# JuanLuisGonzalez/FAL_net

Measured on AMD Instinct MI355X. Metric: stereo-pairs/sec Stage-1 step @256x512 N=49, higher is better.
Workload: dtype bf16; 1 GPU; Stage-1 training step (BASELINE configs[1]), batch 8/GPU, 256x512, N=49, seeded weights, seeded VGG19; global_batch=8, parallelism=dp1, launch=eager launches, recorded sequences issued by falnet_replay (C)

## Files before the change

### fal_net_amd/_lib.py

```python
import ctypes as C
import os
import threading

import torch

F32, BF16, F16 = 0, 1, 2
ACT_NONE, ACT_ELU, ACT_RELU = 0, 1, 2
OUT_NHWC, OUT_PLANAR_F32 = 0, 1
CPAD = 32

DETERMINISTIC = os.environ.get("FALNET_DETERMINISTIC") == "1"

def ab(name, default):
    if os.environ.get("FALNET_AB") != "1":
        return default
    return os.environ.get(name, default)


_LIB_PATH = os.environ.get("FALNET_LIB") or os.path.join(os.path.dirname(os.path.abspath(__file__)), "libfalnet_hip.so")


class Src(C.Structure):
    _fields_ = [("ptr", C.c_void_p), ("C", C.c_int32), ("H", C.c_int32), ("W", C.c_int32),
                ("sb", C.c_int64), ("sy", C.c_int64), ("sx", C.c_int64)]


class Conv(C.Structure):
    _fields_ = [("src", Src * 2), ("nsrc", C.c_int32), ("IH", C.c_int32), ("IW", C.c_int32),
                ("weight", C.c_void_p), ("cin_total", C.c_int32), ("ntaps", C.c_int32),
                ("tap_dy", C.c_int32 * 9), ("tap_dx", C.c_int32 * 9), ("tap_w", C.c_int32 * 9),
                ("w_taps", C.c_int32), ("w_rows", C.c_int32), ("isy", C.c_int32), ("isx", C.c_int32),
                ("B", C.c_int32), ("TH", C.c_int32), ("TW", C.c_int32),
                ("osy", C.c_int32), ("osx", C.c_int32), ("ooy", C.c_int32), ("oox", C.c_int32),
                ("out", C.c_void_p), ("OH", C.c_int32), ("OW", C.c_int32), ("Cout", C.c_int32),
                ("out_cstride", C.c_int32), ("out_layout", C.c_int32), ("bias", C.c_void_p),
                ("addend", C.c_void_p), ("act", C.c_int32), ("actout", C.c_void_p),
                ("actout_kind", C.c_int32), ("dtype", C.c_int32), ("ksplit", C.c_int32), ("splitk_ws", C.c_void_p),
                ("splitk_ws_bytes", C.c_int64), ("variant", C.c_int32), ("pool_out", C.c_void_p),
                ("pool_mode", C.c_int32), ("pool_actout_kind", C.c_int32), ("pool_actout", C.c_void_p), ("weight_up2", C.c_void_p),
                ("scratch", C.c_void_p), ("scratch_bytes", C.c_int64)]


class Wgrad(C.Structure):
    _fields_ = [("src", Src * 2), ("nsrc", C.c_int32), ("IH", C.c_int32), ("IW", C.c_int32),
                ("gout", C.c_void_p), ("gC", C.c_int32), ("ntaps", C.c_int32),
                ("tap_dy", C.c_int32 * 9), ("tap_dx", C.c_int32 * 9), ("isy", C.c_int32), ("isx", C.c_int32),
                ("B", C.c_int32), ("TH", C.c_int32), ("TW", C.c_int32), ("cin_total", C.c_int32),
                ("nsplit", C.c_int32), ("partial", C.c_void_p), ("dtype", C.c_int32), ("variant", C.c_int32), ("bias_grad", C.c_void_p),
                ("cout", C.c_int32), ("up2", C.c_int32)]


class ReduceDesc(C.Structure):
    _fields_ = [("partial", C.c_void_p), ("grad", C.c_void_p), ("nsplit", C.c_int32), ("ntaps", C.c_int32),
                ("w_rows", C.c_int32), ("cin_total", C.c_int32), ("cout", C.c_int32), ("cin", C.c_int32),
                ("c0_real", C.c_int32), ("c0_pad", C.c_int32), ("groups", C.c_int32), ("block_begin", C.c_int32)]


class PackDesc(C.Structure):
    _fields_ = [("w", C.c_void_p), ("wf", C.c_void_p), ("wd", C.c_void_p), ("cout", C.c_int32), ("cin", C.c_int32),
                ("taps", C.c_int32), ("c0_real", C.c_int32), ("c0_pad", C.c_int32), ("cin_pad", C.c_int32),
                ("cout_pad", C.c_int32), ("block_begin", C.c_int32), ("no_update", C.c_int32), ("reserved", C.c_int32)]


class PackUp2Desc(C.Structure):
    _fields_ = [("w", C.c_void_p), ("wu", C.c_void_p), ("cout", C.c_int32), ("cin", C.c_int32), ("cin_pad", C.c_int32), ("cout_pad", C.c_int32),
                ("block_begin", C.c_int32), ("reserved", C.c_int32), ("wdd", C.c_void_p)]


class Cmd(C.Structure):
    _fields_ = [("op", C.c_int32), ("stream", C.c_int32), ("event", C.c_int32), ("nint", C.c_int32), ("nflt", C.c_int32), ("reserved", C.c_int32),
                ("iarg", C.c_uint64 * 18), ("farg", C.c_double * 8)]


CMD_RECORD, CMD_WAIT = -1, -2


class BiasGradDesc(C.Structure):
    _fields_ = [("g", C.c_void_p), ("db", C.c_void_p), ("npix", C.c_int64), ("gC", C.c_int32), ("cout", C.c_int32),
                ("blocks", C.c_int32), ("block_begin", C.c_int32)]


class Aug(C.Structure):
    _fields_ = [("src", C.c_uint64 * 2), ("H", C.c_int32), ("W", C.c_int32), ("rw", C.c_int32), ("rh", C.c_int32), ("x1", C.c_int32),
                ("y1", C.c_int32), ("flip", C.c_int32), ("reserved", C.c_int32), ("gamma", C.c_double), ("bright", C.c_double),
                ("cb", (C.c_double * 3) * 2)]


_P, _I, _L, _F, _D = C.c_void_p, C.c_int, C.c_int64, C.c_float, C.c_double
SIGNATURES = {
    "falnet_version": [],
    "falnet_last_error": [],
    "falnet_channel_pad": [_I],
    "falnet_set_device": [_I],
    "falnet_set_deterministic": [_I],
    "falnet_get_deterministic": [],
    "falnet_conv2d": [C.POINTER(Conv), _P],
    "falnet_conv3x3_c3": [_P, _P, _P, _P, _I, _I, _I, _I, _I, _I, _P],
    "falnet_conv2d_multi": [C.POINTER(Conv), _I, _P],
    "falnet_conv2d_kernel_name": [C.POINTER(Conv), C.c_char_p, _I],
    "falnet_wgrad_workspace_bytes": [C.POINTER(Wgrad)],
    "falnet_wgrad": [C.POINTER(Wgrad), _P],
    "falnet_wgrad_fuses_bias": [C.POINTER(Wgrad)],
    "falnet_wgrad_reduce": [_P, _I, _I, _I, _I, _P, _I, _I, _I, _I, _I, _P],
    "falnet_bias_grad": [_P, _L, _I, _I, _P, _I, _I, _P],
    "falnet_pack_weights_batched": [_P, _I, _I, _I, _P],
    "falnet_adam_pack_batched": [_P, _I, _I, _I, _L, _L, _L, _P, _F, _F, _F, _F, _P, _P],
    "falnet_adam_ranges": [_P, _L, _L, _L, _P, _I, _P, _F, _F, _F, _F, _P, _P],
    "falnet_adam_tick": [_P, _P, _P],
    "falnet_adam_pack_batched_wd": [_P, _I, _I, _I, _L, _L, _L, _P, _F, _F, _F, _F, _D, _P, _P],
    "falnet_adam_ranges_wd": [_P, _L, _L, _L, _P, _P, _I, _P, _F, _F, _F, _F, _P, _P],
    "falnet_pack_up2_batched": [_P, _I, _I, _I, _P],
    "falnet_wgrad_reduce_batched": [_P, _I, _I, _I, _P],
    "falnet_wgrad_reduce_blocks": [_I, _I, _I],
    "falnet_bias_grad_batched": [_P, _I, _I, _I, _P],
    "falnet_bias_grad_batched_det": [_P, _I, _I, _I, _P, _L, _P],
    "falnet_pack_weights": [_P, _I, _I, _I, _I, _I, _I, _I, _P, _P, _I, _P],
    "falnet_nchw_to_nhwc": [_P, _P, _I, _I, _I, _I, _I, _I, _P],
    "falnet_nhwc_to_nchw": [_P, _P, _I, _I, _I, _I, _I, _I, _P],
    "falnet_upsample_bwd": [_P, _P, _P, _I, _I, _I, _I, _I, _I, _I, _P],
    "falnet_wgrad_const_plane": [_P, _P, _L, _P, _L, _P, _I, _I, _I, _I, _I, _I, _I, _I, _I, _P],
    "falnet_maxpool2_fwd": [_P, _P, _I, _I, _I, _I, _I, _P],
    "falnet_maxpool2_bwd": [_P, _P, _P, _P, _I, _I, _I, _I, _I, _P],
    "falnet_act_bwd": [_P, _P, _P, _L, _I, _I, _P],
    "falnet_med_head_fwd": [_P, _P, _P, _P, _P, _P, _P, _I, _I, _I, _I, _P],
    "falnet_med_head_bwd": [_P, _P, _P, _P, _P, _P, _P, _P, _P, _P, _I, _I, _I, _I, _P],
    "falnet_med_head_bwd_nhwc": [_P, _P, _P, _P, _P, _P, _P, _P, _P, _P, _I, _I, _I, _I, _I, _I, _P],
    "falnet_med_head_kernel_name": [_I, _I, _I, _I, C.c_char_p, _I],
    "falnet_med_masks_fwd": [_P, _P, _P, _P, _P, _P, _I, _I, _I, _I, _P],
    "falnet_med_maskr_acfalse_fwd": [_P, _P, _P, _P, _P, _I, _I, _I, _I, _P],
    "falnet_l1_fwd": [_P, _P, _P, _I, _I, _L, _F, _P, _I, _P],
    "falnet_l1_bwd": [_P, _P, _P, _I, _I, _L, _F, _P, _P, _I, _P],
    "falnet_mse_fwd": [_P, _P, _L, _I, _F, _P, _I, _I, _P],
    "falnet_mse_bwd": [_P, _P, _L, _I, _F, _P, _P, _I, _P],
    "falnet_l1_fwd_bwd": [_P, _P, _I, _I, _L, _F, _P, _P, _P, _P],
    "falnet_l1_fwd_bwd_add": [_P, _P, _I, _I, _L, _F, _P, _P, _P, _P, _P],
    "falnet_mse_fwd_bwd": [_P, _P, _L, _I, _F, _P, _F, _P, _P, _I, _P],
    "falnet_mse3_fwd_bwd": [_P, _P, _P, _P, _P, _P, _P, _P, _I, _P],
    "falnet_smooth_fwd_bwd": [_P, _P, _I, _I, _I, _I, _I, _F, _F, _P, _P, _P, _P],
    "falnet_smooth_fwd": [_P, _P, _I, _I, _I, _I, _I, _F, _F, _P, _I, _P],
    "falnet_smooth_bwd": [_P, _P, _I, _I, _I, _I, _I, _F, _F, _P, _P, _I, _P],
    "falnet_step_scalars": [_P, _F, _P, _P],
    "falnet_mask_mix": [_P, _P, _P, _P, _I, _I, _L, _P],
    "falnet_adam_step": [_P, _P, _P, _P, _L, _F, _F, _F, _F, _I, _F, _P],
    "falnet_adam_step_dev": [_P, _P, _P, _P, _L, _P, _F, _F, _F, _F, _P],
    "falnet_adam_step_guarded": [_P, _P, _P, _P, _L, _P, _F, _F, _F, _F, _P, _P],
    "falnet_adam_step_wd": [_P, _P, _P, _P, _L, _P, _P, _I, _P, _F, _F, _F, _F, _P, _P],
    "falnet_grad_guard": [_P, _L, _P, _P],
    "falnet_loss_scale_update": [_P, _F, _F, _I, _F, _F, _P],
    "falnet_loss_seeds": [_P, _P, _P, _I, _P],
    "falnet_hflip": [_P, _P, _L, _I, _P],
    "falnet_resample_u8": [_P, _P, _I, _I, _I, _I, _I, _P, _P, _I, _P],
    "falnet_augment_normalize": [_P, _I, _I, _I, _I, _I, _I, _I, _D, _D, _D, _D, _D, _F, _F, _F, _P, _P],
    "falnet_augment_batch": [_P, _P, _I, _I, _I, _F, _F, _F, _P, _P, _P],
    "falnet_rowmax": [_P, _P, _I, _L, _P],
    "falnet_gemm_f32_small": [_P, _L, _L, _P, _L, _L, _P, _I, _I, _I, _I, _P],
    "falnet_resize_planar": [_P, _P, _L, _I, _I, _I, _I, _I, _F, _P],
    "falnet_disp_prologue": [_P, _P, _F, _F, _P, _P, _P, _I, _I, _I, _P],
    "falnet_occlusion_mask": [_P, _P, _P, _I, _I, _I, _I, _I, _P],
    "falnet_mirror_weight": [_P, _P, _P, _I, _I, _I, _I, _I, _P],
    "falnet_replay_op_index": [C.c_char_p],
    "falnet_replay_op_args": [_I, C.POINTER(C.c_int), C.POINTER(C.c_int)],
    "falnet_replay": [_P, _I, _P, _I, _P, _I, C.POINTER(C.c_int)],
    "falnet_fill_f32": [_P, _L, _F, _P],
    "falnet_copy_bytes": [_P, _P, _L, _P],
    "falnet_spin": [_I, _P],
    "falnet_mfma_probe": [_P, _P, _I, _I, _P],
    "falnet_percentile_workspace_bytes": [_I],
    "falnet_percentile_f32": [_P, _L, _I, _D, _P, _P, _P],
    "falnet_disp_to_plasma_u8": [_P, _P, _P, _P, _I, _I, _I, _P],
    "falnet_image_to_u8": [_P, _F, _F, _F, _P, _I, _I, _I, _P],
    "falnet_feature_to_u8": [_P, _P, _L, _P],
    "falnet_local_norm": [_P, _F, _F, _F, _P, _P, _P, _I, _I, _I, _I, _P],
    "falnet_point_cloud": [_P, _F, _F, _F, _F, _P, _D, _D, _P, _P, _I, _I, _I, _P],
    "falnet_metrics_workspace_bytes": [],
    "falnet_depth_median_scale": [_P, _P, _I, _I, _I, _D, _D, _P, _P, _P],
    "falnet_depth_errors": [_P, _P, _I, _I, _I, _D, _P, _D, _D, _P, _P, _P],
    "falnet_epe": [_P, _I, _I, _P, _I, _I, _I, _I, _P, _P, _P],
    "falnet_view_errors": [_P, _P, _F, _F, _F, _I, _I, _I, _P, _P, _P],
}
_RESTYPES = {"falnet_last_error": C.c_char_p, "falnet_wgrad_workspace_bytes": C.c_int64, "falnet_percentile_workspace_bytes": C.c_int64,
             "falnet_metrics_workspace_bytes": C.c_int64}

_lib = None
_TLS = threading.local()
EXPECTED_VERSION = 600


def lib():
    global _lib
    if _lib is None:
        if not os.path.exists(_LIB_PATH):
            raise RuntimeError(
                f"{_LIB_PATH} is missing: build it with `python -m fal_net_amd._build` "
                "(there is no CPU or PyTorch fallback for the FAL_netB kernels)")
        l = C.CDLL(_LIB_PATH)
        for name, args in SIGNATURES.items():
            fn = getattr(l, name)
            fn.argtypes = args
            fn.restype = _RESTYPES.get(name, C.c_int)
        got = l.falnet_version()
        if got != EXPECTED_VERSION:
            raise RuntimeError(f"{_LIB_PATH} reports falnet_version() = {got}, this binding expects {EXPECTED_VERSION}: rebuild it "
                               "(`python -m fal_net_amd._build`; experiment builds: `--ab <tag>`)")
        if DETERMINISTIC:
            l.falnet_set_deterministic(1)
        _lib = _LibProxy(l)
    return _lib


_MASK64 = (1 << 64) - 1


def _int_arg(a):
    if a is None:
        return 0
    if isinstance(a, int):
        return a & _MASK64
    if isinstance(a, C.c_void_p):
        return a.value or 0
    if isinstance(a, (C.Structure, C.Array)):
        return C.addressof(a)
    obj = getattr(a, "_obj", None)
    if obj is not None:
        return C.addressof(obj)
    if isinstance(a, C._SimpleCData):
        return int(a.value or 0) & _MASK64
    raise TypeError(f"cannot record argument {a!r}")


class Segment:

    def __init__(self, cmds, streams, events, keep):
        self.n = len(cmds)
        self.cmds = (Cmd * max(self.n, 1))(*cmds)
        self.streams = (C.c_void_p * len(streams))(*streams)
        self.events = (C.c_void_p * max(len(events), 1))(*events)
        self.ns, self.ne = len(streams), len(events)
        self.failed = C.c_int(-1)
        self._keep = keep
        self._fn = _lib._cdll.falnet_replay

    def run(self, main_ptr):
        self.streams[0] = main_ptr
        rc = self._fn(self.cmds, self.n, self.streams, self.ns, self.events, self.ne, C.byref(self.failed))
        if rc != 0:
            msg = _lib._cdll.falnet_last_error().decode(errors="replace")
            raise RuntimeError(f"libfalnet_hip replay failed at command {self.failed.value} (rc={rc}): {msg}")


class SegmentChain:

    def __init__(self, parts):
        self.parts = parts

    def run(self, main_ptr):
        for p in self.parts:
            if isinstance(p, Segment):
                p.run(main_ptr)
            else:
                p()


class Recorder:

    def __init__(self, main_ptr):
        self.streams = [int(main_ptr or 0)]
        self.events, self.cmds, self.keep = [], [], []
        self.parts = []
        self._ops = {}

    def cut(self, fn):
        self.parts.append(self.cmds)
        self.parts.append(fn)
        self.cmds = []

# ... 164 lines not shown
```

### fal_net_amd/csrc/conv.hip

```cpp
#include <limits.h>
#include <stdlib.h>
#include <type_traits>
#include "common.h"
#include "conv_epilogue.h"

#define CONV_THREADS 256
#define CONV_BM 128
#define ROWB 64
#define ROWP 80

template <typename T> struct KC;
template <> struct KC<float> { static constexpr int value = 16; };
template <> struct KC<bf16_t> { static constexpr int value = 32; };
template <> struct KC<f16_t> { static constexpr int value = 32; };

template <typename T, int MT, int NT, typename RowOff, typename PoolOff = NoPool>
__device__ __forceinline__ void epilogue_nhwc(const falnet_conv_t& p, f32x16 (&acc)[MT][NT], float* stage, int nbase, int lane,
                                              RowOff rowoff, PoolOff pooloff = PoolOff()) {
    constexpr bool POOL = !std::is_same<PoolOff, NoPool>::value;
    constexpr int PITCHF = NT * 32 + 4;
    constexpr int CS = NT * 4;
    constexpr int RPP = 64 / CS;
    constexpr int PASSES = 32 / RPP;
    const int r = lane & 31, h = lane >> 5;
// ... 1326 lines not shown
    if constexpr (sizeof(T) == 2) {
#pragma unroll
        for (int ks = 0; ks < 2; ++ks)
#pragma unroll
            for (int nt = 0; nt < NT; ++nt)
#pragma unroll
                for (int j = 0; j < 8; ++j) bfr[ks][nt][j] = (short)H16<T>::bits(wv[ks][nt][j]);
    }
    constexpr int MT = PT_TH / 4;
    auto a_elem = [&](const float* base, int k0, int k1) -> float {
        const int o0 = k0 < 27 ? ((k0 / 9) * PH + (k0 % 9) / 3) * PW + (k0 % 9) % 3 : 0;
        const int o1 = k1 < 27 ? ((k1 / 9) * PH + (k1 % 9) / 3) * PW + (k1 % 9) % 3 : 0;
        const float v = base[h ? o1 : o0];
        return ((h ? k1 : k0) < 27) ? v : 0.f;
    };
    const int cstride = p.out_cstride;
    const int tiles_x = (p.OW + PT_TW - 1) / PT_TW;
    C3_STAMP(2);
    __syncthreads();
    C3_STAMP(3);
    for (int tt = 0; tt < C3_TPW; ++tt) {
        if (tt == 1) C3_STAMP(4);
        const int tix = tix0 + tt;
        if (tix >= tiles_x) break;
        const int tx0 = tix * PT_TW;
#pragma unroll 1
        for (int mt = 0; mt < MT; ++mt) {
            f32x16 acc[1][NT];
#pragma unroll
            for (int nt = 0; nt < NT; ++nt)
#pragma unroll
                for (int j = 0; j < 16; ++j) acc[0][nt][j] = 0.f;
            const float* base = patch + (wave * MT + mt) * PW + tt * PT_TW + r;
            if constexpr (sizeof(T) == 2) {
#pragma unroll
                for (int ks = 0; ks < 2; ++ks) {
                    s16x8_t afr;
#pragma unroll
                    for (int j = 0; j < 8; ++j) afr[j] = (short)H16<T>::bits(a_elem(base, ks * 16 + j, ks * 16 + 8 + j));
#pragma unroll
                    for (int nt = 0; nt < NT; ++nt) acc[0][nt] = H16<T>::mma(bfr[ks][nt], afr, acc[0][nt]);
                }
            } else {
#pragma unroll
                for (int ks = 0; ks < 16; ++ks) {
                    const float a = a_elem(base, ks * 2, ks * 2 + 1);
#pragma unroll
                    for (int nt = 0; nt < NT; ++nt) acc[0][nt] = __builtin_amdgcn_mfma_f32_32x32x2f32(wv[ks][nt][0], a, acc[0][nt], 0, 0, 0);
                }
            }
            auto pixoff = [&](int) -> int64_t {
                const int y = ty0 + wave * MT + mt, xx = tx0 + r;
                return (y < p.OH && xx < p.OW) ? (((int64_t)b * p.OH + y) * p.OW + xx) * cstride : (int64_t)-1;
            };
            epilogue_direct<T, 1, NT, decltype(pixoff), NoPool, 1, false, true>(p, acc, bias, 0, lane, pixoff);
        }
    }
    C3_STAMP(5);
    asm volatile("s_waitcnt vmcnt(0)" ::: "memory");
    C3_STAMP(6);
}
#undef C3_STAMP

template <typename T, bool SWAP>
static void launch_conv(const falnet_conv_t& p, int bn, dim3 grid, hipStream_t st) {
    if (bn == 128)
        hipLaunchKernelGGL(HIP_KERNEL_NAME(conv_igemm_kernel<T, 128, SWAP>), grid, dim3(CONV_THREADS), 0, st, p);
    else if (bn == 64)
        hipLaunchKernelGGL(HIP_KERNEL_NAME(conv_igemm_kernel<T, 64, SWAP>), grid, dim3(CONV_THREADS), 0, st, p);
    else
        hipLaunchKernelGGL(HIP_KERNEL_NAME(conv_igemm_kernel<T, 32, SWAP>), grid, dim3(CONV_THREADS), 0, st, p);
}

static bool falnet_mfma16_enabled() {
    static const bool on = [] { const char* e = falnet_ab_env("FALNET_MFMA16"); return !(e && e[0] == '0'); }();
    return on;
}

enum class ConvFamily {
    Gather,
    Patch,
    WeightStationary,
    Dma,
    S2fDma,
    Up2Dma,
    Deep,
    Dma2,
    Dma16,
    Up2d,
    Wave32,
    Wave64p,
};
struct ConvChoice {
    ConvFamily family;
    int bn, kcb, tps, adb, th, nwaves, flip, swap;
};

static bool g_disable_patch = [] { const char* e = falnet_ab_env("FALNET_DISABLE_PATCH"); return e && e[0] == '1'; }();
static int g_patch_kcb = [] { const char* e = falnet_ab_env("FALNET_PATCH_KCB"); return e ? atoi(e) : 128; }();


bool falnet_conv_dma_applicable(const falnet_conv_t& p, int min_oh);
int falnet_conv_dma_launch(const falnet_conv_t& p, int flip, hipStream_t st, int th);
bool falnet_conv_dma2_applicable(const falnet_conv_t& p, int th);
int falnet_conv_dma2_launch(const falnet_conv_t& p, int flip, hipStream_t st, int th);
int falnet_conv_dma16_launch(const falnet_conv_t& p, int flip, hipStream_t st, int th);
bool falnet_conv_up2_dma_applicable(const falnet_conv_t& p);
int falnet_conv_up2_dma_launch(const falnet_conv_t& p, hipStream_t st);
bool falnet_conv_wave32_applicable(const falnet_conv_t& p);
int falnet_conv_wave32_launch(const falnet_conv_t& p, int flip, hipStream_t st);
bool falnet_conv_wave64p_applicable(const falnet_conv_t& p);
int falnet_conv_wave64p_launch(const falnet_conv_t& p, int flip, hipStream_t st);
bool falnet_conv_up2d_applicable(const falnet_conv_t& p);
int falnet_conv_up2d_launch(const falnet_conv_t& p, hipStream_t st);
bool falnet_conv_deep_applicable(const falnet_conv_t& p);
int falnet_conv_deep_launch(const falnet_conv_t& p, hipStream_t st);
int falnet_conv_deep_mtiles(const falnet_conv_t& p);
bool falnet_conv_s2d_dma_applicable(const falnet_conv_t* d, int n);
int falnet_conv_s2d_dma_launch(const falnet_conv_t* d, hipStream_t st);
bool falnet_conv_s2f_dma_applicable(const falnet_conv_t& p);
int falnet_conv_s2f_dma_launch(const falnet_conv_t& p, hipStream_t st);

static int choose_conv_kernel(const falnet_conv_t& p, ConvChoice& c) {
    const bool planar = p.out_layout == FALNET_OUT_PLANAR_F32;
    int ctot = 0;
    for (int s = 0; s < p.nsrc; ++s) ctot += p.src[s].C;
    bool dense3x3 = p.ntaps == 9 && p.isy == 1 && p.isx == 1 && p.osy == 1 && p.osx == 1 && p.ooy == 0 && p.oox == 0 &&
                    p.TH == p.OH && p.TW == p.OW && p.TH == p.IH && p.TW == p.IW && p.TW >= 16;
    int flip = -1;
    if (dense3x3 && p.w_taps == 9) {
        bool fwd = true, bwd = true;
        for (int t = 0; t < 9; ++t) {
            const int sp = (p.tap_dy[t] + 1) * 3 + (p.tap_dx[t] + 1);
            if (p.tap_dy[t] < -1 || p.tap_dy[t] > 1 || p.tap_dx[t] < -1 || p.tap_dx[t] > 1) fwd = bwd = false;
            fwd = fwd && p.tap_w[t] == sp;
            bwd = bwd && p.tap_w[t] == 8 - sp;
        }
        flip = fwd ? 0 : (bwd ? 1 : -1);
    }
    dense3x3 = dense3x3 && flip >= 0;
    const int esz = p.dtype == FALNET_F32 ? 4 : 2;
    bool c128 = true;
    for (int s = 0; s < p.nsrc; ++s) c128 = c128 && (p.src[s].C % (128 / esz) == 0);
    int variant = p.variant;
    int forced_bn = 0;
    if (variant == 11 || variant == 12) {
        forced_bn = variant == 11 ? 32 : 64;
        if (p.w_rows % forced_bn != 0 || p.pool_out) {
            falnet_set_error("conv2d: variant %d (gather, %d channels per workgroup) not applicable to this launch", variant, forced_bn);
            return -2;
        }
        variant = 1;
    }
    if (g_disable_patch) variant = 1;
    switch (variant) {
        case 0: case 1: case 2: case 3: case 4: case 5: case 6: case 7: case 8: case 9: case 10:
        case 13: case 15: case 16: case 17: case 18: case 19: case 20: case 21: case 22: case 23: case 24: case 25: case 26: case 27: case 29:
            break;
        default:
            falnet_set_error("conv2d: unknown variant %d", variant);
            return -1;
    }
    if (variant == 19) {
        if (!falnet_conv_deep_applicable(p)) {
            falnet_set_error("conv2d: variant 19 needs a 16-bit nine-tap stride-1/2 launch on maps of at most 128 positions (128 %% (TH TW) == 0), dense NHWC output, "
                             "w_rows %% 64 == 0, ksplit = cin_total / 32 or / 64 (a multiple of 4), scratch for the partial tiles and the split-K workspace");
            return -2;
        }
        c.flip = 0;
        c.swap = 0;
        c.family = ConvFamily::Deep;
        c.bn = 64; c.kcb = p.ksplit * 32 == p.cin_total ? 1 : 2; c.tps = 9; c.adb = 1; c.th = 0; c.nwaves = falnet_conv_deep_mtiles(p);
        return 0;
    }
    if (variant == 15) {
        if (!falnet_conv_s2f_dma_applicable(p)) {
            falnet_set_error("conv2d: variant 15 needs a canonical 16-bit 3x3 stride-2 pad-1 NHWC launch (>= 8 x 32 outputs) with sources at the input size");
            return -2;
        }
        c.flip = 0;
        c.swap = 0;
        c.family = ConvFamily::S2fDma;
        c.bn = 64; c.kcb = 32; c.tps = 9; c.adb = 1; c.th = 8; c.nwaves = 8;
        return 0;
    }
    if (variant == 29) {
        if (!(dense3x3 && falnet_conv_wave64p_applicable(p))) {
            falnet_set_error("conv2d: variant 29 needs a 16-bit dense 3x3 stride-1 launch over ONE 64-channel source at the launch size, planar f32 output of <= 4 channels, no addend / activation-gradient operand / pool / split-K");
            return -2;
        }
        c.flip = flip;
        c.swap = 0;
        c.family = ConvFamily::Wave64p;
        c.bn = 16; c.kcb = 32; c.tps = 9; c.adb = 1; c.th = 1; c.nwaves = 8;
        return 0;
    }
    if (variant == 27) {
        if (!(dense3x3 && falnet_conv_wave32_applicable(p))) {
            falnet_set_error("conv2d: variant 27 needs a 16-bit dense 3x3 stride-1 NHWC launch over ONE 32-channel source at the launch size with a 32-row packed weight, no pool / split-K");
            return -2;
        }
        c.flip = flip;
        c.swap = 0;
        c.family = ConvFamily::Wave32;
        c.bn = 32; c.kcb = 32; c.tps = 9; c.adb = 1; c.th = 1; c.nwaves = 8;
        return 0;
    }
    if (variant == 26) {
        if (!(falnet_conv_up2d_applicable(p) && p.ntaps == 4 && p.isy == 1 && p.isx == 1 && p.osy == 1 && p.osx == 1 && p.ooy == 0 && p.oox == 0 && p.TH == p.OH && p.TW == p.OW)) {
            falnet_set_error("conv2d: variant 26 needs a 16-bit NHWC launch over ONE source at exactly twice the output map (>= 16 x 32), w_taps = ntaps = 4, cin_total = 4 C, no pool / split-K");
            return -2;
        }
        c.flip = 0;
        c.swap = 0;
        c.family = ConvFamily::Up2d;
        c.bn = 64; c.kcb = 32; c.tps = 4; c.adb = 1; c.th = 16; c.nwaves = 8;
        return 0;
    }
    if (variant == 18) {
        if (!(dense3x3 && flip == 0 && !p.addend && !p.actout && falnet_conv_up2_dma_applicable(p))) {
            falnet_set_error("conv2d: variant 18 needs a 16-bit dense 3x3 forward launch over ONE source at exactly half the launch size, weight_up2 set, no residual / activation-gradient operand");
            return -2;
        }
        c.flip = 0;
        c.swap = 0;
        c.family = ConvFamily::Up2Dma;
        c.bn = 32; c.kcb = 64; c.tps = 16; c.adb = 1; c.th = 16; c.nwaves = 8;
        return 0;
    }
    if (variant >= 23 && variant <= 25) {
        const int th = variant == 23 ? 16 : (variant == 24 ? 4 : 8);
        if (!(dense3x3 && falnet_conv_dma_applicable(p, th)) || (th != 16 && (p.pool_out || planar)) || (planar && p.pool_out)) {
            falnet_set_error("conv2d: variant %d needs a 16-bit dense 3x3 stride-1 launch (>= %d x 32 positions%s) with sources at the launch size or half of it",
                             variant, th, th != 16 ? ", NHWC output, no fused pool" : "");
            return -2;
        }
        c.flip = flip;
        c.swap = 0;
        c.family = ConvFamily::Dma16;
        c.bn = 64; c.kcb = 32; c.tps = 9; c.adb = 1; c.th = th; c.nwaves = th == 4 ? 4 : 8;
        return 0;
    }
    if (variant == 21 || variant == 22) {
        const int th = variant == 21 ? 16 : 32;
        if (!(dense3x3 && falnet_conv_dma2_applicable(p, th))) {
            falnet_set_error("conv2d: variant %d needs a 16-bit dense 3x3 stride-1 NHWC launch (>= %d x 32 positions) with sources at the launch size or half of it", variant, th);
            return -2;
        }
        c.flip = flip;
        c.swap = 0;
        c.family = ConvFamily::Dma2;
        c.bn = 64; c.kcb = 16; c.tps = 9; c.adb = 1; c.th = th; c.nwaves = th / 4;
        return 0;
    }
    if (variant == 13 || variant == 17 || variant == 20) {
        const int th = variant == 17 ? 4 : (variant == 20 ? 8 : 16);
        if (!(dense3x3 && falnet_conv_dma_applicable(p, th)) || (th != 16 && p.pool_out)) {
            falnet_set_error("conv2d: variant %d needs a 16-bit dense 3x3 stride-1 launch (>= %d x 32 positions%s) with sources at the launch size or half of it",
                             variant, th, th != 16 ? ", no fused pool" : "");
            return -2;
        }
        c.flip = flip;
        c.swap = 0;
        c.family = ConvFamily::Dma;
        c.bn = 64; c.kcb = 64; c.tps = 9; c.adb = 1; c.th = th; c.nwaves = th == 4 ? 4 : 8;
        return 0;
    }
    if (variant == 10 || variant == 16) {
        bool ok = dense3x3 && ctot * esz <= 128 && ctot * esz % 64 == 0 && p.src[0].C * esz % 64 == 0;
        for (int s = 0; s < p.nsrc && ok; ++s)
            ok = (p.src[s].H == p.IH || 2 * p.src[s].H == p.IH) && (p.src[s].W == p.IW || 2 * p.src[s].W == p.IW) && p.src[s].C < 4096;
        if (!ok) {
            falnet_set_error("conv2d: variant 10 needs a dense 3x3 launch with <= 128 B of input channels per pixel");
            return -2;
        }
        c.flip = flip;
        c.swap = 0;
        c.family = ConvFamily::WeightStationary;
        c.bn = (p.w_rows % 64 == 0 && p.Cout > 32) ? 64 : 32;
        c.kcb = ctot * esz / 64;
        c.tps = 9; c.adb = variant == 16; c.th = (c.bn == 64 ? 8 : 16) >> c.adb; c.nwaves = 8;
        return 0;
    }
    if (variant >= 2 && (!dense3x3 || (variant == 2 && !c128) || ((variant == 3 || variant == 5 || variant == 6 || variant == 8) && ctot / (64 / esz) < 2) ||
                         ((variant == 6 || variant == 7) && p.OH < 16))) {
        falnet_set_error("conv2d: variant %d not applicable to this launch", variant);
        return -2;
    }
    if (variant == 0) {
        if (!dense3x3 || p.TW < 32) variant = 1;
        else if (c128 && g_patch_kcb == 128) variant = 2;
        else if (ctot / (64 / esz) >= 2 && g_patch_kcb != 0) variant = 3;
        else variant = 4;
    }
    const bool bn64 = p.w_rows % 64 == 0 && p.Cout > 32;
    c.flip = flip;
    c.swap = planar ? 1 : 0;
    c.family = variant >= 2 ? ConvFamily::Patch : ConvFamily::Gather;
    if (p.pool_out && c.family == ConvFamily::Gather) {
        falnet_set_error("conv2d: the fused max pool needs a halo-patch variant (dense 3x3 stride-1 launch)");
        return -2;
    }
    if (c.family == ConvFamily::Gather) {
        c.bn = forced_bn ? forced_bn : (p.w_rows % 128 == 0 && p.Cout > 64) ? 128 : (bn64 ? 64 : 32);
        c.kcb = 64; c.tps = 1; c.adb = 0; c.th = 0; c.nwaves = 4;
        return 0;
    }
    c.th = variant >= 8 ? 4 : (variant >= 6 ? 16 : 8);
    c.nwaves = (variant == 6 || variant == 7) ? 8 : 4;
    const int tiles = p.B * ((p.OW + PT_TW - 1) / PT_TW) * ((p.OH + c.th - 1) / c.th);
    const bool bn128 = p.w_rows % 128 == 0 && p.Cout > 64 && (c.th == 16 || tiles >= 256);
    switch (variant) {
        case 2: c.bn = bn128 ? 128 : (bn64 ? 64 : 32); c.kcb = 128; c.tps = 1; c.adb = ctot / (128 / esz) > 1; break;
        case 3: case 6: c.bn = bn128 ? 128 : (bn64 ? 64 : 32); c.kcb = 64; c.tps = 1; c.adb = 1; break;
        case 8: c.bn = bn64 ? 64 : 32; c.kcb = 64; c.tps = 1; c.adb = 1; break;
        case 5: c.bn = bn64 ? 64 : 32; c.kcb = 64; c.tps = 9; c.adb = 1; break;
        default: c.bn = bn64 ? 64 : 32; c.kcb = 64; c.tps = 9; c.adb = 0; break;
    }
    if (p.pool_out && (c.th / (c.nwaves / (c.bn >= 128 ? 2 : 1))) % 2 != 0) {
        falnet_set_error("conv2d: variant %d gives every wave an odd number of rows: no fused max pool", variant);
        return -2;
    }
    return 0;
}

static bool ws2_whole_lines(const falnet_conv_t& p) {
    static const bool on = !(falnet_ab_env("FALNET_WS2_FULL") && atoi(falnet_ab_env("FALNET_WS2_FULL")) == 0);
    return on && p.nsrc == 1 && (int64_t)p.src[0].C * (p.dtype == FALNET_F32 ? 4 : 2) == 128;
}

static int launch_gather(const falnet_conv_t& p, const ConvChoice& c, hipStream_t st) {
    const bool planar = p.out_layout == FALNET_OUT_PLANAR_F32;
    const int bn = c.bn;
    const int64_t M = (int64_t)p.B * p.TH * p.TW;
    int ksplit = p.ksplit > 1 ? p.ksplit : 1;
    if (ksplit > 1) {
        FALNET_CHECK_ARG(!planar && p.splitk_ws && p.Cout % 8 == 0, "conv2d: split-K needs an NHWC output and a workspace");
        FALNET_CHECK_ARG(M * p.w_rows * 4 <= p.splitk_ws_bytes, "conv2d: split-K workspace too small (%lld needed)", (long long)(M * p.w_rows * 4));
    }
    const dim3 grid((unsigned)((M + CONV_BM - 1) / CONV_BM), (unsigned)((p.Cout + bn - 1) / bn), (unsigned)ksplit);
#define GATHER_L(T)                                          \
    if (planar) launch_conv<T, true>(p, bn, grid, st);       \
    else launch_conv<T, false>(p, bn, grid, st);
    FALNET_DISPATCH_DTYPE(p.dtype, GATHER_L);
#undef GATHER_L
    if (ksplit > 1) {
        const int64_t total = M * (p.w_rows / 8);
        const unsigned eg = (unsigned)((total + 255) / 256 > 2048 ? 2048 : (total + 255) / 256);
#define SPLITK_E(T) hipLaunchKernelGGL(splitk_epilogue_kernel<T>, dim3(eg), dim3(256), 0, st, p)
        FALNET_DISPATCH_DTYPE(p.dtype, SPLITK_E);
#undef SPLITK_E
    }
    return 0;
}

static int launch_patch(const falnet_conv_t& p, const ConvChoice& c, hipStream_t st) {
    const int tiles_x = (p.OW + PT_TW - 1) / PT_TW, tiles_y = (p.OH + c.th - 1) / c.th;
    const dim3 grid((unsigned)(p.B * tiles_x * tiles_y), (unsigned)((p.Cout + c.bn - 1) / c.bn));
    bool launched = false;
#define TRY_PATCH(T, BN, KCB, TPS, ADB, TH, NW)                                                                              \
    if (!launched && c.bn == BN && c.kcb == KCB && c.tps == TPS && c.adb == (ADB ? 1 : 0) && c.th == TH) {                     \
    hipLaunchKernelGGL(HIP_KERNEL_NAME(conv3x3_patch_kernel<T, BN, KCB, TPS, ADB, TH, NW>), grid, dim3(NW * 64), 0, st, p, \
                       tiles_x, tiles_y, c.flip);                                                                          \
    launched = true;                                                                                                       \
    }
#define PATCH_TABLE(T)                                                                                   \
    TRY_PATCH(T, 128, 128, 1, true, 8, 4) TRY_PATCH(T, 64, 128, 1, true, 8, 4) TRY_PATCH(T, 32, 128, 1, true, 8, 4)      \
    TRY_PATCH(T, 128, 128, 1, false, 8, 4) TRY_PATCH(T, 64, 128, 1, false, 8, 4) TRY_PATCH(T, 32, 128, 1, false, 8, 4)   \
    TRY_PATCH(T, 128, 64, 1, true, 8, 4) TRY_PATCH(T, 64, 64, 1, true, 8, 4) TRY_PATCH(T, 32, 64, 1, true, 8, 4)         \
    TRY_PATCH(T, 64, 64, 9, false, 8, 4) TRY_PATCH(T, 32, 64, 9, false, 8, 4)                                             \
    TRY_PATCH(T, 64, 64, 9, true, 8, 4) TRY_PATCH(T, 32, 64, 9, true, 8, 4)                                               \
    TRY_PATCH(T, 128, 64, 1, true, 16, 8) TRY_PATCH(T, 64, 64, 1, true, 16, 8) TRY_PATCH(T, 32, 64, 1, true, 16, 8)      \
    TRY_PATCH(T, 64, 64, 9, false, 16, 8) TRY_PATCH(T, 32, 64, 9, false, 16, 8)                                           \
    TRY_PATCH(T, 64, 64, 1, true, 4, 4) TRY_PATCH(T, 32, 64, 1, true, 4, 4)                                               \
    TRY_PATCH(T, 64, 64, 9, false, 4, 4) TRY_PATCH(T, 32, 64, 9, false, 4, 4)
    FALNET_DISPATCH_DTYPE(p.dtype, PATCH_TABLE);
#undef PATCH_TABLE
#undef TRY_PATCH
    FALNET_CHECK_ARG(launched, "conv2d: no instantiation for bn=%d kcb=%d tps=%d adb=%d th=%d", c.bn, c.kcb, c.tps, c.adb, c.th);
    return 0;
}

static int launch_ws(const falnet_conv_t& p, const ConvChoice& c, hipStream_t st) {
    const int ws_th = c.th;
    const int tiles_x = (p.OW + PT_TW - 1) / PT_TW, tiles_y = (p.OH + ws_th - 1) / ws_th;
    const int ny = (p.Cout + c.bn - 1) / c.bn, ntiles = p.B * tiles_x * tiles_y;
    int gx = 256 / ny;
    if (gx < 1) gx = 1;
    if (gx > ntiles) gx = ntiles;
    const dim3 grid((unsigned)gx, (unsigned)ny);
    const bool m16 = falnet_mfma16_enabled();
    const bool ws2_full = ws2_whole_lines(p);
#define LAUNCH_WS1(K, T, BN, NCH) do { if (m16 && sizeof(T) == 2) hipLaunchKernelGGL(HIP_KERNEL_NAME(K<T, BN, NCH, true>), grid, dim3(512), 0, st, p, tiles_x, tiles_y, c.flip); \
                                   else hipLaunchKernelGGL(HIP_KERNEL_NAME(K<T, BN, NCH, false>), grid, dim3(512), 0, st, p, tiles_x, tiles_y, c.flip); } while (0)
#define LAUNCH_WS2(T, BN, NCH) do { if (NCH == 2 && ws2_full) { if (m16 && sizeof(T) == 2) hipLaunchKernelGGL(HIP_KERNEL_NAME(conv3x3_ws2_kernel<T, BN, 2, true, true>), grid, dim3(512), 0, st, p, tiles_x, tiles_y, c.flip); \
                                     else hipLaunchKernelGGL(HIP_KERNEL_NAME(conv3x3_ws2_kernel<T, BN, 2, false, true>), grid, dim3(512), 0, st, p, tiles_x, tiles_y, c.flip); } \
                                 else LAUNCH_WS1(conv3x3_ws2_kernel, T, BN, NCH); } while (0)
#define LAUNCH_WS(T, BN, NCH) do { if (c.adb) LAUNCH_WS2(T, BN, NCH); else LAUNCH_WS1(conv3x3_ws_kernel, T, BN, NCH); } while (0)
#define WS_TABLE(T)                                                                                 \
    if (c.bn == 64) { if (c.kcb == 2) LAUNCH_WS(T, 64, 2); else LAUNCH_WS(T, 64, 1); }              \
    else { if (c.kcb == 2) LAUNCH_WS(T, 32, 2); else LAUNCH_WS(T, 32, 1); }
    FALNET_DISPATCH_DTYPE(p.dtype, WS_TABLE);
#undef WS_TABLE
#undef LAUNCH_WS
#undef LAUNCH_WS1
#undef LAUNCH_WS2
    return 0;
}

static int ws_symbol(char* buf, int len, const char* t, const falnet_conv_t& p, const ConvChoice& c) {
    const int m16 = (int)(falnet_mfma16_enabled() && p.dtype != FALNET_F32);
    if (c.adb) return snprintf(buf, len, "_Z18conv3x3_ws2_kernelI%sLi%dELi%dELb%dELb%dEEv13falnet_conv_tiii", t, c.bn, c.kcb, m16, (int)(c.kcb == 2 && ws2_whole_lines(p)));
    return snprintf(buf, len, "_Z17conv3x3_ws_kernelI%sLi%dELi%dELb%dEEv13falnet_conv_tiii", t, c.bn, c.kcb, m16);
}

struct ConvFamilyRow {
    ConvFamily family;
    int (*symbol)(char* buf, int len, const char* t, const falnet_conv_t& p, const ConvChoice& c);
    int (*launch)(const falnet_conv_t& p, const ConvChoice& c, hipStream_t st);
};
#define SYMBOL(...) [](char* buf, int len, const char* t, const falnet_conv_t& p, const ConvChoice& c) { return snprintf(buf, len, __VA_ARGS__); }
#define LAUNCH(...) [](const falnet_conv_t& p, const ConvChoice& c, hipStream_t st) { return __VA_ARGS__; }
static const ConvFamilyRow conv_families[] = {
    {ConvFamily::Gather, SYMBOL("_Z17conv_igemm_kernelI%sLi%dELb%dEEv13falnet_conv_t", t, c.bn, c.swap), launch_gather},
    {ConvFamily::Patch, SYMBOL("_Z20conv3x3_patch_kernelI%sLi%dELi%dELi%dELb%dELi%dELi%dEEv13falnet_conv_tiii", t, c.bn, c.kcb, c.tps, c.adb, c.th, c.nwaves), launch_patch},
    {ConvFamily::WeightStationary, ws_symbol, launch_ws},
    {ConvFamily::Dma, SYMBOL("_Z18conv3x3_dma_kernelI%sLi%dELi%dEEv13falnet_conv_tiiii", t, c.th, c.nwaves), LAUNCH(falnet_conv_dma_launch(p, c.flip, st, c.th))},
    {ConvFamily::S2fDma, SYMBOL("_Z22conv3x3_s2f_dma_kernelI%sLi%dEEv13falnet_conv_tiii", t, c.bn), LAUNCH(falnet_conv_s2f_dma_launch(p, st))},
    {ConvFamily::Up2Dma, SYMBOL("_Z22conv3x3_up2_dma_kernelI%sEv13falnet_conv_tiiiii", t), LAUNCH(falnet_conv_up2_dma_launch(p, st))},
    {ConvFamily::Deep, SYMBOL("_Z19conv3x3_deep_kernelI%sLi%dELi%dEEv13falnet_conv_t18falnet_deep_geom_t", t, c.kcb, c.nwaves), LAUNCH(falnet_conv_deep_launch(p, st))},
    {ConvFamily::Dma2, SYMBOL("_Z19conv3x3_dma2_kernelI%sLb%dELi%dEEv13falnet_conv_tiiiii", t, p.pool_out ? 1 : 0, c.nwaves), LAUNCH(falnet_conv_dma2_launch(p, c.flip, st, c.th))},
    {ConvFamily::Dma16, SYMBOL("_Z20conv3x3_dma16_kernelI%sLb%dELi%dELi%dELb%dEEv13falnet_conv_tiiii", t, p.pool_out ? 1 : 0, c.th, c.nwaves, p.out_layout == FALNET_OUT_PLANAR_F32 ? 1 : 0),
     LAUNCH(falnet_conv_dma16_launch(p, c.flip, st, c.th))},
    {ConvFamily::Up2d, SYMBOL("_Z25conv2x2_up2d_dma16_kernelI%sEv13falnet_conv_tiii", t), LAUNCH(falnet_conv_up2d_launch(p, st))},
    {ConvFamily::Wave32, SYMBOL("_Z21conv3x3_wave32_kernelI%sEv13falnet_conv_tiiii", t), LAUNCH(falnet_conv_wave32_launch(p, c.flip, st))},
    {ConvFamily::Wave64p, SYMBOL("_Z22conv3x3_wave64p_kernelI%sEv13falnet_conv_tiiii", t), LAUNCH(falnet_conv_wave64p_launch(p, c.flip, st))},
};
#undef SYMBOL
#undef LAUNCH

static const ConvFamilyRow* conv_family_row(ConvFamily f) {
    for (const ConvFamilyRow& r : conv_families)
        if (r.family == f) return &r;
    falnet_set_error("conv2d: kernel family %d has no table row", (int)f);
    return nullptr;
}

extern "C" int falnet_conv2d_kernel_name(const falnet_conv_t* pp, char* buf, int len) {
    FALNET_CHECK_ARG(pp && buf && len > 0, "conv2d_kernel_name: bad argument");
    ConvChoice c;
    if (int r = choose_conv_kernel(*pp, c)) return r;
    const ConvFamilyRow* row = conv_family_row(c.family);
    if (!row) return -1;
    row->symbol(buf, len, pp->dtype == FALNET_BF16 ? "DF16b" : pp->dtype == FALNET_F16 ? "DF16_" : "f", *pp, c);
    return 0;
}

extern "C" int falnet_conv2d(const falnet_conv_t* pp, void* stream) {
    FALNET_ENTER(stream);
    FALNET_CHECK_ARG(pp, "conv2d: null descriptor");
    const falnet_conv_t& p = *pp;
    FALNET_CHECK_ARG(p.dtype == FALNET_F32 || p.dtype == FALNET_BF16 || p.dtype == FALNET_F16, "conv2d: bad dtype %d", p.dtype);
    const int kc = p.dtype == FALNET_F32 ? 16 : 32;
    FALNET_CHECK_ARG(p.nsrc == 1 || p.nsrc == 2, "conv2d: nsrc=%d", p.nsrc);
    int ctot = 0;
    for (int s = 0; s < p.nsrc; ++s) {
        if (int r = check_src(p.src[s], kc, "conv2d")) return r;
        ctot += p.src[s].C;
    }
    FALNET_CHECK_ARG(ctot <= p.cin_total, "conv2d: sources carry %d channels, packed weight row holds %d", ctot, p.cin_total);
    FALNET_CHECK_ARG(p.ntaps >= 1 && p.ntaps <= 9 && p.w_taps >= 1, "conv2d: ntaps=%d", p.ntaps);
    for (int t = 0; t < p.ntaps; ++t) FALNET_CHECK_ARG(p.tap_w[t] >= 0 && p.tap_w[t] < p.w_taps, "conv2d: tap_w[%d] out of range", t);
    FALNET_CHECK_ARG(p.B > 0 && p.TH > 0 && p.TW > 0 && p.IH > 0 && p.IW > 0 && p.OH > 0 && p.OW > 0, "conv2d: empty shape");
    FALNET_CHECK_ARG(p.weight && (p.out || p.pool_out) && p.Cout > 0 && p.w_rows >= p.Cout && p.w_rows % 32 == 0, "conv2d: bad weight/out (Cout=%d w_rows=%d)", p.Cout, p.w_rows);
    FALNET_CHECK_ARG(!p.pool_out || (p.out_layout == FALNET_OUT_NHWC && !p.actout && p.ksplit <= 1 && (p.pool_mode == 0 || p.pool_mode == 1)),
                     "conv2d: pool_out needs a plain NHWC launch (no actout / split-K) and pool_mode 0|1");
    FALNET_CHECK_ARG((int64_t)p.B * p.OH * p.OW * (p.out_layout == FALNET_OUT_PLANAR_F32 ? p.Cout : 1) < (1ll << 31), "conv2d: output too large for 32-bit pixel index");
    const bool planar = p.out_layout == FALNET_OUT_PLANAR_F32;
    FALNET_CHECK_ARG(!planar || (!p.addend && !p.actout), "conv2d: planar output supports bias/act epilogue only");
    if (p.ksplit > 1 && p.variant != 19 && falnet_deterministic()) {
        falnet_set_error("conv2d: split-K (f32 atomics) is not available in deterministic mode");
        return -2;
    }
    hipStream_t st = (hipStream_t)stream;
    ConvChoice c;
    if (int r = choose_conv_kernel(p, c)) return r;
    const ConvFamilyRow* row = conv_family_row(c.family);
    if (!row) return -1;
    if (int r = row->launch(p, c, st)) return r;
    FALNET_RETURN_LAUNCH();
}

extern "C" int falnet_conv3x3_c3(const float* x_nchw, const float* w_oihw, const float* bias, void* out, int B, int H, int W, int Cout,
                                 int act, int dtype, void* stream) {
    FALNET_ENTER(stream);
    FALNET_CHECK_ARG(x_nchw && w_oihw && out && B > 0 && H > 0 && W > 0, "conv3x3_c3: bad argument");
    FALNET_CHECK_ARG(Cout == 32 || Cout == 64, "conv3x3_c3: Cout must be 32 or 64 (got %d)", Cout);
    falnet_conv_t p = {};
    p.IH = p.OH = H;
    p.IW = p.OW = W;
    p.out = out;
    p.Cout = Cout;
    p.out_cstride = Cout;
    p.bias = bias;
    p.act = act;
#ifdef C3_STAMPS
    if (const char* e = getenv("FALNET_C3_STAMP_PTR")) p.pool_actout = reinterpret_cast<const void*>(strtoull(e, nullptr, 10));
#endif
    const int tiles_x = ((W + PT_TW - 1) / PT_TW + C3_TPW - 1) / C3_TPW , tiles_y = (H + PT_TH - 1) / PT_TH;
    const dim3 grid((unsigned)(B * tiles_x * tiles_y));
    hipStream_t st = (hipStream_t)stream;
#define C3_L(T)                                                                                                                                          \
    if (Cout == 64) hipLaunchKernelGGL(HIP_KERNEL_NAME(conv3x3_c3_kernel<T, 2>), grid, dim3(CONV_THREADS), 0, st, x_nchw, w_oihw, p, tiles_x, tiles_y); \
    else hipLaunchKernelGGL(HIP_KERNEL_NAME(conv3x3_c3_kernel<T, 1>), grid, dim3(CONV_THREADS), 0, st, x_nchw, w_oihw, p, tiles_x, tiles_y);
    FALNET_CHECK_ARG(dtype == FALNET_F32 || dtype == FALNET_BF16 || dtype == FALNET_F16, "conv3x3_c3: bad dtype %d", dtype);
    FALNET_DISPATCH_DTYPE(dtype, C3_L);
#undef C3_L
    FALNET_RETURN_LAUNCH();
}

extern "C" int falnet_conv2d_multi(const falnet_conv_t* descs, int n, void* stream) {
    FALNET_ENTER(stream);
    FALNET_CHECK_ARG(descs && n >= 1 && n <= 4, "conv2d_multi: 1..4 descriptors");
    if (descs[0].variant == 14) {
        for (int i = 0; i < n; ++i)
            for (int s = 0; s < descs[i].nsrc && s < 2; ++s)
                if (int r = check_src(descs[i].src[s], 32, "conv2d_multi")) return r;
        FALNET_CHECK_ARG(falnet_conv_s2d_dma_applicable(descs, n), "conv2d_multi: variant 14 needs the four parity classes of one 16-bit 3x3 stride-2 data gradient");
        return falnet_conv_s2d_dma_launch(descs, (hipStream_t)stream);
    }
    if (descs[0].ksplit > 1 && falnet_deterministic()) {
        falnet_set_error("conv2d_multi: split-K (f32 atomics) is not available in deterministic mode");
        return -2;
    }
    falnet_conv4_t pp;
    int64_t maxM = 0;
    ConvChoice c0;
    for (int i = 0; i < n; ++i) {
        const falnet_conv_t& p = descs[i];
        FALNET_CHECK_ARG(p.dtype == descs[0].dtype && p.w_rows == descs[0].w_rows && p.Cout == descs[0].Cout && p.out_layout == FALNET_OUT_NHWC &&
                         p.ksplit == descs[0].ksplit && p.nsrc >= 1 && p.nsrc <= 2 && p.weight && p.out && p.ntaps >= 1 && p.ntaps <= 9,
                         "conv2d_multi: members must share dtype / Cout / w_rows / ksplit and be plain NHWC gather launches");
        if (p.ksplit > 1) {
            const int64_t need = (int64_t)p.B * p.TH * p.TW * p.w_rows * 4;
            FALNET_CHECK_ARG(p.splitk_ws && p.Cout % 8 == 0 && need <= p.splitk_ws_bytes, "conv2d_multi: split-K needs a workspace of %lld bytes per member", (long long)need);
            for (int j = 0; j < i; ++j) {
                const char* a = (const char*)p.splitk_ws; const char* bq = (const char*)descs[j].splitk_ws;
                const int64_t needj = (int64_t)descs[j].B * descs[j].TH * descs[j].TW * descs[j].w_rows * 4;
                FALNET_CHECK_ARG(a + need <= bq || bq + needj <= a, "conv2d_multi: split-K workspace regions of members %d and %d overlap", j, i);
            }
        }
        for (int s = 0; s < p.nsrc; ++s)
            if (int r = check_src(p.src[s], p.dtype == FALNET_F32 ? 16 : 32, "conv2d_multi")) return r;
        ConvChoice c;
        falnet_conv_t q = p;
        q.variant = (p.variant == 11 || p.variant == 12) ? p.variant : 1;
        if (int r = choose_conv_kernel(q, c)) return r;
        if (i == 0) c0 = c;
        const int64_t M = (int64_t)p.B * p.TH * p.TW;
        maxM = M > maxM ? M : maxM;
        pp.c[i] = p;
    }
    for (int i = n; i < 4; ++i) pp.c[i] = descs[0];
    const int ksplit = descs[0].ksplit > 1 ? descs[0].ksplit : 1;
    const dim3 grid((unsigned)((maxM + CONV_BM - 1) / CONV_BM), (unsigned)((descs[0].Cout + c0.bn - 1) / c0.bn), (unsigned)(n * ksplit));
    hipStream_t st = (hipStream_t)stream;
#define LAUNCH_MULTI(T)                                                                                              \
    do {                                                                                                             \
        if (c0.bn == 128) hipLaunchKernelGGL(HIP_KERNEL_NAME(conv_igemm_multi_kernel<T, 128>), grid, dim3(CONV_THREADS), 0, st, pp, ksplit); \
        else if (c0.bn == 64) hipLaunchKernelGGL(HIP_KERNEL_NAME(conv_igemm_multi_kernel<T, 64>), grid, dim3(CONV_THREADS), 0, st, pp, ksplit); \
        else hipLaunchKernelGGL(HIP_KERNEL_NAME(conv_igemm_multi_kernel<T, 32>), grid, dim3(CONV_THREADS), 0, st, pp, ksplit);  \
    } while (0)
    FALNET_DISPATCH_DTYPE(descs[0].dtype, LAUNCH_MULTI);
#undef LAUNCH_MULTI
    if (ksplit > 1) {
        const int64_t total = maxM * (descs[0].w_rows / 8);
        const dim3 eg((unsigned)((total + 255) / 256 > 1024 ? 1024 : (total + 255) / 256), (unsigned)n);
#define SPLITK_M(T) hipLaunchKernelGGL(splitk_epilogue_multi_kernel<T>, eg, dim3(256), 0, st, pp)
        FALNET_DISPATCH_DTYPE(descs[0].dtype, SPLITK_M);
#undef SPLITK_M
    }
    FALNET_RETURN_LAUNCH();
}
```

### fal_net_amd/csrc/conv_dma.hip

```cpp
#include <stdlib.h>
#include "conv_epilogue.h"

#ifndef FALNET_DMA_ROW_REUSE
#define FALNET_DMA_ROW_REUSE 1
#endif
#ifndef FALNET_DMA_EPI_AHEAD
#define FALNET_DMA_EPI_AHEAD -1
#endif
#ifndef FALNET_DMA16_EPI_AHEAD
#define FALNET_DMA16_EPI_AHEAD 0
#endif

#define CD_ZERO_BYTES 32768
__device__ uint4 g_cd_zero[CD_ZERO_BYTES / 16] = {};

typedef __attribute__((address_space(3))) void* cd_lptr_t;

__device__ __forceinline__ void cd_glds16(const void* gsrc, unsigned lds_dst) {
    unsigned keep;
    asm volatile("s_mov_b32 %0, m0\n\ts_mov_b32 m0, %2\n\ts_nop 0\n\tglobal_load_lds_dwordx4 %1, off\n\ts_mov_b32 m0, %0"
                 : "=&s"(keep)
                 : "v"(gsrc), "s"(lds_dst)
                 : "memory");
}
// ... 402 lines not shown
        q.c0 += KCV;
        q.kofs += KCV;
        if (q.s == 0 && q.c0 >= C0) {
            q.s = 1;
            q.c0 = 0;
            tile_offsets(q.tile, 1);
        }
    };
    auto issue_piece = [&](const Cur& q, int buf, int i) {
        const unsigned dst0 = lds_base + buf * BUF;
        if (i < KP) {
            const int id = wave + NWAVES * i;
            const T* sbase = (q.s == 0 ? sptr[0] + sbat[0] : sptr[1] + sbat[1]) + q.c0;
            if (id < A_PIECES) cd_glds16(sbase + a_off[i], dst0 + id * 1024);
        } else {
            const int wid = wave + NWAVES * (i - KP);
            if (wid < B_PIECES) cd_glds16(wptr + q.kofs + w_off[i - KP], dst0 + A_BYTES + wid * 1024);
        }
    };

    int a_lane[3];
#pragma unroll
    for (int dx = 0; dx < 3; ++dx) a_lane[dx] = ((wave * MT) * C2_PW + dx + r) * 32 + ((h ^ (((dx + r) >> 3) & 1)) << 4);
    const int b_lane = A_BYTES + r * 32 + ((h ^ ((r >> 3) & 1)) << 4);

    f32x16 acc[NT][MT][1];
#pragma unroll
    for (int mt = 0; mt < MT; ++mt)
#pragma unroll
        for (int nt = 0; nt < NT; ++nt)
#pragma unroll
            for (int j = 0; j < 16; ++j) acc[nt][mt][0][j] = 0.f;
    Cur qi = {(int)blockIdx.x, 0, 0, 0, 0};
    if (total > 0) {
        tile_offsets(qi.tile, 0);
#pragma unroll
        for (int i = 0; i < KP + KW; ++i) issue_piece(qi, 0, i);
        advance(qi);
    }
    int ctile = blockIdx.x, cc = 0;
    for (int it = 0; it < total; ++it) {
        asm volatile("s_waitcnt vmcnt(0) lgkmcnt(0)" ::: "memory");
        __builtin_amdgcn_s_barrier();
        const bool more = it + 1 < total;
        int bo = (it & 1) * BUF;
        asm volatile("" : "+s"(bo));
        const char* const Bf = lds;
        int aa[3];
#pragma unroll
        for (int dx = 0; dx < 3; ++dx) aa[dx] = a_lane[dx] + bo;
        const int bb = b_lane + bo;
        s16x8_t fa[3][MT + 2], fb[2][NT];
        auto a_read = [&](int dx, int rs) { return *reinterpret_cast<const s16x8_t*>(Bf + aa[dx] + rs * ROWB); };
        auto b_read = [&](int st, int set) {
            const int t = (st % 3) * 3 + st / 3;
#pragma unroll
            for (int nt = 0; nt < NT; ++nt) fb[set][nt] = *reinterpret_cast<const s16x8_t*>(Bf + bb + (t * BN + nt * 32) * 32);
        };
#pragma unroll
        for (int rs = 0; rs < 4; ++rs) fa[0][rs] = a_read(0, rs);
        b_read(0, 0);
#pragma unroll
        for (int st = 0; st < 9; ++st) {
            const int dx = st / 3, dy = st % 3;
            if (st + 1 < 9) b_read(st + 1, (st + 1) & 1);
            if (dy == 0) fa[dx][4] = a_read(dx, 4);
            if (dy == 1) fa[dx][5] = a_read(dx, 5);
            if (dx + 1 < 3) {
                if (dy == 1) { fa[dx + 1][0] = a_read(dx + 1, 0); fa[dx + 1][1] = a_read(dx + 1, 1); }
                if (dy == 2) { fa[dx + 1][2] = a_read(dx + 1, 2); fa[dx + 1][3] = a_read(dx + 1, 3); }
            }
#pragma unroll
            for (int half = 0; half < 2; ++half) {
                const int i = 2 * st + half;
                if (i < KP + KW && more) issue_piece(qi, (it + 1) & 1, i);
#pragma unroll
                for (int m2 = 0; m2 < 2; ++m2) {
                    const int mt = 2 * half + m2;
#pragma unroll
                    for (int nt = 0; nt < NT; ++nt) acc[nt][mt][0] = H16<T>::mma(fb[st & 1][nt], fa[dx][mt + dy], acc[nt][mt][0]);
                }
            }
            if (st == 8) __builtin_amdgcn_sched_group_barrier(0x100, 0, 0);
            else if (dy == 1 && dx < 2) __builtin_amdgcn_sched_group_barrier(0x100, 5, 0);
            else if (dy == 2) __builtin_amdgcn_sched_group_barrier(0x100, 4, 0);
            else __builtin_amdgcn_sched_group_barrier(0x100, 3, 0);
            __builtin_amdgcn_sched_group_barrier(0x008, MT * NT, 0);
        }
        if (more) advance(qi);
        if (++cc == nchunks) {
            cc = 0;
            int b, ty0, tx0;
            tile_coords(ctile, b, ty0, tx0);
            ctile += gridDim.x;
            const int cstride = p.out_cstride;
            const int x = tx0 + r;
            auto pixoff = [&](int mt) -> int64_t {
                const int y = ty0 + wave * MT + mt;
                if (!(y < p.OH && x < p.OW)) return (int64_t)-1;
                return (((int64_t)b * p.OH + y) * p.OW + x) * cstride;
            };
            auto pooloff = [&](int mt) -> int64_t {
                const int py = (ty0 + wave * MT + mt) >> 1, px = x >> 1, PH = p.OH >> 1, PW = p.OW >> 1;
                return (py < PH && px < PW) ? (((int64_t)b * PH + py) * PW + px) * cstride : (int64_t)-1;
            };
#pragma unroll
            for (int nt = 0; nt < NT; ++nt) {
                float bias[1][16];
                load_bias16_lds(lds_bias, 32 * nt, h, bias);
                if constexpr (POOL) epilogue_direct<T, MT, 1, decltype(pixoff), decltype(pooloff), -1, false, true>(p, acc[nt], bias, n0 + 32 * nt, lane, pixoff, pooloff);
                else epilogue_direct<T, MT, 1, decltype(pixoff), NoPool, -1, false, true>(p, acc[nt], bias, n0 + 32 * nt, lane, pixoff);
#pragma unroll
                for (int mt = 0; mt < MT; ++mt)
#pragma unroll
                    for (int j = 0; j < 16; ++j) acc[nt][mt][0][j] = 0.f;
            }
        }
    }
}

bool falnet_conv_dma2_applicable(const falnet_conv_t& p, int th) {
    return falnet_conv_dma_applicable(p, th) && p.out_layout == FALNET_OUT_NHWC;
}

int falnet_conv_dma2_launch(const falnet_conv_t& p, int flip, hipStream_t st, int th) {
    const int tiles_x = (p.OW + 31) / 32, tiles_y = (p.OH + th - 1) / th;
    const int ntiles = p.B * tiles_x * tiles_y;
    const int ny = (p.Cout + 63) / 64;
    int gx = (th == 32 ? 256 : 512) / ny;
    if (gx < 1) gx = 1;
    if (gx > ntiles) gx = ntiles;
    const dim3 grid((unsigned)gx, (unsigned)ny);
    static const int skew_pct = [] { const char* e = falnet_ab_env("FALNET_DMA2_SKEW"); return e ? atoi(e) : 0; }();
    int cin = 0;
    for (int s = 0; s < p.nsrc; ++s) cin += p.src[s].C;
    const int skew = (th == 16 && gx * ny > 256) ? (int)((int64_t)skew_pct * (cin / 16) * 5200 / 100 / 64) : 0;
#define DMA2_K(T, PL, NW) hipLaunchKernelGGL(HIP_KERNEL_NAME(conv3x3_dma2_kernel<T, PL, NW>), grid, dim3(NW * 64), 0, st, p, tiles_x, tiles_y, flip, ntiles, skew)
#define DMA2_L(T)                                              \
    do {                                                       \
        if (th == 32) {                                        \
            if (p.pool_out) DMA2_K(T, true, 8);                \
            else DMA2_K(T, false, 8);                          \
        } else {                                               \
            if (p.pool_out) DMA2_K(T, true, 4);                \
            else DMA2_K(T, false, 4);                          \
        }                                                      \
    } while (0)
    FALNET_DISPATCH_16(p.dtype, DMA2_L);
#undef DMA2_L
#undef DMA2_K
    FALNET_RETURN_LAUNCH();
}

template <typename T, bool POOL, int TH, int NWAVES, bool PLANAR>
__global__ __launch_bounds__(NWAVES * 64, NWAVES == 8 ? 2 : 1) void conv3x3_dma16_kernel(const falnet_conv_t p, int tiles_x, int tiles_y, int flip, int ntiles) {
    constexpr int MT = TH / NWAVES, BN = 64, NT = BN / 32;
    static_assert(sizeof(T) == 2 && (MT == 1 || MT == 2) && (MT == 2 || !POOL), "16-bit operands; one or two rows per wave; the fused pool needs row pairs");
    constexpr int KCV = 32;
    constexpr int NPIX = (TH + 2) * CD_PW;
    constexpr int A_PIECES = (NPIX + 15) / 16, B_PIECES = 9 * BN / 16, NPIECES = A_PIECES + B_PIECES;
    constexpr int A_BYTES = A_PIECES * 1024, BUF = NPIECES * 1024;
    constexpr int ROWB = CD_PW * 64;
    __shared__ __attribute__((aligned(1024))) char lds[2 * BUF];
    __shared__ __attribute__((aligned(16))) float lds_bias[BN];
    const int tid = threadIdx.x, lane = tid & 63;
    const int wave = __builtin_amdgcn_readfirstlane(tid >> 6);
    const unsigned lds_base = (unsigned)(unsigned long)(cd_lptr_t)lds;
    const int r = lane & 31, h = lane >> 5;
    const int lp = lane & 15, lg = lane >> 4;
    const int n0 = blockIdx.y * BN;
    const char* const zero_page = reinterpret_cast<const char*>(g_cd_zero);
    stage_bias_lds(p, n0, BN, lds_bias);

    const int nsrc = p.nsrc, IH = p.IH, IW = p.IW;
    const int C0 = p.src[0].C, C1 = nsrc > 1 ? p.src[1].C : 0;
    const int nchunks = (C0 + C1) / KCV;
    int my_tiles = 0;
    for (int t = blockIdx.x; t < ntiles; t += gridDim.x) ++my_tiles;
    const int total = my_tiles * nchunks;

    constexpr int KP = (A_PIECES + NWAVES - 1) / NWAVES, KW = (B_PIECES + NWAVES - 1) / NWAVES;
    const int l4 = lane >> 2, segpos = lane & 3;
    const T* const wptr = reinterpret_cast<const T*>(p.weight);
    const T* const zero_t = reinterpret_cast<const T*>(zero_page);
    int64_t w_off[KW];
#pragma unroll
    for (int k = 0; k < KW; ++k) {
        const int wid = wave + NWAVES * k;
        const int tap = wid >> 2, co = n0 + ((wid & 3) << 4) + l4;
        const int gseg = segpos ^ (((l4 >> 2) & 1) << 1);
        w_off[k] = (wid < B_PIECES && co < p.w_rows) ? (int64_t)(co * p.w_taps + (flip ? 8 - tap : tap)) * p.cin_total + gseg * 8 : (int64_t)(zero_t - wptr);
    }
    const T* sptr[2] = {reinterpret_cast<const T*>(p.src[0].ptr), reinterpret_cast<const T*>(nsrc > 1 ? p.src[1].ptr : p.src[0].ptr)};
    struct TPos { int b, ty, tx; };
    TPos step_;
    {
        const int g = (int)gridDim.x;
        step_.tx = g % tiles_x;
        const int q = g / tiles_x;
        step_.ty = q % tiles_y;
        step_.b = q / tiles_y;
    }
    auto pos_of = [&](int tile) {
        TPos t;
        t.tx = tile % tiles_x;
        const int q = tile / tiles_x;
        t.ty = q % tiles_y;
        t.b = q / tiles_y;
        return t;
    };
    auto pos_next = [&](TPos& t) {
        t.tx += step_.tx;
        if (t.tx >= tiles_x) { t.tx -= tiles_x; ++t.ty; }
        t.ty += step_.ty;
        if (t.ty >= tiles_y) { t.ty -= tiles_y; ++t.b; }
        t.b += step_.b;
    };
    int pr_[KP], pc_[KP], a_lc[2][KP];
#pragma unroll
    for (int k = 0; k < KP; ++k) {
        const int pix = 16 * (wave + NWAVES * k) + l4;
        const int pr = pix / CD_PW, pc = pix - pr * CD_PW;
        pr_[k] = pix < NPIX ? pr : -(1 << 20);
        pc_[k] = pc;
#pragma unroll
        for (int s2 = 0; s2 < 2; ++s2) {
            const falnet_src_t& S = s2 == 0 ? p.src[0] : p.src[(nsrc > 1) ? 1 : 0];
            const int hs = S.H != IH ? 1 : 0, ws = S.W != IW ? 1 : 0;
            a_lc[s2][k] = ((pr - 1) >> hs) * (int)S.sy + ((pc - 1) >> ws) * (int)S.sx + (segpos ^ (((pc >> 2) & 1) << 1)) * 8;
        }
    }
    int a_off[KP];
    unsigned a_ok = 0;
    const T* a_base = sptr[0];
    auto tile_offsets = [&](const TPos& t, int s2) {
        const falnet_src_t& S = s2 == 0 ? p.src[0] : p.src[1];
        const int hs = S.H != IH ? 1 : 0, ws = S.W != IW ? 1 : 0;
        const int ty0 = t.ty * TH, tx0 = t.tx * 32;
        a_base = sptr[s2] + ((int64_t)t.b * S.sb + (int64_t)((ty0 >> hs) * (int)S.sy + (tx0 >> ws) * (int)S.sx));
        a_ok = 0;
#pragma unroll
        for (int k = 0; k < KP; ++k) {
            const int vy = ty0 - 1 + pr_[k], vx = tx0 - 1 + pc_[k];
            a_ok |= (vy >= 0 && vy < IH && vx >= 0 && vx < IW) ? 1u << k : 0u;
            a_off[k] = a_lc[s2][k];
        }
    };
    struct Cur { int tile, c, s, c0, kofs; TPos t; };
    auto advance = [&](Cur& q) {
        if (++q.c == nchunks) {
            q.c = 0; q.s = 0; q.c0 = 0; q.kofs = 0;
            q.tile += gridDim.x;
            pos_next(q.t);
            if (q.tile < ntiles) tile_offsets(q.t, 0);
            return;
        }
        q.c0 += KCV;
        q.kofs += KCV;
        if (q.s == 0 && q.c0 >= C0) {
            q.s = 1;
            q.c0 = 0;
            tile_offsets(q.t, 1);
        }
    };
    auto issue_piece = [&](const Cur& q, int buf, int i) {
        const unsigned dst0 = lds_base + buf * BUF;
        if (i < KP) {
            const int id = wave + NWAVES * i;
            const T* src = ((a_ok >> i) & 1) ? a_base + q.c0 + a_off[i] : zero_t;
            if (id < A_PIECES) cd_glds16(src, dst0 + id * 1024);
        } else {
            const int wid = wave + NWAVES * (i - KP);
            if (wid < B_PIECES) cd_glds16(wptr + q.kofs + w_off[i - KP], dst0 + A_BYTES + wid * 1024);
        }
    };

    int a_lane[3][2];
#pragma unroll
    for (int dx = 0; dx < 3; ++dx)
#pragma unroll
        for (int pt = 0; pt < 2; ++pt) {
            const int col = dx + 16 * pt + lp;
            a_lane[dx][pt] = ((wave * MT) * CD_PW + col) * 64 + ((lg ^ (((col >> 2) & 1) << 1)) << 4);
        }
    const int wrow = m16_row_channel(lp);
    const int b_lane = A_BYTES + wrow * 64 + ((lg ^ (((wrow >> 2) & 1) << 1)) << 4);

    Acc16 acc[MT][NT];
#pragma unroll
    for (int mt = 0; mt < MT; ++mt)
#pragma unroll
        for (int nt = 0; nt < NT; ++nt) acc[mt][nt].zero();
    Cur qi = {(int)blockIdx.x, 0, 0, 0, 0, pos_of((int)blockIdx.x)};
    TPos ct = qi.t;
    if (total > 0) {
        tile_offsets(qi.t, 0);
#pragma unroll
        for (int i = 0; i < KP + KW; ++i) issue_piece(qi, 0, i);
        advance(qi);
    }
    int cc = 0;
#ifdef FALNET_CD_STAMPS
    unsigned long long* stamp_out = reinterpret_cast<unsigned long long*>(p.splitk_ws);
    int stamp_i = 0;
#define CD16_STAMP()                                                                                 \
    do {                                                                                             \
        __builtin_amdgcn_sched_barrier(0);                                                           \
        unsigned long long t_;                                                                       \
        asm volatile("s_memtime %0\n\ts_waitcnt lgkmcnt(0)" : "=s"(t_)::"memory");                  \
        __builtin_amdgcn_sched_barrier(0);                                                           \
        if (stamp_out && blockIdx.x == 0 && blockIdx.y == 0 && lane == 0 && stamp_i < 256) stamp_out[wave * 256 + stamp_i] = t_; \
        ++stamp_i;                                                                                   \
    } while (0)
#else
#define CD16_STAMP() do {} while (0)
#endif
#if defined(FALNET_CD_STAMPS) && FALNET_CD_STAMPS == 2
#define CD16_A() do {} while (0)
#define CD16_B() CD16_STAMP()
#else
#define CD16_A() CD16_STAMP()
#define CD16_B() do {} while (0)
#endif
    for (int it = 0; it < total; ++it) {
        CD16_STAMP();
        asm volatile("s_waitcnt vmcnt(0) lgkmcnt(0)" ::: "memory");
        CD16_A();
        __builtin_amdgcn_s_barrier();
        CD16_STAMP();
        CD16_A();
        const bool more = it + 1 < total;
        int bo = (it & 1) * BUF;
        asm volatile("" : "+s"(bo));
        const char* const Bf = lds;
        int aa[3][2];
#pragma unroll
        for (int dx = 0; dx < 3; ++dx)
#pragma unroll
            for (int pt = 0; pt < 2; ++pt) aa[dx][pt] = a_lane[dx][pt] + bo;
        const int bb = b_lane + bo;
        s16x8_t fa[3][MT + 2][2], fb[2][NT][2];
        auto a_read = [&](int dx, int rs, int pt) { return *reinterpret_cast<const s16x8_t*>(Bf + aa[dx][pt] + rs * ROWB); };
        auto b_read = [&](int st, int set) {
            const int t = (st % 3) * 3 + st / 3;
#pragma unroll
            for (int nt = 0; nt < NT; ++nt)
#pragma unroll
                for (int ct = 0; ct < 2; ++ct) fb[set][nt][ct] = *reinterpret_cast<const s16x8_t*>(Bf + bb + (t * BN + nt * 32 + ct * 16) * 64);
        };
        static_assert(KP + KW <= 18, "two DMA issue slots per step");
#pragma unroll
        for (int rs = 0; rs < MT; ++rs)
#pragma unroll
            for (int pt = 0; pt < 2; ++pt) fa[0][rs][pt] = a_read(0, rs, pt);
        b_read(0, 0);
#pragma unroll
        for (int st = 0; st < 9; ++st) {
            const int dx = st / 3, dy = st % 3;
            if (st + 1 < 9) b_read(st + 1, (st + 1) & 1);
            if (dy < 2) { fa[dx][MT + dy][0] = a_read(dx, MT + dy, 0); fa[dx][MT + dy][1] = a_read(dx, MT + dy, 1); }
            if (dy == 2 && dx + 1 < 3) {
#pragma unroll
                for (int rs = 0; rs < MT; ++rs)
#pragma unroll
                    for (int pt = 0; pt < 2; ++pt) fa[dx + 1][rs][pt] = a_read(dx + 1, rs, pt);
            }
#pragma unroll
            for (int half = 0; half < 2; ++half) {
                const int i = 2 * st + half;
                if (i < KP + KW && more) issue_piece(qi, (it + 1) & 1, i);
#pragma unroll
                for (int mt = 0; mt < MT; ++mt)
#pragma unroll
                    for (int nt = (MT == 2 ? 0 : half); nt < (MT == 2 ? NT : half + 1); ++nt) {
                        if (MT == 2 && mt != half) continue;
#pragma unroll
                        for (int ct = 0; ct < 2; ++ct)
#pragma unroll
                            for (int pt = 0; pt < 2; ++pt)
                                acc[mt][nt].t[ct][pt] = H16<T>::mma16(fb[st & 1][nt][ct], fa[dx][mt + dy][pt], acc[mt][nt].t[ct][pt]);
                    }
            }
            if (st == 8) __builtin_amdgcn_sched_group_barrier(0x100, 0, 0);
            else if (dy == 2 && MT == 2) __builtin_amdgcn_sched_group_barrier(0x100, 8, 0);
            else __builtin_amdgcn_sched_group_barrier(0x100, 6, 0);
            if constexpr (MT == 2) __builtin_amdgcn_sched_group_barrier(0x008, 16, 0);
            else __builtin_amdgcn_sched_group_barrier(0x008, 8, 0);
        }
        CD16_STAMP();
        if (more) advance(qi);
        CD16_B();
        if (++cc == nchunks) {
            cc = 0;
            const int b = ct.b, ty0 = ct.ty * TH, tx0 = ct.tx * 32;
            pos_next(ct);
            const int cstride = p.out_cstride;
            const int x = tx0 + r;
            const int64_t obase = PLANAR ? ((int64_t)b * p.Cout * p.OH + ty0) * p.OW + tx0 : (((int64_t)b * p.OH + ty0) * p.OW + tx0) * cstride;
            auto pixoff = [&](int mt) -> int64_t {
                const int y = ty0 + wave * MT + mt;
                if (!(y < p.OH && x < p.OW)) return (int64_t)-1;
                if constexpr (PLANAR) return obase + ((wave * MT + mt) * p.OW + r);
                else return obase + ((wave * MT + mt) * p.OW + r) * cstride;
            };
            auto pooloff = [&](int mt) -> int64_t {
                const int py = (ty0 + wave * MT + mt) >> 1, px = x >> 1, PH = p.OH >> 1, PW = p.OW >> 1;
                return (py < PH && px < PW) ? (((int64_t)b * PH + py) * PW + px) * cstride : (int64_t)-1;
            };
#pragma unroll
            for (int nt = 0; nt < NT; ++nt) {
                float bias[1][16];
                load_bias16_lds(lds_bias, 32 * nt, h, bias);
                f32x16 v[MT][1];
#pragma unroll
                for (int mt = 0; mt < MT; ++mt) {
                    acc[mt][nt].to32(v[mt][0]);
                    acc[mt][nt].zero();
                }
                if constexpr (POOL) epilogue_direct<T, MT, 1, decltype(pixoff), decltype(pooloff), -1, false, true>(p, v, bias, n0 + 32 * nt, lane, pixoff, pooloff);
                else epilogue_direct<T, MT, 1, decltype(pixoff), NoPool, (PLANAR ? -1 : FALNET_DMA16_EPI_AHEAD), false, !PLANAR, PLANAR>(p, v, bias, n0 + 32 * nt, lane, pixoff);
                if (nt == 0) CD16_B();
            }
        } else {
            CD16_B();
        }
        CD16_STAMP();
    }
#undef CD16_STAMP
#undef CD16_A
#undef CD16_B
}

int falnet_conv_dma16_launch(const falnet_conv_t& p, int flip, hipStream_t st, int th) {
    const int tiles_x = (p.OW + 31) / 32, tiles_y = (p.OH + th - 1) / th;
    const int ntiles = p.B * tiles_x * tiles_y;
    const int ny = (p.Cout + 63) / 64;
    int gx = 256 / ny;
    if (gx < 1) gx = 1;
    if (gx > ntiles) gx = ntiles;
    const dim3 grid((unsigned)gx, (unsigned)ny);
    const bool planar = p.out_layout == FALNET_OUT_PLANAR_F32;
#define DMA16_K(T, PL, TH_, NW, PN) hipLaunchKernelGGL(HIP_KERNEL_NAME(conv3x3_dma16_kernel<T, PL, TH_, NW, PN>), grid, dim3(NW * 64), 0, st, p, tiles_x, tiles_y, flip, ntiles)
#define DMA16_L(T)                                        \
    do {                                                  \
        if (th == 4) DMA16_K(T, false, 4, 4, false);      \
        else if (th == 8) DMA16_K(T, false, 8, 8, false); \
        else if (planar) DMA16_K(T, false, 16, 8, true);  \
        else if (p.pool_out) DMA16_K(T, true, 16, 8, false); \
        else DMA16_K(T, false, 16, 8, false);             \
    } while (0)
    FALNET_DISPATCH_16(p.dtype, DMA16_L);
#undef DMA16_L
#undef DMA16_K
    FALNET_RETURN_LAUNCH();
}

template <typename T>
__global__ __launch_bounds__(512, 2) void conv2x2_up2d_dma16_kernel(const falnet_conv_t p, int tiles_x, int tiles_y, int ntiles) {
    constexpr int TH = 16, NWAVES = 8, MT = 2, BN = 64, NT = 2, KCV = 32;
    constexpr int NPIX = (TH + 1) * CD_PW;
    constexpr int A_PIECES = (NPIX + 15) / 16, B_PIECES = 4 * BN / 16, NPIECES = A_PIECES + B_PIECES;
    constexpr int A_BYTES = A_PIECES * 1024, BUF = NPIECES * 1024;
    constexpr int ROWB = CD_PW * 64;
    __shared__ __attribute__((aligned(1024))) char lds[2 * BUF];
    __shared__ __attribute__((aligned(16))) float lds_bias[BN];
    const int tid = threadIdx.x, lane = tid & 63;
    const int wave = __builtin_amdgcn_readfirstlane(tid >> 6);
    const unsigned lds_base = (unsigned)(unsigned long)(cd_lptr_t)lds;
    const int r = lane & 31;
    const int lp = lane & 15, lg = lane >> 4;
    const int n0 = blockIdx.y * BN;
    const char* const zero_page = reinterpret_cast<const char*>(g_cd_zero);
    stage_bias_lds(p, n0, BN, lds_bias);

    const falnet_src_t& S = p.src[0];
    const int GH = S.H, GW = S.W, CP = S.C;
    const int cpc = CP / KCV;
    const int nchunks = 4 * cpc;
    int my_tiles = 0;
    for (int t = blockIdx.x; t < ntiles; t += gridDim.x) ++my_tiles;
    const int total = my_tiles * nchunks;

    constexpr int KP = (A_PIECES + NWAVES - 1) / NWAVES, KW = (B_PIECES + NWAVES - 1) / NWAVES;
    static_assert(KP + KW <= 8, "two DMA issue slots per step");
    const int l4 = lane >> 2, segpos = lane & 3;
    const T* const wptr = reinterpret_cast<const T*>(p.weight);
    const T* const zero_t = reinterpret_cast<const T*>(zero_page);
    const T* const sptr = reinterpret_cast<const T*>(S.ptr);
    int64_t w_off[KW];
#pragma unroll
    for (int k = 0; k < KW; ++k) {
        const int wid = wave + NWAVES * k;
        const int tap = wid >> 2, co = n0 + ((wid & 3) << 4) + l4;
        const int gseg = segpos ^ (((l4 >> 2) & 1) << 1);
        w_off[k] = (wid < B_PIECES && co < p.w_rows) ? (int64_t)(co * 4 + tap) * p.cin_total + gseg * 8 : (int64_t)(zero_t - wptr);
    }
    struct TPos { int b, ty, tx; };
    TPos step_;
    {
        const int g = (int)gridDim.x;
        step_.tx = g % tiles_x;
        const int q = g / tiles_x;
        step_.ty = q % tiles_y;
        step_.b = q / tiles_y;
    }
    auto pos_of = [&](int tile) {
        TPos t;
        t.tx = tile % tiles_x;
        const int q = tile / tiles_x;
        t.ty = q % tiles_y;
        t.b = q / tiles_y;
        return t;
    };
    auto pos_next = [&](TPos& t) {
        t.tx += step_.tx;
        if (t.tx >= tiles_x) { t.tx -= tiles_x; ++t.ty; }
        t.ty += step_.ty;
        if (t.ty >= tiles_y) { t.ty -= tiles_y; ++t.b; }
        t.b += step_.b;
    };
    int pr_[KP], pc_[KP], a_off[KP];
#pragma unroll
    for (int k = 0; k < KP; ++k) {
        const int pix = 16 * (wave + NWAVES * k) + l4;
        const int pr = pix / CD_PW, pc = pix - pr * CD_PW;
        pr_[k] = pix < NPIX ? pr : (1 << 20);
        pc_[k] = pc;
        a_off[k] = 2 * pr * (int)S.sy + 2 * pc * (int)S.sx + (segpos ^ (((pc >> 2) & 1) << 1)) * 8;
    }
    unsigned a_ok = 0;
    const T* a_base = sptr;
    auto tile_offsets = [&](const TPos& t, int e, int f) {
        const int y0 = 2 * t.ty * TH - 1 + e, x0 = 2 * t.tx * 32 - 1 + f;
        a_base = sptr + ((int64_t)t.b * S.sb + (int64_t)y0 * (int)S.sy + (int64_t)x0 * (int)S.sx);
        a_ok = 0;
#pragma unroll
        for (int k = 0; k < KP; ++k) {
            const int vy = y0 + 2 * pr_[k], vx = x0 + 2 * pc_[k];
            a_ok |= (vy >= 0 && vy < GH && vx >= 0 && vx < GW) ? 1u << k : 0u;
        }
    };
    struct Cur { int tile, c, cin, ef, kofs; TPos t; };
    auto advance = [&](Cur& q) {
        q.kofs += KCV;
        ++q.c;
        if (++q.cin == cpc) {
            q.cin = 0;
            if (++q.ef == 4) {
                q.ef = 0; q.c = 0; q.kofs = 0;
                q.tile += gridDim.x;
                pos_next(q.t);
                if (q.tile >= ntiles) return;
            }
            tile_offsets(q.t, q.ef >> 1, q.ef & 1);
        }
    };
    auto issue_piece = [&](const Cur& q, int buf, int i) {
        const unsigned dst0 = lds_base + buf * BUF;
        if (i < KP) {
            const int id = wave + NWAVES * i;
            const T* src = ((a_ok >> i) & 1) ? a_base + q.cin * KCV + a_off[i] : zero_t;
            if (id < A_PIECES) cd_glds16(src, dst0 + id * 1024);
        } else {
            const int wid = wave + NWAVES * (i - KP);
            if (wid < B_PIECES) cd_glds16(wptr + q.kofs + w_off[i - KP], dst0 + A_BYTES + wid * 1024);
        }
    };

    int a_lane[2][2];
#pragma unroll
    for (int dv = 0; dv < 2; ++dv)
#pragma unroll
        for (int pt = 0; pt < 2; ++pt) {
            const int col = dv + 16 * pt + lp;
            a_lane[dv][pt] = ((wave * MT) * CD_PW + col) * 64 + ((lg ^ (((col >> 2) & 1) << 1)) << 4);
        }
    const int wrow = m16_row_channel(lp);
    const int b_lane = A_BYTES + wrow * 64 + ((lg ^ (((wrow >> 2) & 1) << 1)) << 4);

    Acc16 acc[MT][NT];
#pragma unroll
    for (int mt = 0; mt < MT; ++mt)
#pragma unroll
        for (int nt = 0; nt < NT; ++nt) acc[mt][nt].zero();
    Cur qi = {(int)blockIdx.x, 0, 0, 0, 0, pos_of((int)blockIdx.x)};
    TPos ct = qi.t;
    if (total > 0) {
        tile_offsets(qi.t, 0, 0);
#pragma unroll
        for (int i = 0; i < KP + KW; ++i) issue_piece(qi, 0, i);
        advance(qi);
    }
    int cc = 0;
    for (int it = 0; it < total; ++it) {
        asm volatile("s_waitcnt vmcnt(0) lgkmcnt(0)" ::: "memory");
        __builtin_amdgcn_s_barrier();
        const bool more = it + 1 < total;
        int bo = (it & 1) * BUF;
        asm volatile("" : "+s"(bo));
        const char* const Bf = lds;
// ... 1047 lines not shown
```

### fal_net_amd/csrc/conv_epilogue.h

```cpp
#pragma once
#include <type_traits>
#include "common.h"

typedef f32x16_t f32x16;

__device__ __forceinline__ float max_raw(float a, float b) {
    float r;
    asm("v_max_f32 %0, %1, %2" : "=v"(r) : "v"(a), "v"(b));
    return r;
}
__device__ __forceinline__ float elu_f(float v) {
    const float e = __builtin_amdgcn_fmed3f(__builtin_amdgcn_exp2f(v * 1.44269504088896340736f), 0.f, 1.f);
    return max_raw(v, e - 1.f);
}
__device__ __forceinline__ float relu_f(float v) { return max_raw(v, 0.f); }
__device__ __forceinline__ float elu_grad_from_out(float y) { return __builtin_amdgcn_fmed3f(y + 1.f, 0.f, 1.f); }
__device__ __forceinline__ float apply_act(float v, int act) {
    if (act == FALNET_ACT_ELU) return elu_f(v);
    if (act == FALNET_ACT_RELU) return relu_f(v);
    return v;
}
__device__ __forceinline__ float act_grad_from_out(float y, int kind) {
    if (kind == FALNET_ACT_ELU) return elu_grad_from_out(y);
    if (kind == FALNET_ACT_RELU) return y > 0.f ? 1.f : 0.f;
// ... 83 lines not shown
            v[4 * k + 2] = __uint_as_float(r.c[k].z);
            v[4 * k + 3] = __uint_as_float(r.c[k].w);
        }
    }
}
template <typename T>
__device__ __forceinline__ void tile_store(T* __restrict__ base, int64_t o, int cbase, int h, int Cout, const float (&v)[16]) {
    if constexpr (sizeof(T) == 2) {
        unsigned w[4][2];
#pragma unroll
        for (int k = 0; k < 4; ++k) {
            w[k][0] = pack16x2<T>(v[4 * k + 0], v[4 * k + 1]);
            w[k][1] = pack16x2<T>(v[4 * k + 2], v[4 * k + 3]);
        }
#pragma unroll
        for (int q = 0; q < 2; ++q) {
            half_swap(w[2 * q][0], w[2 * q + 1][0]);
            half_swap(w[2 * q][1], w[2 * q + 1][1]);
            const int cb = cbase + 16 * q + 8 * h;
            if (o >= 0 && cb < Cout) *reinterpret_cast<uint4*>(base + o + cb) = make_uint4(w[2 * q][0], w[2 * q][1], w[2 * q + 1][0], w[2 * q + 1][1]);
        }
    } else {
#pragma unroll
        for (int k = 0; k < 4; ++k) {
            const int cb = cbase + 8 * k + 4 * h;
            if (o >= 0 && cb < Cout) *reinterpret_cast<float4*>(base + o + cb) = make_float4(v[4 * k], v[4 * k + 1], v[4 * k + 2], v[4 * k + 3]);
        }
    }
}
template <typename T>
struct PackedTile {
    static constexpr int N = sizeof(T) == 2 ? 8 : 16;
    unsigned w[N];
};
template <typename T>
__device__ __forceinline__ void tile_pack(const float (&v)[16], PackedTile<T>& t) {
    if constexpr (sizeof(T) == 2) {
#pragma unroll
        for (int k = 0; k < 4; ++k) {
            t.w[2 * k + 0] = pack16x2<T>(v[4 * k + 0], v[4 * k + 1]);
            t.w[2 * k + 1] = pack16x2<T>(v[4 * k + 2], v[4 * k + 3]);
        }
    } else {
#pragma unroll
        for (int j = 0; j < 16; ++j) t.w[j] = __float_as_uint(v[j]);
    }
}
template <typename T>
__device__ __forceinline__ void tile_store_packed(T* __restrict__ base, int64_t o, int cbase, int h, int Cout, PackedTile<T>& t) {
    if constexpr (sizeof(T) == 2) {
#pragma unroll
        for (int q = 0; q < 2; ++q) {
            half_swap(t.w[4 * q + 0], t.w[4 * q + 2]);
            half_swap(t.w[4 * q + 1], t.w[4 * q + 3]);
            const int cb = cbase + 16 * q + 8 * h;
            if (o >= 0 && cb < Cout) *reinterpret_cast<uint4*>(base + o + cb) = make_uint4(t.w[4 * q + 0], t.w[4 * q + 1], t.w[4 * q + 2], t.w[4 * q + 3]);
        }
    } else {
#pragma unroll
        for (int k = 0; k < 4; ++k) {
            const int cb = cbase + 8 * k + 4 * h;
            if (o >= 0 && cb < Cout) *reinterpret_cast<uint4*>(base + o + cb) = make_uint4(t.w[4 * k], t.w[4 * k + 1], t.w[4 * k + 2], t.w[4 * k + 3]);
        }
    }
}
template <typename T, int MT, int NT>
struct PackedOut {
    PackedTile<T> out[MT][NT];
    PackedTile<T> pool[(MT + 1) / 2][NT];
};

__device__ __forceinline__ int m16_row_channel(int i) { return ((i >> 2) & 1) * 8 + (i >> 3) * 4 + (i & 3); }
struct Acc16 {
    f32x4_t t[2][2];
    __device__ __forceinline__ void zero() {
#pragma unroll
        for (int ct = 0; ct < 2; ++ct)
#pragma unroll
            for (int pt = 0; pt < 2; ++pt) t[ct][pt] = f32x4_t{0.f, 0.f, 0.f, 0.f};
    }
    __device__ __forceinline__ void to32(f32x16_t& v) const {
#pragma unroll
        for (int ct = 0; ct < 2; ++ct)
#pragma unroll
            for (int f = 0; f < 4; ++f) {
                const auto r = __builtin_amdgcn_permlane16_swap(__float_as_uint(t[ct][0][f]), __float_as_uint(t[ct][1][f]), false, false);
                v[4 * (2 * ct) + f] = __uint_as_float(r[0]);
                v[4 * (2 * ct + 1) + f] = __uint_as_float(r[1]);
            }
    }
};

__device__ __forceinline__ void act16(float (&v)[16], int act) {
    if (act == FALNET_ACT_ELU) {
#pragma unroll
        for (int j0 = 0; j0 < 16; j0 += 8) {
            typedef float f32x2 __attribute__((ext_vector_type(2)));
            f32x2 e[4];
#pragma unroll
            for (int j = 0; j < 4; ++j) e[j] = f32x2{v[j0 + 2 * j], v[j0 + 2 * j + 1]} * 1.44269504088896340736f;
#pragma unroll
            for (int j = 0; j < 4; ++j) {
                e[j].x = __builtin_amdgcn_fmed3f(__builtin_amdgcn_exp2f(e[j].x), 0.f, 1.f);
                e[j].y = __builtin_amdgcn_fmed3f(__builtin_amdgcn_exp2f(e[j].y), 0.f, 1.f);
            }
#pragma unroll
            for (int j = 0; j < 4; ++j) e[j] = e[j] - 1.f;
#pragma unroll
            for (int j = 0; j < 4; ++j) {
                v[j0 + 2 * j] = max_raw(v[j0 + 2 * j], e[j].x);
                v[j0 + 2 * j + 1] = max_raw(v[j0 + 2 * j + 1], e[j].y);
            }
        }
    } else if (act == FALNET_ACT_RELU) {
#pragma unroll
        for (int j = 0; j < 16; ++j) v[j] = relu_f(v[j]);
    }
}
__device__ __forceinline__ void actgrad16(float (&v)[16], const float (&y)[16], int kind) {
    if (kind == FALNET_ACT_ELU) {
#pragma unroll
        for (int j = 0; j < 16; ++j) v[j] *= elu_grad_from_out(y[j]);
    } else if (kind == FALNET_ACT_RELU) {
#pragma unroll
        for (int j = 0; j < 16; ++j) v[j] = y[j] > 0.f ? v[j] : 0.f;
    }
}
template <int NT>
__device__ __forceinline__ void load_bias16(const falnet_conv_t& p, int nbase, int h, float (&bias)[NT][16]) {
#pragma unroll
    for (int nt = 0; nt < NT; ++nt)
#pragma unroll
        for (int j = 0; j < 16; ++j) {
            const int c = nbase + nt * 32 + 8 * (j >> 2) + 4 * h + (j & 3);
            bias[nt][j] = (p.bias && c < p.Cout) ? p.bias[c] : 0.f;
        }
}
__device__ __forceinline__ void stage_bias_lds(const falnet_conv_t& p, int n0, int bn, float* lds_bias) {
    for (int i = threadIdx.x; i < bn; i += blockDim.x) lds_bias[i] = (p.bias && n0 + i < p.Cout) ? p.bias[n0 + i] : 0.f;
}
__device__ __forceinline__ void load_bias16_lds(const float* lds_bias, int cb, int h, float (&bias)[1][16]) {
#pragma unroll
    for (int m = 0; m < 4; ++m) {
        const float4 v = *reinterpret_cast<const float4*>(lds_bias + cb + 8 * m + 4 * h);
        bias[0][4 * m + 0] = v.x;
        bias[0][4 * m + 1] = v.y;
        bias[0][4 * m + 2] = v.z;
        bias[0][4 * m + 3] = v.w;
    }
}
__device__ __forceinline__ float lane_xor1(float v) {
    return __int_as_float(__builtin_amdgcn_mov_dpp(__float_as_int(v), 0xB1, 0xF, 0xF, true));
}
template <typename T, int MT, int NT, typename PixOff, typename PoolOff = NoPool, int AHEAD = 1, bool DEFER = false, bool NHWC_ONLY = false, bool PLANAR_PTR = false>
__device__ __forceinline__ void epilogue_direct(const falnet_conv_t& p, f32x16 (&acc)[MT][NT], const float (&bias)[NT][16], int nbase, int lane,
                                                PixOff pixoff, PoolOff pooloff = PoolOff(), PackedOut<T, MT, NT>* defer = nullptr) {
    constexpr bool POOL = !std::is_same<PoolOff, NoPool>::value;
    const int h = lane >> 5;
    const T* addend = reinterpret_cast<const T*>(p.addend);
    const T* actout = reinterpret_cast<const T*>(p.actout);
    T* out = reinterpret_cast<T*>(p.out);
    T* pool_out = reinterpret_cast<T*>(p.pool_out);
    const bool pooling = POOL && pool_out != nullptr;
    const bool psum = p.pool_mode == 1;
#pragma unroll
    for (int nt = 0; nt < NT; ++nt) {
        const int cbase = nbase + nt * 32;
        float hp[16];
        constexpr int NR = AHEAD < 0 ? 1 : 1 + AHEAD;
        TileRaw<T> ra[NR], rb[NR];
        if (AHEAD > 0) {
            if (addend) tile_fetch<T>(addend, pixoff(0), cbase, h, p.Cout, ra[0]);
            if (actout) tile_fetch<T>(actout, pixoff(0), cbase, h, p.Cout, rb[0]);
        }
#pragma unroll
        for (int mt = 0; mt < MT; ++mt) {
            const int64_t o = pixoff(mt);
            if (AHEAD >= 0 && (AHEAD ? mt + 1 < MT : true)) {
                const int mf = mt + AHEAD;
                if (addend) tile_fetch<T>(addend, pixoff(mf), cbase, h, p.Cout, ra[mf & AHEAD]);
                if (actout) tile_fetch<T>(actout, pixoff(mf), cbase, h, p.Cout, rb[mf & AHEAD]);
            }
            float v[16];
#pragma unroll
            for (int j = 0; j < 16; ++j) v[j] = acc[mt][nt][j] + bias[nt][j];
            if (addend) {
                float a[16];
                if constexpr (AHEAD < 0) tile_load<T>(addend, o, cbase, h, p.Cout, a);
                else tile_unpack<T>(ra[mt & (AHEAD < 0 ? 0 : AHEAD)], a);
#pragma unroll
                for (int j = 0; j < 16; ++j) v[j] += a[j];
            }
            act16(v, p.act);
            if (actout) {
                float a[16];
                if constexpr (AHEAD < 0) tile_load<T>(actout, o, cbase, h, p.Cout, a);
                else tile_unpack<T>(rb[mt & (AHEAD < 0 ? 0 : AHEAD)], a);
                actgrad16(v, a, p.actout_kind);
            }
            if constexpr (DEFER) {
                tile_pack<T>(v, defer->out[mt][nt]);
            } else if (!NHWC_ONLY && p.out_layout == FALNET_OUT_PLANAR_F32) {
                float* po = reinterpret_cast<float*>(p.out);
                const int64_t cs = (int64_t)p.OH * p.OW;
                if constexpr (PLANAR_PTR) {
                    if (o >= 0) {
                        float* q = po + o + (int64_t)(cbase + 4 * h) * cs;
#pragma unroll
                        for (int j = 0; j < 16; ++j) {
                            const int c = cbase + 8 * (j >> 2) + 4 * h + (j & 3);
                            asm volatile("" : "+v"(q));
                            if (c < p.Cout) *q = v[j];
                            q += ((j & 3) == 3) ? 5 * cs : cs;
                        }
                    }
                } else if (o >= 0) {
#pragma unroll
                    for (int j = 0; j < 16; ++j) {
                        const int c = cbase + 8 * (j >> 2) + 4 * h + (j & 3);
                        if (c < p.Cout) po[o + c * cs] = v[j];
                    }
                }
            } else if (!POOL || out) tile_store<T>(out, o, cbase, h, p.Cout, v);
            if constexpr (POOL) {
                if (pooling) {
                    float m[16];
                    if (psum) {
#pragma unroll
                        for (int j = 0; j < 16; ++j) m[j] = v[j] + lane_xor1(v[j]);
                    } else {
#pragma unroll
                        for (int j = 0; j < 16; ++j) m[j] = fmaxf(v[j], lane_xor1(v[j]));
                    }
                    if ((mt & 1) == 0) {
#pragma unroll
                        for (int j = 0; j < 16; ++j) hp[j] = m[j];
                    } else {
                        if (psum) {
#pragma unroll
                            for (int j = 0; j < 16; ++j) m[j] += hp[j];
                        } else {
#pragma unroll
                            for (int j = 0; j < 16; ++j) m[j] = fmaxf(m[j], hp[j]);
                        }
                        const int64_t po = (lane & 1) ? (int64_t)-1 : pooloff(mt);
                        if (p.pool_actout) {
                            float a[16];
                            tile_load<T>(reinterpret_cast<const T*>(p.pool_actout), po, cbase, h, p.Cout, a);
                            actgrad16(m, a, p.pool_actout_kind);
                        }
                        if constexpr (DEFER) tile_pack<T>(m, defer->pool[mt >> 1][nt]);
                        else tile_store<T>(pool_out, po, cbase, h, p.Cout, m);
                    }
                }
            }
        }
    }
}

template <typename T, int MT, int NT, typename PixOff, typename PoolOff>
__device__ __forceinline__ void epilogue_store_packed(const falnet_conv_t& p, PackedOut<T, MT, NT>& d, int nbase, int lane, PixOff pixoff, PoolOff pooloff) {
    const int h = lane >> 5;
    T* out = reinterpret_cast<T*>(p.out);
    T* pool_out = reinterpret_cast<T*>(p.pool_out);
#pragma unroll
    for (int nt = 0; nt < NT; ++nt) {
        const int cbase = nbase + nt * 32;
#pragma unroll
        for (int mt = 0; mt < MT; ++mt) {
            if (out) tile_store_packed<T>(out, pixoff(mt), cbase, h, p.Cout, d.out[mt][nt]);
            if ((mt & 1) && pool_out) {
                const int64_t po = (lane & 1) ? (int64_t)-1 : pooloff(mt);
                tile_store_packed<T>(pool_out, po, cbase, h, p.Cout, d.pool[mt >> 1][nt]);
            }
        }
    }
}
```

### fal_net_amd/csrc/elementwise.hip

```cpp
#include <stdlib.h>
#include "common.h"

#define EW_THREADS 256
static inline int ew_grid(int64_t n) {
    int64_t g = (n + EW_THREADS - 1) / EW_THREADS;
    return (int)(g < 1 ? 1 : (g > 8192 ? 8192 : g));
}

__device__ __forceinline__ void store8_as(float* p, const float (&v)[8]) {
    reinterpret_cast<float4*>(p)[0] = make_float4(v[0], v[1], v[2], v[3]);
    reinterpret_cast<float4*>(p)[1] = make_float4(v[4], v[5], v[6], v[7]);
}
template <typename T>
__device__ __forceinline__ void store8_as(T* p, const float (&v)[8]) {
    uint4 q;
#pragma unroll
    for (int i = 0; i < 4; ++i) (&q.x)[i] = pack16x2<T>(v[2 * i], v[2 * i + 1]);
    *reinterpret_cast<uint4*>(p) = q;
}
__device__ __forceinline__ void load8_as(const float* p, float (&v)[8]) {
    const float4 a = reinterpret_cast<const float4*>(p)[0], b = reinterpret_cast<const float4*>(p)[1];
    v[0] = a.x; v[1] = a.y; v[2] = a.z; v[3] = a.w; v[4] = b.x; v[5] = b.y; v[6] = b.z; v[7] = b.w;
}
template <typename T>
// ... 17 lines not shown
    const int ld = Cpad + 1;
    for (int i = threadIdx.x; i < 64 * Cpad; i += blockDim.x) {
        const int c = i >> 6, px = i & 63;
        const int64_t p = p0 + px;
        tile[px * ld + c] = (c < C && p < HW) ? src[((int64_t)b * C + c) * HW + p] : 0.f;
    }
    __syncthreads();
    if (Cpad % 8 == 0) {
        const int cg = Cpad / 8;
        for (int i = threadIdx.x; i < 64 * cg; i += blockDim.x) {
            const int px = i / cg, c0 = (i % cg) * 8;
            const int64_t p = p0 + px;
            if (p < HW) {
                float v[8];
#pragma unroll
                for (int j = 0; j < 8; ++j) v[j] = tile[px * ld + c0 + j];
                store8_as(dst + ((int64_t)b * HW + p) * Cpad + c0, v);
            }
        }
        return;
    }
    for (int i = threadIdx.x; i < 64 * Cpad; i += blockDim.x) {
        const int px = i / Cpad, c = i % Cpad;
        const int64_t p = p0 + px;
        if (p < HW) dst[((int64_t)b * HW + p) * Cpad + c] = from_f32<T>(tile[px * ld + c]);
    }
}

template <typename T>
__global__ __launch_bounds__(EW_THREADS) void nhwc_to_nchw_kernel(const T* __restrict__ src, float* __restrict__ dst,
                                                                  int C, int64_t HW, int Cpad) {
    extern __shared__ __attribute__((aligned(16))) char smem[];
    float* tile = reinterpret_cast<float*>(smem);
    const int b = blockIdx.y;
    const int64_t p0 = (int64_t)blockIdx.x * 64;
    const int ld = Cpad + 1;
    for (int i = threadIdx.x; i < 64 * Cpad; i += blockDim.x) {
        const int px = i / Cpad, c = i % Cpad;
        const int64_t p = p0 + px;
        tile[px * ld + c] = p < HW ? to_f32(src[((int64_t)b * HW + p) * Cpad + c]) : 0.f;
    }
    __syncthreads();
    for (int i = threadIdx.x; i < 64 * C; i += blockDim.x) {
        const int c = i >> 6, px = i & 63;
        const int64_t p = p0 + px;
        if (p < HW) dst[((int64_t)b * C + c) * HW + p] = tile[px * ld + c];
    }
}

__device__ __forceinline__ float elu_grad_from_out(float y) { return y > 0.f ? 1.f : y + 1.f; }

template <typename T>
__global__ __launch_bounds__(EW_THREADS) void upsample_bwd_kernel(const T* __restrict__ gup, T* __restrict__ gsrc,
                                                                  const T* __restrict__ actout, int B, int IH, int IW,
                                                                  int H, int W, int C) {
    const int cg = C / 8;
    const int64_t total = (int64_t)B * H * W * cg;
    for (int64_t i = (int64_t)blockIdx.x * blockDim.x + threadIdx.x; i < total; i += (int64_t)gridDim.x * blockDim.x) {
        const int c0 = (int)(i % cg) * 8;
        const int sx = (int)((i / cg) % W), sy = (int)((i / ((int64_t)cg * W)) % H), b = (int)(i / ((int64_t)cg * W * H));
        const int vy0 = (sy * IH + H - 1) / H, vy1 = ((sy + 1) * IH + H - 1) / H;
        const int vx0 = (sx * IW + W - 1) / W, vx1 = ((sx + 1) * IW + W - 1) / W;
        float acc[8] = {0, 0, 0, 0, 0, 0, 0, 0};
        for (int vy = vy0; vy < vy1; ++vy)
            for (int vx = vx0; vx < vx1; ++vx) {
                const T* g = gup + (((int64_t)b * IH + vy) * IW + vx) * C + c0;
#pragma unroll
                for (int j = 0; j < 8; ++j) acc[j] += to_f32(g[j]);
            }
        const int64_t o = (((int64_t)b * H + sy) * W + sx) * C + c0;
#pragma unroll
        for (int j = 0; j < 8; ++j) {
            float v = acc[j];
            if (actout) v *= elu_grad_from_out(to_f32(actout[o + j]));
            gsrc[o + j] = from_f32<T>(v);
        }
    }
}

template <typename T>
__global__ __launch_bounds__(EW_THREADS) void maxpool2_fwd_kernel(const T* __restrict__ x, T* __restrict__ y, int B, int H,
                                                                  int W, int C) {
    const int OH = H / 2, OW = W / 2;
    const int64_t total = (int64_t)B * OH * OW * C;
    for (int64_t i = (int64_t)blockIdx.x * blockDim.x + threadIdx.x; i < total; i += (int64_t)gridDim.x * blockDim.x) {
        const int c = (int)(i % C), ox = (int)((i / C) % OW), oy = (int)((i / ((int64_t)C * OW)) % OH);
        const int b = (int)(i / ((int64_t)C * OW * OH));
        const T* p = x + (((int64_t)b * H + 2 * oy) * W + 2 * ox) * C + c;
        const float v = fmaxf(fmaxf(to_f32(p[0]), to_f32(p[C])), fmaxf(to_f32(p[(int64_t)W * C]), to_f32(p[(int64_t)W * C + C])));
        y[i] = from_f32<T>(v);
    }
}

template <typename T>
__global__ __launch_bounds__(EW_THREADS) void maxpool2_bwd_kernel(const T* __restrict__ x, const T* __restrict__ gy,
                                                                  T* __restrict__ gx, int B, int H, int W, int C) {
    const int OH = H / 2, OW = W / 2;
    const int64_t total = (int64_t)B * OH * OW * C;
    for (int64_t i = (int64_t)blockIdx.x * blockDim.x + threadIdx.x; i < total; i += (int64_t)gridDim.x * blockDim.x) {
        const int c = (int)(i % C), ox = (int)((i / C) % OW), oy = (int)((i / ((int64_t)C * OW)) % OH);
        const int b = (int)(i / ((int64_t)C * OW * OH));
        const int64_t base = (((int64_t)b * H + 2 * oy) * W + 2 * ox) * C + c;
        const int64_t off[4] = {0, C, (int64_t)W * C, (int64_t)W * C + C};
        float best = to_f32(x[base]);
        int arg = 0;
#pragma unroll
        for (int j = 1; j < 4; ++j) {
            const float v = to_f32(x[base + off[j]]);
            if (v > best) {
                best = v;
                arg = j;
            }
        }
        const float g = best > 0.f ? to_f32(gy[i]) : 0.f;
#pragma unroll
        for (int j = 0; j < 4; ++j) gx[base + off[j]] = from_f32<T>(j == arg ? g : 0.f);
    }
}

template <typename T>
__global__ __launch_bounds__(EW_THREADS) void maxpool2_bwd_vec_kernel(const T* __restrict__ x, const T* __restrict__ gy,
                                                                      T* __restrict__ gx, int B, int H, int W, int C) {
    const int OH = H / 2, OW = W / 2, cg = C / 8;
    const int64_t total = (int64_t)B * OH * OW * cg;
    for (int64_t i = (int64_t)blockIdx.x * blockDim.x + threadIdx.x; i < total; i += (int64_t)gridDim.x * blockDim.x) {
        const int c0 = (int)(i % cg) * 8, ox = (int)((i / cg) % OW), oy = (int)((i / ((int64_t)cg * OW)) % OH);
        const int b = (int)(i / ((int64_t)cg * OW * OH));
        const int64_t base = (((int64_t)b * H + 2 * oy) * W + 2 * ox) * C + c0;
        const int64_t off[4] = {0, C, (int64_t)W * C, (int64_t)W * C + C};
        float xv[4][8], g[8], o[4][8];
#pragma unroll
        for (int j = 0; j < 4; ++j) load8_as(x + base + off[j], xv[j]);
        load8_as(gy + (((int64_t)b * OH + oy) * OW + ox) * C + c0, g);
#pragma unroll
        for (int e = 0; e < 8; ++e) {
            float best = xv[0][e];
            int arg = 0;
#pragma unroll
            for (int j = 1; j < 4; ++j)
                if (xv[j][e] > best) {
                    best = xv[j][e];
                    arg = j;
                }
            const float ge = best > 0.f ? g[e] : 0.f;
#pragma unroll
            for (int j = 0; j < 4; ++j) o[j][e] = j == arg ? ge : 0.f;
        }
#pragma unroll
        for (int j = 0; j < 4; ++j) store8_as(gx + base + off[j], o[j]);
    }
}

template <typename T>
__global__ __launch_bounds__(EW_THREADS) void act_bwd_kernel(const T* __restrict__ g, const T* __restrict__ y,
                                                             T* __restrict__ gx, int64_t n, int kind) {
    for (int64_t i = (int64_t)blockIdx.x * blockDim.x + threadIdx.x; i < n; i += (int64_t)gridDim.x * blockDim.x) {
        const float yy = to_f32(y[i]);
        const float d = kind == FALNET_ACT_RELU ? (yy > 0.f ? 1.f : 0.f) : elu_grad_from_out(yy);
        gx[i] = from_f32<T>(to_f32(g[i]) * d);
    }
}


extern "C" int falnet_nchw_to_nhwc(const float* src, void* dst, int B, int C, int H, int W, int Cpad, int dtype,
                                   void* stream) {
    FALNET_ENTER(stream);
    FALNET_CHECK_ARG(src && dst && B > 0 && C > 0 && H > 0 && W > 0 && Cpad >= C && Cpad <= 512, "nchw_to_nhwc: bad argument");
    const int64_t HW = (int64_t)H * W;
    const dim3 grid((unsigned)((HW + 63) / 64), B);
    const size_t lds = (size_t)64 * (Cpad + 1) * sizeof(float);
#define EW_L(T) hipLaunchKernelGGL(nchw_to_nhwc_kernel<T>, grid, dim3(EW_THREADS), lds, (hipStream_t)stream, src, (T*)dst, C, HW, Cpad)
    FALNET_DISPATCH_DTYPE(dtype, EW_L);
#undef EW_L
    FALNET_RETURN_LAUNCH();
}

extern "C" int falnet_nhwc_to_nchw(const void* src, float* dst, int B, int C, int H, int W, int Cpad, int dtype,
                                   void* stream) {
    FALNET_ENTER(stream);
    FALNET_CHECK_ARG(src && dst && B > 0 && C > 0 && H > 0 && W > 0 && Cpad >= C && Cpad <= 512, "nhwc_to_nchw: bad argument");
    const int64_t HW = (int64_t)H * W;
    const dim3 grid((unsigned)((HW + 63) / 64), B);
    const size_t lds = (size_t)64 * (Cpad + 1) * sizeof(float);
#define EW_L(T) hipLaunchKernelGGL(nhwc_to_nchw_kernel<T>, grid, dim3(EW_THREADS), lds, (hipStream_t)stream, (const T*)src, dst, C, HW, Cpad)
    FALNET_DISPATCH_DTYPE(dtype, EW_L);
#undef EW_L
    FALNET_RETURN_LAUNCH();
}

extern "C" int falnet_upsample_bwd(const void* gup, void* gsrc, const void* actout, int B, int IH, int IW, int H, int W,
                                   int C, int dtype, void* stream) {
    FALNET_ENTER(stream);
    FALNET_CHECK_ARG(gup && gsrc && B > 0 && IH >= H && IW >= W && H > 0 && W > 0 && C % 8 == 0, "upsample_bwd: bad argument");
    FALNET_CHECK_ARG((int64_t)H * IH + H <= INT32_MAX && (int64_t)W * IW + W <= INT32_MAX, "upsample_bwd: %dx%d -> %dx%d too large for 32-bit index ranges", H, W, IH, IW);
    const int64_t total = (int64_t)B * H * W * (C / 8);
#define EW_L(T) hipLaunchKernelGGL(upsample_bwd_kernel<T>, dim3(ew_grid(total)), dim3(EW_THREADS), 0, (hipStream_t)stream, (const T*)gup, (T*)gsrc, (const T*)actout, B, IH, IW, H, W, C)
    FALNET_DISPATCH_DTYPE(dtype, EW_L);
#undef EW_L
    FALNET_RETURN_LAUNCH();
}

template <typename T>
__global__ __launch_bounds__(256) void const_plane_stats_kernel(const T* __restrict__ g, float* __restrict__ ws, int TH, int TW, int gC, int rows_per_block) {
    __shared__ float red[256 * 8];
    const int b = blockIdx.y, segs = gC >> 3, npl = 256 / segs;
    const int seg = threadIdx.x % segs, pl = threadIdx.x / segs;
    const int r0 = blockIdx.x * rows_per_block, r1 = min(r0 + rows_per_block, TH);
    float st[9][8];
#pragma unroll
    for (int k = 0; k < 9; ++k)
#pragma unroll
        for (int i = 0; i < 8; ++i) st[k][i] = 0.f;
    const bool has_top = r0 == 0, has_bot = r1 == TH;
    if (pl < npl) {
        for (int y = r0; y < r1; ++y) {
            const bool top = y == 0, bot = y == TH - 1;
            const T* row = g + (((int64_t)b * TH + y) * TW) * gC + seg * 8;
            float rs[8];
#pragma unroll
            for (int i = 0; i < 8; ++i) rs[i] = 0.f;
            for (int x = pl; x < TW; x += npl) {
                float v[8];
                load8_as(row + (int64_t)x * gC, v);
#pragma unroll
                for (int i = 0; i < 8; ++i) rs[i] += v[i];
                if (x == 0) {
#pragma unroll
                    for (int i = 0; i < 8; ++i) {
                        st[3][i] += v[i];
                        if (top) st[5][i] += v[i];
                        if (bot) st[7][i] += v[i];
                    }
                }
                if (x == TW - 1) {
#pragma unroll
                    for (int i = 0; i < 8; ++i) {
                        st[4][i] += v[i];
                        if (top) st[6][i] += v[i];
                        if (bot) st[8][i] += v[i];
                    }
                }
            }
#pragma unroll
            for (int i = 0; i < 8; ++i) {
                st[0][i] += rs[i];
                if (top) st[1][i] += rs[i];
                if (bot) st[2][i] += rs[i];
            }
        }
    }
#pragma unroll
    for (int k = 0; k < 9; ++k) {
        if ((k == 1 || k == 5 || k == 6) && !has_top) continue;
        if ((k == 2 || k == 7 || k == 8) && !has_bot) continue;
#pragma unroll
        for (int i = 0; i < 8; ++i) red[threadIdx.x * 8 + i] = st[k][i];
        __syncthreads();
        if ((int)threadIdx.x < gC) {
            const int c = threadIdx.x, sg = c >> 3, i = c & 7;
            float t = 0.f;
            for (int q = 0; q < npl; ++q) t += red[(q * segs + sg) * 8 + i];
            if (t != 0.f) atomicAdd(ws + ((int64_t)b * 9 + k) * gC + c, t);
        }
        __syncthreads();
    }
}

template <typename T>
__global__ __launch_bounds__(1024) void const_plane_combine_kernel(float* __restrict__ ws, const T* __restrict__ plane, int64_t plane_stride, float* __restrict__ grad,
                                                                   int64_t co_stride, int B, int gC, int cout, int ex_bot, int ex_rt) {
    for (int e = threadIdx.x; e < cout * 9; e += blockDim.x) {
        const int co = e / 9, tap = e - co * 9, ky = tap / 3, kx = tap - ky * 3;
        const float et = ky == 0 ? 1.f : 0.f, eb = ((ex_bot >> ky) & 1) ? 1.f : 0.f, el = kx == 0 ? 1.f : 0.f, er = ((ex_rt >> kx) & 1) ? 1.f : 0.f;
        float acc = 0.f;
        for (int b = 0; b < B; ++b) {
            const float* w = ws + (int64_t)b * 9 * gC + co;
            const float s = w[0] - et * w[gC] - eb * w[2 * gC] - el * w[3 * gC] - er * w[4 * gC] + et * el * w[5 * gC] + et * er * w[6 * gC] +
                            eb * el * w[7 * gC] + eb * er * w[8 * gC];
            acc += to_f32(plane[b * plane_stride]) * s;
        }
        atomicAdd(grad + co * co_stride + tap, acc);
    }
    __syncthreads();
    for (int e = threadIdx.x; e < B * 9 * gC; e += blockDim.x) ws[e] = 0.f;
}

extern "C" int falnet_wgrad_const_plane(const void* gout, const void* plane, int64_t plane_stride, float* grad, int64_t grad_co_stride, float* ws, int B,
                                        int TH, int TW, int gC, int cout, int IH, int IW, int stride, int dtype, void* stream) {
    FALNET_ENTER(stream);
    FALNET_CHECK_ARG(gout && plane && grad && ws && B > 0 && TH >= 2 && TW >= 2 && gC % 8 == 0 && gC <= 256 && cout > 0 && cout <= gC,
                     "wgrad_const_plane: bad argument (B=%d TH=%d TW=%d gC=%d cout=%d)", B, TH, TW, gC, cout);
    FALNET_CHECK_ARG((stride == 1 || stride == 2) && TH == (IH + stride - 1) / stride && TW == (IW + stride - 1) / stride,
                     "wgrad_const_plane: a 3x3 pad-1 conv of stride %d maps %dx%d to %dx%d, not %dx%d", stride, IH, IW, (IH + stride - 1) / stride,
                     (IW + stride - 1) / stride, TH, TW);
    FALNET_CHECK_ARG(!falnet_deterministic(), "wgrad_const_plane adds with f32 atomics: not available in deterministic mode");
    int ex_bot = 0, ex_rt = 0;
    for (int k = 0; k < 3; ++k) {
        if ((TH - 1) * stride + k - 1 >= IH) ex_bot |= 1 << k;
        if ((TW - 1) * stride + k - 1 >= IW) ex_rt |= 1 << k;
    }
    const int rows_per_block = TH >= 64 ? 4 : 1;
    const dim3 grid((unsigned)((TH + rows_per_block - 1) / rows_per_block), (unsigned)B);
#define EW_L(T)                                                                                                                                         \
    hipLaunchKernelGGL(const_plane_stats_kernel<T>, grid, dim3(256), 0, (hipStream_t)stream, (const T*)gout, ws, TH, TW, gC, rows_per_block);           \
    hipLaunchKernelGGL(const_plane_combine_kernel<T>, dim3(1), dim3(1024), 0, (hipStream_t)stream, ws, (const T*)plane, plane_stride, grad, grad_co_stride, \
                       B, gC, cout, ex_bot, ex_rt)
    FALNET_DISPATCH_DTYPE(dtype, EW_L);
#undef EW_L
    FALNET_RETURN_LAUNCH();
}

extern "C" int falnet_maxpool2_fwd(const void* x, void* y, int B, int H, int W, int C, int dtype, void* stream) {
    FALNET_ENTER(stream);
    FALNET_CHECK_ARG(x && y && B > 0 && H >= 2 && W >= 2 && C > 0, "maxpool2_fwd: bad argument");
    const int64_t total = (int64_t)B * (H / 2) * (W / 2) * C;
#define EW_L(T) hipLaunchKernelGGL(maxpool2_fwd_kernel<T>, dim3(ew_grid(total)), dim3(EW_THREADS), 0, (hipStream_t)stream, (const T*)x, (T*)y, B, H, W, C)
    FALNET_DISPATCH_DTYPE(dtype, EW_L);
#undef EW_L
    FALNET_RETURN_LAUNCH();
}

extern "C" int falnet_maxpool2_bwd(const void* x, const void* y, const void* gy, void* gx, int B, int H, int W, int C,
                                   int dtype, void* stream) {
    FALNET_ENTER(stream);
    (void)y;
    FALNET_CHECK_ARG(x && gy && gx && B > 0 && H >= 2 && W >= 2 && H % 2 == 0 && W % 2 == 0 && C > 0,
                     "maxpool2_bwd: bad argument (even H, W required)");
    if (C % 8 == 0 && (((uintptr_t)x | (uintptr_t)gy | (uintptr_t)gx) & 15) == 0) {
        const int64_t tv = (int64_t)B * (H / 2) * (W / 2) * (C / 8);
#define EW_L(T) hipLaunchKernelGGL(maxpool2_bwd_vec_kernel<T>, dim3(ew_grid(tv)), dim3(EW_THREADS), 0, (hipStream_t)stream, (const T*)x, (const T*)gy, (T*)gx, B, H, W, C)
        FALNET_DISPATCH_DTYPE(dtype, EW_L);
#undef EW_L
        FALNET_RETURN_LAUNCH();
    }
    const int64_t total = (int64_t)B * (H / 2) * (W / 2) * C;
#define EW_L(T) hipLaunchKernelGGL(maxpool2_bwd_kernel<T>, dim3(ew_grid(total)), dim3(EW_THREADS), 0, (hipStream_t)stream, (const T*)x, (const T*)gy, (T*)gx, B, H, W, C)
    FALNET_DISPATCH_DTYPE(dtype, EW_L);
#undef EW_L
    FALNET_RETURN_LAUNCH();
}

extern "C" int falnet_act_bwd(const void* g, const void* y, void* gx, int64_t n, int kind, int dtype, void* stream) {
    FALNET_ENTER(stream);
    FALNET_CHECK_ARG(g && y && gx && n > 0, "act_bwd: bad argument");
#define EW_L(T) hipLaunchKernelGGL(act_bwd_kernel<T>, dim3(ew_grid(n)), dim3(EW_THREADS), 0, (hipStream_t)stream, (const T*)g, (const T*)y, (T*)gx, n, kind)
    FALNET_DISPATCH_DTYPE(dtype, EW_L);
#undef EW_L
    FALNET_RETURN_LAUNCH();
}

__global__ __launch_bounds__(EW_THREADS) void gemm_f32_small_kernel(const float* __restrict__ A, int64_t sam, int64_t sak,
                                                                    const float* __restrict__ Bm, int64_t sbk, int64_t sbn,
                                                                    float* __restrict__ C, int M, int N, int K, int accumulate) {
    for (int64_t i = (int64_t)blockIdx.x * blockDim.x + threadIdx.x; i < (int64_t)M * N; i += (int64_t)gridDim.x * blockDim.x) {
        const int m = (int)(i / N), n = (int)(i % N);
        const float* a = A + m * sam;
        const float* b = Bm + n * sbn;
        float acc = 0.f;
        int k = 0;
        for (; k + 8 <= K; k += 8) {
            float av[8], bv[8];
#pragma unroll
            for (int u = 0; u < 8; ++u) {
                av[u] = a[(k + u) * sak];
                bv[u] = b[(k + u) * sbk];
            }
#pragma unroll
            for (int u = 0; u < 8; ++u) acc = fmaf(av[u], bv[u], acc);
        }
        for (; k < K; ++k) acc = fmaf(a[k * sak], b[k * sbk], acc);
        C[i] = accumulate ? C[i] + acc : acc;
    }
}

__global__ __launch_bounds__(EW_THREADS) void gemm_f32_small_wave_kernel(const float* __restrict__ A, int64_t sam, int64_t sak,
                                                                         const float* __restrict__ Bm, int64_t sbk, int64_t sbn,
                                                                         float* __restrict__ C, int M, int N, int K, int accumulate) {
    const int lane = threadIdx.x & 63;
    const int64_t nwaves = (int64_t)gridDim.x * (blockDim.x >> 6);
    for (int64_t i = (int64_t)blockIdx.x * (blockDim.x >> 6) + (threadIdx.x >> 6); i < (int64_t)M * N; i += nwaves) {
        const int m = (int)(i / N), n = (int)(i % N);
        const float* a = A + m * sam;
        const float* b = Bm + n * sbn;
        float acc = 0.f;
        for (int k = lane; k < K; k += 64) acc = fmaf(a[k * sak], b[k * sbk], acc);
        acc = wave_sum(acc);
        if (lane == 0) C[i] = accumulate ? C[i] + acc : acc;
    }
}

extern "C" int falnet_gemm_f32_small(const float* A, int64_t sam, int64_t sak, const float* B, int64_t sbk, int64_t sbn, float* C,
                                     int M, int N, int K, int accumulate, void* stream) {
    FALNET_ENTER(stream);
    FALNET_CHECK_ARG(A && B && C && M > 0 && N > 0 && K > 0 && (int64_t)M * N * K <= (1ll << 32), "gemm_f32_small: bad argument (small products only)");
    static const bool wave_form = [] { const char* e = falnet_ab_env("FALNET_GEMM_WAVE"); return !(e && e[0] == '0'); }();
    if (wave_form && K >= 256 && (int64_t)M * N <= 65536) {
        const int64_t waves = (int64_t)M * N;
        hipLaunchKernelGGL(gemm_f32_small_wave_kernel, dim3((unsigned)((waves + 3) / 4 > 4096 ? 4096 : (waves + 3) / 4)), dim3(EW_THREADS), 0,
                           (hipStream_t)stream, A, sam, sak, B, sbk, sbn, C, M, N, K, accumulate);
        FALNET_RETURN_LAUNCH();
    }
    hipLaunchKernelGGL(gemm_f32_small_kernel, dim3(ew_grid((int64_t)M * N)), dim3(EW_THREADS), 0, (hipStream_t)stream, A, sam, sak, B, sbk, sbn, C,
                       M, N, K, accumulate);
    FALNET_RETURN_LAUNCH();
}

__global__ __launch_bounds__(EW_THREADS) void resize_planar_kernel(const float* __restrict__ src, float* __restrict__ dst, int H, int W,
                                                                   int OH, int OW, int bilinear, float scale, int64_t total) {
    const float ry = OH > 1 ? (float)(H - 1) / (float)(OH - 1) : 0.f, rx = OW > 1 ? (float)(W - 1) / (float)(OW - 1) : 0.f;
    const float ny = (float)H / (float)OH, nx = (float)W / (float)OW;
    for (int64_t i = (int64_t)blockIdx.x * blockDim.x + threadIdx.x; i < total; i += (int64_t)gridDim.x * blockDim.x) {
        const int ox = (int)(i % OW), oy = (int)((i / OW) % OH);
        const float* pl = src + (i / ((int64_t)OW * OH)) * ((int64_t)H * W);
        float v;
        if (bilinear) {
            const float fy = ry * oy, fx = rx * ox;
            const int y0 = (int)fy, x0 = (int)fx;
            const int y1 = min(y0 + 1, H - 1), x1 = min(x0 + 1, W - 1);
            const float wy = fy - y0, wx = fx - x0;
            v = (1.f - wy) * ((1.f - wx) * pl[(int64_t)y0 * W + x0] + wx * pl[(int64_t)y0 * W + x1]) +
                wy * ((1.f - wx) * pl[(int64_t)y1 * W + x0] + wx * pl[(int64_t)y1 * W + x1]);
        } else {
            const int sy = min((int)floorf(oy * ny), H - 1), sx = min((int)floorf(ox * nx), W - 1);
            v = pl[(int64_t)sy * W + sx];
        }
        dst[i] = v * scale;
    }
}

extern "C" int falnet_resize_planar(const float* src, float* dst, int64_t planes, int H, int W, int OH, int OW, int bilinear, float scale,
                                    void* stream) {
    FALNET_ENTER(stream);
    FALNET_CHECK_ARG(src && dst && planes > 0 && H > 0 && W > 0 && OH > 0 && OW > 0, "resize_planar: bad argument");
    const int64_t total = planes * OH * OW;
    hipLaunchKernelGGL(resize_planar_kernel, dim3(ew_grid(total)), dim3(EW_THREADS), 0, (hipStream_t)stream, src, dst, H, W, OH, OW, bilinear, scale, total);
    FALNET_RETURN_LAUNCH();
}

template <typename T>
__global__ void disp_prologue_kernel(const float* __restrict__ max_disp, const float* __restrict__ min_disp, float mul, float div,
                                     float* __restrict__ min_out, float* __restrict__ max_out, T* __restrict__ flow, int flow_stride, int B) {
    const int b = blockIdx.x * blockDim.x + threadIdx.x;
    if (b >= B) return;
    const float mx = max_disp[b];
    min_out[b] = min_disp ? min_disp[b] : mx * mul / div;
    max_out[b] = mx;
    flow[(int64_t)b * flow_stride] = from_f32<T>(mx / 100.0f);
}

extern "C" int falnet_disp_prologue(const float* max_disp, const float* min_disp, float mul, float div, float* min_out, float* max_out,
                                    void* flow, int flow_stride, int B, int dtype, void* stream) {
    FALNET_ENTER(stream);
    FALNET_CHECK_ARG(max_disp && min_out && max_out && flow && B > 0 && flow_stride > 0 && (min_disp || div != 0.0f), "disp_prologue: bad argument");
#define EW_L(T) hipLaunchKernelGGL(disp_prologue_kernel<T>, dim3((B + 63) / 64), dim3(64), 0, (hipStream_t)stream, max_disp, min_disp, mul, div, min_out, max_out, (T*)flow, flow_stride, B)
    FALNET_DISPATCH_DTYPE(dtype, EW_L);
#undef EW_L
    FALNET_RETURN_LAUNCH();
}

__global__ void spin_kernel(long long ticks) {
    const long long t0 = (long long)__builtin_amdgcn_s_memrealtime();
    while ((long long)__builtin_amdgcn_s_memrealtime() - t0 < ticks) __builtin_amdgcn_s_sleep(8);
}
extern "C" int falnet_spin(int microseconds, void* stream) {
    FALNET_ENTER(stream);
    FALNET_CHECK_ARG(microseconds >= 0 && microseconds <= 100000, "spin: 0..100000 us");
    hipLaunchKernelGGL(spin_kernel, dim3(1), dim3(64), 0, (hipStream_t)stream, (long long)microseconds * 100);
    FALNET_RETURN_LAUNCH();
}

template <typename T>
__global__ __launch_bounds__(256, 2) void mfma_probe_kernel(const T* __restrict__ ab, float* __restrict__ out, int iters) {
    const int lane = threadIdx.x & 63, wave = (blockIdx.x * 4 + (threadIdx.x >> 6)) & 63;
    s16x8_t a[4], b[4];
#pragma unroll
    for (int k = 0; k < 4; ++k) {
        a[k] = *reinterpret_cast<const s16x8_t*>(ab + ((size_t)(wave * 8 + k) * 64 + lane) * 8);
        b[k] = *reinterpret_cast<const s16x8_t*>(ab + ((size_t)(wave * 8 + 4 + k) * 64 + lane) * 8);
    }
    f32x4_t acc[4][4];
#pragma unroll
    for (int i = 0; i < 4; ++i)
#pragma unroll
        for (int j = 0; j < 4; ++j) acc[i][j] = f32x4_t{0.f, 0.f, 0.f, 0.f};
    for (int it = 0; it < iters; ++it) {
#pragma unroll
        for (int i = 0; i < 4; ++i)
#pragma unroll
            for (int j = 0; j < 4; ++j) acc[i][j] = H16<T>::mma16(a[i], b[j], acc[i][j]);
// ... 17 lines not shown
```

### fal_net_amd/csrc/replay.cpp

```cpp
#include <string.h>
#include <tuple>
#include <type_traits>
#include <utility>

#include "common.h"

namespace {

template <typename T>
inline T take(const falnet_cmd_t& c, int& ii, int& fi) {
    if constexpr (std::is_floating_point<T>::value) return (T)c.farg[fi++];
    else if constexpr (std::is_pointer<T>::value) return (T)(uintptr_t)c.iarg[ii++];
    else return (T)(int64_t)c.iarg[ii++];
}

template <typename F>
struct FnTraits;
template <typename... Args>
struct FnTraits<int (*)(Args...)> {
    using tuple = std::tuple<Args...>;
    static constexpr size_t N = sizeof...(Args);
};

template <auto FN>
struct OpThunk {
    using Tup = typename FnTraits<decltype(FN)>::tuple;
    static constexpr size_t N = FnTraits<decltype(FN)>::N;
    static_assert(N >= 1 && std::is_same<std::tuple_element_t<N - 1, Tup>, void*>::value, "launch functions end in `void* stream`");
    template <size_t... I>
    static int call_impl(const falnet_cmd_t& c, void* stream, std::index_sequence<I...>) {
        int ii = 0, fi = 0;
        std::tuple<std::tuple_element_t<I, Tup>...> args{take<std::tuple_element_t<I, Tup>>(c, ii, fi)...};
        (void)ii, (void)fi;
        return FN(std::get<I>(args)..., stream);
    }
    static int call(const falnet_cmd_t& c, void* stream) { return call_impl(c, stream, std::make_index_sequence<N - 1>{}); }
    template <size_t... I>
    static constexpr int count_flt(std::index_sequence<I...>) {
        return (0 + ... + (std::is_floating_point<std::tuple_element_t<I, Tup>>::value ? 1 : 0));
    }
    static constexpr int nflt() { return count_flt(std::make_index_sequence<N - 1>{}); }
    static constexpr int nint() { return (int)(N - 1) - nflt(); }
    static_assert(nint() <= FALNET_CMD_MAX_INT && nflt() <= FALNET_CMD_MAX_FLT, "entry point does not fit a falnet_cmd_t: widen iarg / farg");
};
static_assert(sizeof(((falnet_cmd_t*)0)->iarg) / sizeof(uint64_t) == FALNET_CMD_MAX_INT && sizeof(((falnet_cmd_t*)0)->farg) / sizeof(double) == FALNET_CMD_MAX_FLT,
              "falnet_cmd_t slot counts");

struct Op {
    const char* name;
    int (*call)(const falnet_cmd_t&, void*);
    int nint, nflt;
};
#define FALNET_OP(fn) {#fn, &OpThunk<&fn>::call, OpThunk<&fn>::nint(), OpThunk<&fn>::nflt()}
const Op g_ops[] = {
    FALNET_OP(falnet_conv2d), FALNET_OP(falnet_conv3x3_c3), FALNET_OP(falnet_conv2d_multi), FALNET_OP(falnet_wgrad), FALNET_OP(falnet_wgrad_reduce),
    FALNET_OP(falnet_bias_grad), FALNET_OP(falnet_pack_weights_batched), FALNET_OP(falnet_adam_pack_batched), FALNET_OP(falnet_adam_ranges),
    FALNET_OP(falnet_adam_tick), FALNET_OP(falnet_pack_up2_batched), FALNET_OP(falnet_wgrad_reduce_batched), FALNET_OP(falnet_bias_grad_batched),
    FALNET_OP(falnet_bias_grad_batched_det), FALNET_OP(falnet_pack_weights), FALNET_OP(falnet_nchw_to_nhwc), FALNET_OP(falnet_nhwc_to_nchw),
    FALNET_OP(falnet_upsample_bwd), FALNET_OP(falnet_wgrad_const_plane), FALNET_OP(falnet_maxpool2_fwd), FALNET_OP(falnet_maxpool2_bwd),
    FALNET_OP(falnet_act_bwd), FALNET_OP(falnet_med_head_fwd), FALNET_OP(falnet_med_head_bwd), FALNET_OP(falnet_med_head_bwd_nhwc),
    FALNET_OP(falnet_med_masks_fwd), FALNET_OP(falnet_med_maskr_acfalse_fwd), FALNET_OP(falnet_l1_fwd), FALNET_OP(falnet_l1_bwd),
    FALNET_OP(falnet_mse_fwd), FALNET_OP(falnet_mse_bwd), FALNET_OP(falnet_smooth_fwd), FALNET_OP(falnet_smooth_bwd), FALNET_OP(falnet_l1_fwd_bwd),
    FALNET_OP(falnet_l1_fwd_bwd_add), FALNET_OP(falnet_mse_fwd_bwd), FALNET_OP(falnet_smooth_fwd_bwd), FALNET_OP(falnet_step_scalars),
    FALNET_OP(falnet_mask_mix), FALNET_OP(falnet_adam_step), FALNET_OP(falnet_adam_step_dev), FALNET_OP(falnet_grad_guard),
    FALNET_OP(falnet_adam_step_guarded), FALNET_OP(falnet_loss_scale_update), FALNET_OP(falnet_loss_seeds), FALNET_OP(falnet_occlusion_mask),
    FALNET_OP(falnet_mirror_weight), FALNET_OP(falnet_hflip), FALNET_OP(falnet_rowmax), FALNET_OP(falnet_gemm_f32_small),
    FALNET_OP(falnet_resize_planar), FALNET_OP(falnet_disp_prologue), FALNET_OP(falnet_resample_u8), FALNET_OP(falnet_augment_normalize),
    FALNET_OP(falnet_fill_f32), FALNET_OP(falnet_copy_bytes), FALNET_OP(falnet_spin), FALNET_OP(falnet_adam_pack_batched_wd),
    FALNET_OP(falnet_adam_ranges_wd), FALNET_OP(falnet_adam_step_wd), FALNET_OP(falnet_augment_batch),
};
constexpr int g_nops = (int)(sizeof(g_ops) / sizeof(g_ops[0]));

}

extern "C" int falnet_replay_op_index(const char* name) {
    if (!name) return -1;
    for (int i = 0; i < g_nops; ++i)
        if (strcmp(g_ops[i].name, name) == 0) return i;
    return -1;
}

extern "C" int falnet_replay_op_args(int op, int* nint, int* nflt) {
    FALNET_CHECK_ARG(op >= 0 && op < g_nops && nint && nflt, "replay_op_args: unknown op %d", op);
    *nint = g_ops[op].nint;
    *nflt = g_ops[op].nflt;
    return 0;
}

extern "C" int falnet_replay(const falnet_cmd_t* cmds, int n, void* const* streams, int nstreams, void* const* events, int nevents, int* failed_at) {
    FALNET_CHECK_ARG(cmds && n >= 0 && streams && nstreams > 0, "replay: bad argument");
    hipDevice_t dev0 = -1;
    for (int s = 0; s < nstreams; ++s) {
        if (!streams[s]) continue;
        hipDevice_t d;
        if (hipStreamGetDevice((hipStream_t)streams[s], &d) != hipSuccess) {
            (void)hipGetLastError();
            falnet_set_error("replay: stream %d is not a valid stream handle", s);
            return -1;
        }
        if (dev0 >= 0 && d != dev0) {
            falnet_set_error("replay: streams of devices %d and %d in one sequence", (int)dev0, (int)d);
            return -1;
        }
        dev0 = d;
    }
    const bool pin = streams[0] != nullptr;
    if (pin) falnet_enter_stream(streams[0]);
    struct Depth {
        int* d;
        bool on;
        explicit Depth(bool o) : d(falnet_replay_depth()), on(o) { if (on) ++*d; }
        ~Depth() { if (on) --*d; }
    } depth_guard(pin);
    for (int i = 0; i < n; ++i) {
        const falnet_cmd_t& c = cmds[i];
        int rc = 0;
        if (c.stream < 0 || c.stream >= nstreams) {
            falnet_set_error("replay: command %d names stream %d of %d", i, c.stream, nstreams);
            rc = -1;
        } else if (c.op == FALNET_CMD_RECORD || c.op == FALNET_CMD_WAIT) {
            if (!events || c.event < 0 || c.event >= nevents || !events[c.event]) {
                falnet_set_error("replay: command %d names event %d of %d", i, c.event, nevents);
                rc = -1;
            } else {
                const hipError_t e = c.op == FALNET_CMD_RECORD ? hipEventRecord((hipEvent_t)events[c.event], (hipStream_t)streams[c.stream])
                                                               : hipStreamWaitEvent((hipStream_t)streams[c.stream], (hipEvent_t)events[c.event], 0);
                if (e != hipSuccess) {
                    falnet_set_error("replay: command %d (%s): %s", i, c.op == FALNET_CMD_RECORD ? "event record" : "stream wait", hipGetErrorString(e));
                    rc = (int)e;
                }
            }
        } else if (c.op >= 0 && c.op < g_nops) {
            if (c.nint < 0 || c.nint > FALNET_CMD_MAX_INT || c.nflt < 0 || c.nflt > FALNET_CMD_MAX_FLT || c.nint != g_ops[c.op].nint || c.nflt != g_ops[c.op].nflt) {
                falnet_set_error("replay: command %d (%s) carries %d + %d arguments, the entry point takes %d + %d", i, g_ops[c.op].name, c.nint, c.nflt,
                                 g_ops[c.op].nint, g_ops[c.op].nflt);
                rc = -1;
            } else {
                rc = g_ops[c.op].call(c, streams[c.stream]);
            }
        } else {
            falnet_set_error("replay: command %d has unknown op %d", i, c.op);
            rc = -1;
        }
        if (rc != 0) {
            if (failed_at) *failed_at = i;
            return rc;
        }
    }
    if (failed_at) *failed_at = -1;
    return 0;
}

extern "C" int falnet_fill_f32(float* p, int64_t n, float value, void* stream) {
    FALNET_ENTER(stream);
    FALNET_CHECK_ARG(p && n >= 0, "fill_f32: bad argument");
    if (n == 0) return 0;
    const hipError_t e = value == 0.f ? hipMemsetAsync(p, 0, (size_t)n * 4, (hipStream_t)stream)
                                      : hipMemsetD32Async((hipDeviceptr_t)p, __builtin_bit_cast(int, value), (size_t)n, (hipStream_t)stream);
    if (e != hipSuccess) {
        falnet_set_error("fill_f32: %s", hipGetErrorString(e));
        return (int)e;
    }
    return 0;
}

extern "C" int falnet_copy_bytes(void* dst, const void* src, int64_t nbytes, void* stream) {
    FALNET_ENTER(stream);
    FALNET_CHECK_ARG(dst && src && nbytes >= 0, "copy_bytes: bad argument");
    if (nbytes == 0) return 0;
    const hipError_t e = hipMemcpyAsync(dst, src, (size_t)nbytes, hipMemcpyDeviceToDevice, (hipStream_t)stream);
    if (e != hipSuccess) {
        falnet_set_error("copy_bytes: %s", hipGetErrorString(e));
        return (int)e;
    }
    return 0;
}
```

### fal_net_amd/loss_functions.py

```python
import os
import weakref

import torch
import torch.nn as nn
import torch.nn.functional as F

from . import _lib as L
from . import ops, synthetic
from .ops import PackedConv

_MEAN = (0.411, 0.432, 0.45)
_SLICES = ((0, 2), (5, 7), (10, 12, 14, 16))


_GOUT_OF = {}
_MAX_HELD_PLANS = 4


def _forget_gouts(keys):
    for k in keys:
        _GOUT_OF.pop(k, None)


def _release_plan(plan, gen):
    if plan.gen == gen:
        plan.busy = False


class _VggPlan:

    def __init__(self, owner, B, H, W, dtype, device, need_grad=True):
        self.B, self.H, self.W, self.dtype, self.device = B, H, W, dtype, device
        self.busy, self.need_grad, self.gen = False, need_grad, 0
        code = L.dtype_code(dtype)
        self.fwd, self.bwd = [], []
        _conv = lambda *a, **kw: ops.conv_call(*a, ws_owner=("vgg", id(self)), **kw)
        pcs = owner._packed
        x_in = torch.empty(B, 3, H, W, dtype=torch.float32, device=device)
        x0 = x_in
        self.x_in, self.keep = x_in, []
        cur, h, w = x0, H, W
        self.outs, acts = [], []
        for convs in _SLICES:
            for idx in convs:
                pc = pcs[idx]
                last = idx == convs[-1]
                pooled = torch.empty(B, h // 2, w // 2, pc.cout, dtype=dtype, device=device) if last else None
                y = torch.empty(B, h, w, pc.cout, dtype=dtype, device=device) if (need_grad or not last) else None
                kw = dict(bias=pc.bias, act=L.ACT_RELU, name=f"vgg conv{idx}", flops=2 * B * h * w * pc.cout * pc.cin * 9)
                args = (dtype, [ops.nhwc_src(cur)], h, w, pc.wf, pc.cin_pad, ops.fwd_taps(3), 9, pc.cout_pad, 1, B, h, w)
                fused = False
                if cur is x0:
                    self.c3_call = ops.conv_c3_call(dtype, x_in, pc, y, L.ACT_RELU, name="vgg conv0(c3)")
                    self.fwd.append(self.c3_call)
                elif last and L.ab("FALNET_FUSED_POOL", "1") == "1":
                    try:
                        self.fwd.append(_conv(*args, y, h, w, pc.cout, pc.cout, pool_out=pooled, **kw))
                        fused = True
                    except ValueError:
                        pass
                if not fused and cur is not x0:
                    if y is None:
                        y = torch.empty(B, h, w, pc.cout, dtype=dtype, device=device)
                    self.fwd.append(_conv(*args, y, h, w, pc.cout, pc.cout, **kw))
                if last and not fused:
                    self.fwd.append(ops.simple_call("falnet_maxpool2_fwd", L.ptr(y), L.ptr(pooled), B, h, w, pc.cout, code))
                acts.append((pc, cur, y, h, w))
                cur = y
            acts.append(("pool", cur, pooled, h, w))
            self.outs.append(pooled)
            cur, h, w = pooled, h // 2, w // 2
        self.run_fwd = ops.ReplayList(self.fwd, eager_head=1)
        self.run_bwd = None
        if not need_grad:
            return
        self.gouts = [torch.empty_like(o) for o in self.outs]
        for o, g in zip(self.outs, self.gouts):
            _GOUT_OF[o.data_ptr()] = [g, False]
        weakref.finalize(self, _forget_gouts, [o.data_ptr() for o in self.outs])
        g_next = None
        slice_i = len(self.outs) - 1
        for entry in reversed(acts):
            if entry[0] == "pool":
                _, x, pooled, h, w = entry
                gy = self.gouts[slice_i] if g_next is None else g_next
                gx = torch.empty_like(x)
                self.bwd.append(ops.simple_call("falnet_maxpool2_bwd", L.ptr(x), L.ptr(pooled), L.ptr(gy), L.ptr(gx), B, h, w,
                                                x.shape[3], code))
                g_next, slice_i = gx, slice_i - 1
                self.keep.append(gx)
            else:
                pc, x, y, h, w = entry
                if x is x0:
                    self.g_in = torch.empty(B, 3, H, W, dtype=torch.float32, device=device)
                    self.bwd.append(_conv(dtype, [ops.nhwc_src(g_next)], h, w, pc.wd, pc.cout_pad, ops.dgrad_taps_s1(3), 9,
                                          ops.pad_c(3), 1, B, h, w, self.g_in, h, w, 3, 0, out_layout=L.OUT_PLANAR_F32, name="vgg dgrad0",
                                          flops=2 * B * h * w * pc.cout * pc.cin * 9))
                else:
                    from_pool = any(x is o for o in self.outs)
                    gin = torch.empty_like(x)
                    own = next((g for o, g in zip(self.outs, self.gouts) if x is o), None)
                    self.bwd.append(_conv(dtype, [ops.nhwc_src(g_next)], h, w, pc.wd, pc.cout_pad, ops.dgrad_taps_s1(3), 9,
                                                  pc.cin_pad, 1, B, h, w, gin, h, w, pc.cin_pad, pc.cin_pad, addend=own,
                                                  actout=None if from_pool else x,
                                                  actout_kind=L.ACT_NONE if from_pool else L.ACT_RELU, name="vgg dgrad",
                                                  flops=2 * B * h * w * pc.cout * pc.cin * 9))
                    self.keep.append(gin)
                    g_next = gin
        self.run_bwd = ops.ReplayList(self.bwd)


class _VggFunction(torch.autograd.Function):
    @staticmethod
    def forward(ctx, owner, plan, x):
        plan.c3_call.set_input(x)
        plan.run_fwd()
        ctx.plan, ctx.owner, ctx.gen = plan, owner, plan.gen
        weakref.finalize(ctx, _release_plan, plan, plan.gen)
        return tuple(o.permute(0, 3, 1, 2) for o in plan.outs)

    @staticmethod
    def backward(ctx, *gouts):
        plan = ctx.plan
        if plan.gen != ctx.gen:
            raise RuntimeError(f"this VGG call's plan was recycled: more than {_MAX_HELD_PLANS} grad-enabled vgg() calls of one shape "
                               "were alive without a backward")
        for buf, g in zip(plan.gouts, gouts):
            if g is None:
                buf.zero_()
            elif g.data_ptr() != buf.data_ptr():
                buf.copy_(g.permute(0, 2, 3, 1))
        plan.run_bwd()
        out = plan.g_in.clone()
        plan.busy = False
        return None, None, out


class Vgg19_pc(nn.Module):

    def __init__(self, requires_grad=False, compute_dtype=None, state_dict=None):
        super().__init__()
        self.features = nn.ModuleDict({str(i): nn.Conv2d(cin, cout, 3, padding=1) for i, (cin, cout) in synthetic.VGG19_PC_CONVS.items()})
        sd = state_dict
        path = os.environ.get("FALNET_VGG19_WEIGHTS")
        if sd is None and path:
            sd = torch.load(path, map_location="cpu")
        self.weights_source = "file" if sd is not None else "seeded"
        if sd is None:
            sd = synthetic.seeded_vgg19_state_dict()
        with torch.no_grad():
            for i, conv in self.features.items():
                conv.weight.copy_(sd[f"features.{i}.weight"])
                conv.bias.copy_(sd[f"features.{i}.bias"])
        for p in self.parameters():
            p.requires_grad = requires_grad
        self.compute_dtype = compute_dtype
        self._plans, self._packed, self._packed_key = {}, None, None

    def _prepare(self, device, dtype):
        key = (device, dtype)
        if self._packed_key != key:
            if next(self.parameters()).device != device:
                self.to(device)
            self._packed = {}
            for i, conv in self.features.items():
                pc = PackedConv(f"vgg{i}", conv.weight, conv.bias, [conv.weight.shape[1]], 1)
                pc.alloc(dtype, device)
                pc.pack_call()()
                self._packed[int(i)] = pc
            self._packed_key, self._plans = key, {}

    def _plan(self, B, H, W, dtype, device, hold):
        pool = self._plans.setdefault((B, H, W, hold), [])
        p = next((q for q in pool if not q.busy), None)
        if p is None and hold and len(pool) >= _MAX_HELD_PLANS:
            p = min(pool, key=lambda q: q.gen)
        if p is None:
            p = _VggPlan(self, B, H, W, dtype, device, need_grad=hold)
            pool.append(p)
        self._gen = getattr(self, "_gen", 0) + 1
        p.busy, p.gen = hold, self._gen
        if hold:
            for o in p.outs:
                _GOUT_OF[o.data_ptr()][1] = False
        return p

    def forward(self, x, full=False, borrow=False):
        if full:
            raise NotImplementedError("slice4 (relu4_4) is never used on the FAL_net hot path (loss_functions.py:40-42)")
        if not x.is_cuda:
            raise RuntimeError("fal_net_amd Vgg19_pc runs on an MI355X only (no CPU fallback)")
        dtype = self.compute_dtype or _default_dtype()
        self._prepare(x.device, dtype)
        B, C, H, W = x.shape
        assert C == 3 and H % 8 == 0 and W % 8 == 0, "VGG19 slices need a 3-channel input with H, W divisible by 8"
        need_grad = torch.is_grad_enabled() and x.requires_grad
        plan = self._plan(B, H, W, dtype, x.device, hold=need_grad)
        xs = x.float().contiguous() if need_grad else x.detach().float().contiguous()
        if need_grad:
            return _VggFunction.apply(self, plan, xs)
        with torch.no_grad():
            plan.c3_call.set_input(xs)
            plan.run_fwd()
            return tuple((o if borrow else o.clone()).permute(0, 3, 1, 2) for o in plan.outs)


_DEFAULT_DTYPE = [torch.float32]


def set_compute_dtype(dtype):
    _DEFAULT_DTYPE[0] = dtype


def _default_dtype():
    return _DEFAULT_DTYPE[0]


class _LazyVgg:

    def __init__(self):
        self._m = None

    def _get(self):
        if self._m is None:
            self._m = Vgg19_pc()
        return self._m

    def __call__(self, x, full=False, **kw):
        return self._get()(x, full, **kw)

    def __getattr__(self, name):
        return getattr(self._get(), name)


vgg = _LazyVgg()


class _L1Mean(torch.autograd.Function):

    @staticmethod
    def forward(ctx, synth, label, mask, scale=None):
# ... 174 lines not shown
```

### fal_net_amd/ops.py

```python
import ctypes as C
import os
import sys

import torch

from . import _lib as L

CPAD = L.CPAD
H16 = (torch.bfloat16, torch.float16)
TYPE_SYM = {torch.bfloat16: "DF16b", torch.float16: "DF16_", torch.float32: "f"}

TIMER = None
AUTOTUNE = os.environ.get("FALNET_AUTOTUNE", "1") != "0"
DETERMINISTIC = L.DETERMINISTIC
UP2W = L.ab("FALNET_UP2W", "0") == "1"
UP2D = L.ab("FALNET_UP2D", "1") == "1"


_PKG_CACHE = os.path.join(os.path.dirname(os.path.abspath(__file__)), "autotune_cache.json")
_CACHE_PATH = os.environ.get("FALNET_AUTOTUNE_CACHE", _PKG_CACHE)
_CACHE_WRITABLE = ("FALNET_AUTOTUNE_CACHE" in os.environ and _CACHE_PATH != "0") or os.environ.get("FALNET_AUTOTUNE_CACHE_WRITE") == "1"
_GATES = {"FALNET_NO_DMA": "0", "FALNET_WS2": "1", "FALNET_S2F_DMA": "1", "FALNET_S2D_DMA": "1", "FALNET_S2_SPLITK": "1",
          "FALNET_GATHER_NARROW": "0", "FALNET_S2_MULTI": None, "FALNET_SMALL_TILE_DMA": "1", "FALNET_UP2": "1", "FALNET_DEEP": "1", "FALNET_TILE8": "1"}
if os.environ.get("FALNET_AB") == "1" and any(os.environ.get(k, v) != v for k, v in _GATES.items()):
# ... 150 lines not shown
        lib = L.lib()
        c0_real = self.groups_real[0]
        c0_pad = self.groups_pad[0] if len(self.groups_real) == 2 else self.cin_pad
        if len(self.groups_real) == 1:
            c0_real = self.cin
        args = (L.ptr(self.weight), self.cout, self.cin, self.taps, c0_real, c0_pad, self.cin_pad, self.cout_pad,
                L.ptr(self.wf), L.ptr(self.wd if need_dgrad else None), L.dtype_code(self._dtype))

        def call():
            L.check(lib.falnet_pack_weights(*args, L.stream_ptr()), "pack_weights " + self.name)
        return call

    def group_channels(self):
        c0_real = self.groups_real[0] if len(self.groups_real) == 2 else self.cin
        c0_pad = self.groups_pad[0] if len(self.groups_real) == 2 else self.cin_pad
        return c0_real, c0_pad


def conv_c3_call(dtype, x_planar, pc, out, act, name="conv0(c3)"):
    lib = L.lib()
    B, C, H, W = x_planar.shape
    assert C == 3 and pc.cin == 3 and pc.cout in (32, 64) and out.shape == (B, H, W, pc.cout)
    tail = (L.ptr(pc.weight), L.ptr(pc.bias), L.ptr(out), B, H, W, pc.cout, act, L.dtype_code(dtype))
    tn, nt = TYPE_SYM[dtype], pc.cout // 32
    cur = [x_planar]

    def launch(_keep=(pc, out)):
        L.check(lib.falnet_conv3x3_c3(L.ptr(cur[0]), *tail, L.stream_ptr()), name)
    call = _timed(f"_Z17conv3x3_c3_kernelI{tn}Li{nt}EEvPKfS1_13falnet_conv_tii", 2 * B * H * W * pc.cout * 27, 0, launch, name)

    def set_input(t):
        assert t.shape == x_planar.shape and t.dtype == torch.float32 and t.is_contiguous() and t.device == x_planar.device
        cur[0] = t
    call.set_input = set_input
    return call


def pack_all_call(pcs, dtype, device):
    lib = L.lib()
    descs = (L.PackDesc * len(pcs))()
    blk = 0
    for i, pc in enumerate(pcs):
        c0_real, c0_pad = pc.group_channels()
        d = descs[i]
        d.w, d.wf, d.wd = pc.weight.data_ptr(), pc.wf.data_ptr(), pc.wd.data_ptr()
        d.cout, d.cin, d.taps, d.c0_real, d.c0_pad, d.cin_pad, d.cout_pad, d.block_begin = (
            pc.cout, pc.cin, pc.taps, c0_real, c0_pad, pc.cin_pad, pc.cout_pad, blk)
        blk += (pc.cout_pad // 32) * (pc.cin_pad // 32)
    dev = torch.frombuffer(bytearray(bytes(descs)), dtype=torch.uint8).to(device)
    n, total, code = len(pcs), blk, L.dtype_code(dtype)

    def launch(_keep=(dev, pcs)):
        L.check(lib.falnet_pack_weights_batched(L.ptr(dev), n, total, code, L.stream_ptr()), "pack_weights_batched")
    return _timed("pack_weights_batched", 0, 0, launch, "pack_weights_batched")


def adam_pack_call(pcs, dtype, device, derived=()):
    lib = L.lib()
    n_own = len(pcs)
    pcs = list(pcs) + list(derived)
    descs = (L.PackDesc * len(pcs))()
    blk = 0
    for i, pc in enumerate(pcs):
        descs[i].no_update = int(i >= n_own)
        c0_real, c0_pad = pc.group_channels()
        d = descs[i]
        d.w, d.wf, d.wd = pc.weight.data_ptr(), pc.wf.data_ptr(), pc.wd.data_ptr()
        d.cout, d.cin, d.taps, d.c0_real, d.c0_pad, d.cin_pad, d.cout_pad, d.block_begin = (
            pc.cout, pc.cin, pc.taps, c0_real, c0_pad, pc.cin_pad, pc.cout_pad, blk)
        blk += (pc.cout_pad // 32) * (pc.cin_pad // 32)
    dev = torch.frombuffer(bytearray(bytes(descs)), dtype=torch.uint8).to(device)
    n, total, code = len(pcs), blk, L.dtype_code(dtype)

    def launch(g_off, m_off, v_off, state, b1, b2, eps, grad_scale, scaler, weight_decay=0.0, _keep=(dev, pcs)):
        if weight_decay:
            L.check(lib.falnet_adam_pack_batched_wd(L.ptr(dev), n, total, code, g_off, m_off, v_off, L.ptr(state), b1, b2, eps, float(grad_scale),
                                                    float(weight_decay), L.ptr(scaler), L.stream_ptr()), "adam_pack_batched_wd")
            return
        L.check(lib.falnet_adam_pack_batched(L.ptr(dev), n, total, code, g_off, m_off, v_off, L.ptr(state), b1, b2, eps, float(grad_scale),
                                             L.ptr(scaler), L.stream_ptr()), "adam_pack_batched")
    return launch


class DecayTable:

    def __init__(self, is_bias, device):
        self.is_bias = [bool(b) for b in is_bias]
        self.dev = torch.zeros(len(self.is_bias), dtype=torch.float64, device=device)
        self.key = (0.0, 0.0)

    def get(self, weight_decay, bias_decay):
        key = (float(weight_decay), float(bias_decay))
        if key != self.key:
            self.dev.copy_(torch.tensor([key[1] if b else key[0] for b in self.is_bias], dtype=torch.float64))
            self.key = key
        return self.dev


def pack_up2_call(pcs, dtype, device):
    lib = L.lib()
    pcs = [pc for pc in pcs if pc.wu is not None]
    if not pcs:
        return None
    descs = (L.PackUp2Desc * len(pcs))()
    blk = 0
    for i, pc in enumerate(pcs):
        d = descs[i]
        d.w, d.wu, d.cout, d.cin, d.cin_pad, d.cout_pad, d.block_begin = pc.weight.data_ptr(), pc.wu.data_ptr(), pc.cout, pc.cin, pc.cin_pad, pc.cout_pad, blk
        d.wdd = 0 if pc.wdd is None else pc.wdd.data_ptr()
        blk += (pc.cout_pad // 32) * (pc.cin_pad // 32)
    dev = torch.frombuffer(bytearray(bytes(descs)), dtype=torch.uint8).to(device)
    n, total, code = len(pcs), blk, L.dtype_code(dtype)

    def launch(_keep=(dev, pcs)):
        L.check(lib.falnet_pack_up2_batched(L.ptr(dev), n, total, code, L.stream_ptr()), "pack_up2_batched")
    return _timed("pack_up2_batched", 0, 0, launch, "pack_up2_batched")


def fwd_taps(ksize):
    if ksize == 1:
        return [(0, 0, 0)]
    KH, KW = (3, 3) if ksize == 3 else ksize
    return [(kh - KH // 2, kw - KW // 2, kh * KW + kw) for kh in range(KH) for kw in range(KW)]


def dgrad_taps_s1(ksize):
    return [(-dy, -dx, t) for dy, dx, t in fwd_taps(ksize)]


def dgrad_taps_s2(py, px):
    taps = []
    for kh in range(3):
        if (py + 1 - kh) % 2:
            continue
        for kw in range(3):
            if (px + 1 - kw) % 2:
                continue
            taps.append(((py + 1 - kh) // 2, (px + 1 - kw) // 2, kh * 3 + kw))
    return taps


def _fill_taps(d, taps):
    d.ntaps = len(taps)
    for i, (dy, dx, w) in enumerate(taps):
        d.tap_dy[i], d.tap_dx[i] = dy, dx
        if hasattr(d, "tap_w"):
            d.tap_w[i] = w


def conv_call(dtype, srcs, IH, IW, weight, cin_total, taps, w_taps, w_rows, stride_in, B, TH, TW, out, OH, OW,
              Cout, out_cstride, out_layout=L.OUT_NHWC, out_step=(1, 1, 0, 0), bias=None, addend=None,
              act=L.ACT_NONE, actout=None, actout_kind=L.ACT_NONE, weight_offset_elems=0, name="conv", flops=0,
              autotune=True, ws_owner=None, pool_out=None, pool_mode=0, pool_actout=None, pool_actout_kind=L.ACT_NONE, weight_up2=None,
              variant=None):
    lib = L.lib()
    d = L.Conv()
    d.nsrc = len(srcs)
    for i, s in enumerate(srcs):
        d.src[i] = s
    d.IH, d.IW = IH, IW
    d.weight = weight.data_ptr() + weight_offset_elems * weight.element_size()
    d.cin_total, d.w_taps, d.w_rows = cin_total, w_taps, w_rows
    _fill_taps(d, taps)
    d.isy = d.isx = stride_in
    d.B, d.TH, d.TW = B, TH, TW
    d.osy, d.osx, d.ooy, d.oox = out_step
    d.out, d.OH, d.OW, d.Cout, d.out_cstride, d.out_layout = (0 if out is None else out.data_ptr()), OH, OW, Cout, out_cstride, out_layout
    d.pool_out = 0 if pool_out is None else pool_out.data_ptr()
    d.pool_mode, d.pool_actout_kind = pool_mode, pool_actout_kind
    d.pool_actout = 0 if pool_actout is None else pool_actout.data_ptr()
    d.weight_up2 = 0 if weight_up2 is None else weight_up2.data_ptr()
    dev_t = out if out is not None else pool_out
    d.bias = 0 if bias is None else bias.data_ptr()
    d.addend = 0 if addend is None else addend.data_ptr()
    d.act = act
    d.actout = 0 if actout is None else actout.data_ptr()
    d.actout_kind = actout_kind
    d.dtype = L.dtype_code(dtype)
    d.variant = 0
    d.ksplit = 1
    ws = _splitk_workspace(dev_t.device, ws_owner) if dev_t.is_cuda and out_layout == L.OUT_NHWC and pool_out is None else None
    d.splitk_ws = 0 if ws is None else ws.data_ptr()
    d.splitk_ws_bytes = 0 if ws is None else ws.numel() * 4
    scratch = None
    if ws is not None and dtype in H16 and TH * TW <= 128 and len(taps) == 9:
        scratch = _deep_scratch(dev_t.device, ws_owner)
        d.scratch, d.scratch_bytes = scratch.data_ptr(), scratch.numel() * 4
    ref = C.byref(d)
    keep = (d, srcs, weight, out, bias, addend, actout, ws, pool_out, pool_actout, weight_up2, scratch)
    if variant is not None:
        d.variant = variant
        if lib.falnet_conv2d_kernel_name(ref, C.create_string_buffer(160), 160) != 0:
            raise ValueError(f"falnet_conv2d variant {variant} does not apply to this launch: {lib.falnet_last_error().decode(errors='replace')}")
    elif AUTOTUNE and autotune and dev_t.is_cuda:
        key = conv_signature(d)
        hit = cache_get(key)
        if hit is not None:
            d.variant, d.ksplit = int(hit[0]), int(hit[1])
            if DETERMINISTIC and d.ksplit > 1 and d.variant != 19:
                d.variant, d.ksplit = 1, 1
            if lib.falnet_conv2d_kernel_name(ref, C.create_string_buffer(160), 160) != 0:
                hit = None
        if hit is None and DETERMINISTIC:
            d.variant, d.ksplit = 0, 1
        elif hit is None:
            d.variant, d.ksplit = _autotune_conv(lib, d, ref, B * TH * TW, w_rows, Cout)
            cache_put(key, [int(d.variant), int(d.ksplit)])
    if pool_out is not None and lib.falnet_conv2d_kernel_name(ref, C.create_string_buffer(160), 160) != 0:
        raise ValueError("no fused-pool kernel applies to this launch")

    def launch(_keep=keep):
        L.check(lib.falnet_conv2d(ref, L.stream_ptr()), name)
    buf = C.create_string_buffer(160)
    L.check(lib.falnet_conv2d_kernel_name(ref, buf, 160), name)
    tag = buf.value.decode()
    call = _timed(tag, flops, 0, launch, f"{name} v{d.variant} k{d.ksplit}")
    call.desc, call.ref = d, ref
    return call


UP2D_TAPS = [(0, 0, 0), (0, 1, 1), (1, 0, 2), (1, 1, 3)]


def deconv_dgrad_call(dtype, gout, pc, B, gin, actout, name="", flops=0, ws_owner=None):
    if pc.wdd is None:
        raise ValueError("no low-resolution data-gradient weights for this layer")
    GH, GW = gout.shape[1], gout.shape[2]
    OH, OW = GH // 2, GW // 2
    assert (2 * OH, 2 * OW) == (GH, GW) and gout.shape[3] == pc.cout_pad and gin.shape[1:3] == (OH, OW)
    return conv_call(dtype, [nhwc_src(gout)], GH, GW, pc.wdd, 4 * pc.cout_pad, UP2D_TAPS, 4, pc.cin_pad, 1, B, OH, OW, gin, OH, OW, pc.cin_pad, gin.shape[3],
                     actout=actout, actout_kind=L.ACT_ELU if actout is not None else L.ACT_NONE, name="dgrad(low-res) " + name, flops=flops,
                     ws_owner=ws_owner, variant=26)


_SPLITK_WS = {}


def _splitk_workspace(device, owner=None, nbytes=32 << 20):
    key = (device.type, device.index, owner)
    if key not in _SPLITK_WS:
        _SPLITK_WS[key] = torch.zeros(nbytes // 4, dtype=torch.float32, device=device)
    return _SPLITK_WS[key]


def _deep_scratch(device, owner=None, nbytes=32 << 20):
    key = (device.type, device.index, owner, "deep")
    if key not in _SPLITK_WS:
        _SPLITK_WS[key] = torch.empty(nbytes // 4, dtype=torch.float32, device=device)
    return _SPLITK_WS[key]


def best_of(*calls, reps=5, key=None):
    if key is not None:
        hit = cache_get(key)
        if hit is not None and 0 <= int(hit) < len(calls):
            return calls[int(hit)]
    if DETERMINISTIC:
        return calls[0]

    def t(c):
        c()
        best = None
        for _ in range(3):
            e0, e1 = torch.cuda.Event(enable_timing=True), torch.cuda.Event(enable_timing=True)
            e0.record()
            for _ in range(reps):
                c()
            e1.record()
            e1.synchronize()
            best = e0.elapsed_time(e1) if best is None else min(best, e0.elapsed_time(e1))
        return best
    times = [t(c) for c in calls]
    if key is not None:
        cache_put(key, times.index(min(times)))
    return calls[times.index(min(times))]


GATHER_NARROW = L.ab("FALNET_GATHER_NARROW", "0") == "1"


def gather_bn(w_rows, Cout):
    return 128 if (w_rows % 128 == 0 and Cout > 64) else (64 if (w_rows % 64 == 0 and Cout > 32) else 32)


def conv_multi_call(calls, name="conv multi", bn=None, ksplit=1, s2d=False):
    lib = L.lib()
    if ksplit > 1 and DETERMINISTIC:
        raise ValueError("split-K is not available in deterministic mode")
    n = len(calls)
    arr = (L.Conv * n)()
    off = 0
    for i, c in enumerate(calls):
        C.memmove(C.byref(arr[i]), C.byref(c.desc), C.sizeof(L.Conv))
        arr[i].variant, arr[i].ksplit = (14 if s2d else {32: 11, 64: 12}.get(bn, 1)), ksplit
        if ksplit > 1:
            need = (arr[i].B * arr[i].TH * arr[i].TW * arr[i].w_rows * 4 + 255) // 256 * 256
            if not c.desc.splitk_ws or off + need > c.desc.splitk_ws_bytes or arr[i].Cout % 8:
                raise ValueError("split-K workspace too small for a fused multi launch")
            arr[i].splitk_ws = c.desc.splitk_ws + off
            arr[i].splitk_ws_bytes = need
            off += need
    keep = (arr, calls)
    dn = {L.BF16: "DF16b", L.F16: "DF16_"}.get(arr[0].dtype, "f")
    bn = bn or gather_bn(arr[0].w_rows, arr[0].Cout)

    def launch(_keep=keep):
        L.check(lib.falnet_conv2d_multi(arr, n, L.stream_ptr()), name)
    sym = f"_Z22conv3x3_s2d_dma_kernelI{dn}Ev13falnet_conv_tiiiii" if s2d else f"_Z23conv_igemm_multi_kernelI{dn}Li{bn}EEv14falnet_conv4_t"
    return _timed(sym, sum(c.flops for c in calls), 0, launch, name)


_AUTOTUNE_LOG = os.environ.get("FALNET_AUTOTUNE_LOG") == "1"


def _autotune_conv(lib, d, ref, M, w_rows, Cout, reps=3):
    st = L.stream_ptr()
    cands = [(1, 1)]
    bn = 128 if (w_rows % 128 == 0 and Cout > 64) else (64 if (w_rows % 64 == 0 and Cout > 32) else 32)
    wgs = ((M + 127) // 128) * ((Cout + bn - 1) // bn)
    if wgs < 256 and M * w_rows * 4 <= d.splitk_ws_bytes and Cout % 8 == 0:
        cands += [(1, k) for k in (2, 4, 8, 16) if wgs * k <= 2048]
    if wgs < 256 and GATHER_NARROW:
        for v, nb in ((12, 64), (11, 32)):
            if nb < bn and w_rows % nb == 0:
                w2 = ((M + 127) // 128) * ((Cout + nb - 1) // nb)
                cands += [(v, 1)]
                if M * w_rows * 4 <= d.splitk_ws_bytes and Cout % 8 == 0:
                    cands += [(v, k) for k in (2, 4) if w2 * k <= 2048]
    cands += [(2, 1), (3, 1), (4, 1), (6, 1), (7, 1), (10, 1)]
    if L.ab("FALNET_WS2", "1") == "1":
        cands += [(16, 1)]
    if L.ab("FALNET_NO_DMA", "0") != "1":
        cands += [(13, 1)]
        if L.ab("FALNET_DMA2", "0") == "1":
            cands += [(21, 1), (22, 1)]
        if L.ab("FALNET_DMA16", "1") == "1":
            cands += [(23, 1)]
            if wgs < int(L.ab("FALNET_SMALL_TILE_MAXWGS", "1024")):
                cands += [(24, 1), (25, 1)]
        if d.cin_total == 32 and w_rows == 32 and L.ab("FALNET_CONV_WAVE", "1") == "1":
            cands += [(27, 1)]
        if d.cin_total == 64 and d.out_layout == L.OUT_PLANAR_F32 and Cout <= 4 and L.ab("FALNET_CONV_WAVE", "1") == "1":
# ... 376 lines not shown
```

### include/falnet_hip.h

```cpp
#ifndef FALNET_HIP_H
#define FALNET_HIP_H

#include <stdint.h>

#ifdef __cplusplus
extern "C" {
#endif

enum { FALNET_F32 = 0, FALNET_BF16 = 1, FALNET_F16 = 2 };
enum { FALNET_ACT_NONE = 0, FALNET_ACT_ELU = 1, FALNET_ACT_RELU = 2 };
enum { FALNET_OUT_NHWC = 0, FALNET_OUT_PLANAR_F32 = 1 };

int falnet_version(void);
const char* falnet_last_error(void);
int falnet_channel_pad(int dtype);
int falnet_set_device(int device);
int falnet_set_deterministic(int on);
int falnet_get_deterministic(void);

typedef struct {
    const void* ptr;
    int32_t C;
    int32_t H, W;
    int64_t sb, sy, sx;
} falnet_src_t;

typedef struct {
    falnet_src_t src[2];
    int32_t nsrc;
    int32_t IH, IW;
    const void* weight;
    int32_t cin_total;
    int32_t ntaps;
    int32_t tap_dy[9], tap_dx[9], tap_w[9];
    int32_t w_taps;
    int32_t w_rows;
    int32_t isy, isx;
    int32_t B, TH, TW;
    int32_t osy, osx, ooy, oox;
    void* out;
    int32_t OH, OW;
    int32_t Cout;
    int32_t out_cstride;
    int32_t out_layout;
    const float* bias;
    const void* addend;
    int32_t act;
    const void* actout;
    int32_t actout_kind;
    int32_t dtype;
    int32_t ksplit;
    float* splitk_ws;
    int64_t splitk_ws_bytes;
    int32_t variant;
    void* pool_out;
    int32_t pool_mode;
    int32_t pool_actout_kind;
    const void* pool_actout;
    const void* weight_up2;
    void* scratch;
    int64_t scratch_bytes;
} falnet_conv_t;
int falnet_conv2d(const falnet_conv_t* p, void* stream);
int falnet_conv3x3_c3(const float* x_nchw, const float* w_oihw, const float* bias, void* out, int B, int H, int W, int Cout,
                      int act, int dtype, void* stream);
int falnet_conv2d_multi(const falnet_conv_t* descs, int n, void* stream);
int falnet_conv2d_kernel_name(const falnet_conv_t* p, char* buf, int len);

typedef struct {
    falnet_src_t src[2];
    int32_t nsrc;
    int32_t IH, IW;
    const void* gout;
    int32_t gC;
    int32_t ntaps;
    int32_t tap_dy[9], tap_dx[9];
    int32_t isy, isx;
    int32_t B, TH, TW;
    int32_t cin_total;
    int32_t nsplit;
    float* partial;
    int32_t dtype;
    int32_t variant;
    float* bias_grad;
    int32_t cout;
    int32_t up2;
} falnet_wgrad_t;
int falnet_wgrad_fuses_bias(const falnet_wgrad_t* p);
int64_t falnet_wgrad_workspace_bytes(const falnet_wgrad_t* p);
int falnet_wgrad(const falnet_wgrad_t* p, void* stream);
int falnet_wgrad_reduce(const float* partial, int nsplit, int ntaps, int cout_pad, int cin_total,
                        float* grad, int cout, int cin, int c0_real, int c0_pad, int accumulate, void* stream);
int falnet_bias_grad(const void* g, int64_t npix, int gC, int cout, float* db,
                     int accumulate, int dtype, void* stream);

int falnet_wgrad_reduce_blocks(int cout, int cin_total, int groups);
typedef struct {
    const float* partial; float* grad;
    int32_t nsplit, ntaps, w_rows, cin_total, cout, cin, c0_real, c0_pad, groups, block_begin;
} falnet_reduce_t;
typedef struct {
    const void* g; float* db; int64_t npix;
    int32_t gC, cout, blocks, block_begin;
} falnet_biasgrad_t;
typedef struct {
    const float* w; void* wf; void* wd;
    int32_t cout, cin, taps, c0_real, c0_pad, cin_pad, cout_pad, block_begin;
    int32_t no_update, reserved;
} falnet_pack_t;
int falnet_pack_weights_batched(const falnet_pack_t* descs_dev, int n, int total_blocks, int dtype, void* stream);
int falnet_adam_pack_batched(const falnet_pack_t* descs_dev, int n, int total_blocks, int dtype, int64_t g_off, int64_t m_off, int64_t v_off,
                             const float* state, float b1, float b2, float eps, float grad_scale, const float* scaler, void* stream);
int falnet_adam_ranges(float* p, int64_t g_off, int64_t m_off, int64_t v_off, const int64_t* ranges_dev, int n_ranges, const float* state,
                       float b1, float b2, float eps, float grad_scale, const float* scaler, void* stream);
int falnet_adam_tick(float* state, const float* scaler, void* stream);
int falnet_adam_pack_batched_wd(const falnet_pack_t* descs_dev, int n, int total_blocks, int dtype, int64_t g_off, int64_t m_off, int64_t v_off,
                                const float* state, float b1, float b2, float eps, float grad_scale, double weight_decay, const float* scaler,
                                void* stream);
int falnet_adam_ranges_wd(float* p, int64_t g_off, int64_t m_off, int64_t v_off, const int64_t* ranges_dev, const double* decays_dev, int n_ranges,
                          const float* state, float b1, float b2, float eps, float grad_scale, const float* scaler, void* stream);
typedef struct {
    const float* w; void* wu;
    int32_t cout, cin, cin_pad, cout_pad, block_begin;
    int32_t reserved;
    void* wdd;
} falnet_pack_up2_t;
int falnet_pack_up2_batched(const falnet_pack_up2_t* descs_dev, int n, int total_blocks, int dtype, void* stream);
int falnet_wgrad_reduce_batched(const falnet_reduce_t* descs_dev, int n, int total_blocks, int accumulate, void* stream);
int falnet_bias_grad_batched(const falnet_biasgrad_t* descs_dev, int n, int total_blocks, int dtype, void* stream);
int falnet_bias_grad_batched_det(const falnet_biasgrad_t* descs_dev, int n, int total_blocks, int dtype, float* ws, int64_t ws_floats,
                                 void* stream);

int falnet_pack_weights(const float* w_oihw, int cout, int cin, int taps,
                        int c0_real, int c0_pad, int cin_pad_total, int cout_pad,
                        void* wf, void* wd, int dtype, void* stream);

int falnet_nchw_to_nhwc(const float* src, void* dst, int B, int C, int H, int W, int Cpad,
                        int dtype, void* stream);
int falnet_nhwc_to_nchw(const void* src, float* dst, int B, int C, int H, int W, int Cpad,
                        int dtype, void* stream);
int falnet_upsample_bwd(const void* gup, void* gsrc, const void* actout, int B, int IH, int IW,
                        int H, int W, int C, int dtype, void* stream);
int falnet_wgrad_const_plane(const void* gout, const void* plane, int64_t plane_stride, float* grad, int64_t grad_co_stride, float* ws,
                             int B, int TH, int TW, int gC, int cout, int IH, int IW, int stride, int dtype, void* stream);
int falnet_maxpool2_fwd(const void* x, void* y, int B, int H, int W, int C, int dtype, void* stream);
int falnet_maxpool2_bwd(const void* x, const void* y, const void* gy, void* gx, int B, int H, int W, int C,
                        int dtype, void* stream);
int falnet_act_bwd(const void* g, const void* y, void* gx, int64_t n, int kind, int dtype, void* stream);

int falnet_med_head_fwd(const float* dlog0, const float* left, const float* min_disp, const float* max_disp,
                        float* disp, float* p_im0, float* stats, int B, int N, int H, int W, void* stream);
int falnet_med_head_bwd(const float* dlog0, const float* left, const float* min_disp, const float* max_disp,
                        const float* disp, const float* p_im0, const float* stats,
                        const float* grad_disp, const float* grad_p_im0, float* grad_dlog0,
                        int B, int N, int H, int W, void* stream);
int falnet_med_head_bwd_nhwc(const float* dlog0, const float* left, const float* min_disp, const float* max_disp,
                             const float* disp, const float* p_im0, const float* stats,
                             const float* grad_disp, const float* grad_p_im0, void* grad_dlog0_nhwc, int cpad, int dtype,
                             int B, int N, int H, int W, void* stream);
int falnet_med_head_kernel_name(int pass, int dtype, int N, int W, char* buf, int len);
int falnet_med_masks_fwd(const float* dlog0, const float* min_disp, const float* max_disp, const float* stats,
                         float* maskL, float* maskR, int B, int N, int H, int W, void* stream);
int falnet_med_maskr_acfalse_fwd(const float* dlog0, const float* min_disp, const float* max_disp, const float* stats,
                                 float* maskR, int B, int N, int H, int W, void* stream);

int falnet_l1_fwd(const float* a, const float* b, const float* mask, int B, int C, int64_t HW,
                  float scale, float* out, int accumulate, void* stream);
int falnet_l1_bwd(const float* a, const float* b, const float* mask, int B, int C, int64_t HW,
                  float scale, const float* gscale, float* ga, int accumulate, void* stream);
int falnet_mse_fwd(const void* a, const void* b, int64_t npix, int Cpad, float scale, float* out,
                   int accumulate, int dtype, void* stream);
int falnet_mse_bwd(const void* a, const void* b, int64_t npix, int Cpad, float scale, const float* gscale,
                   void* ga, int dtype, void* stream);
int falnet_smooth_fwd(const float* img, const float* disp, int B, int H, int W, int x0, int x1,
                      float gamma, float scale, float* out, int accumulate, void* stream);
int falnet_smooth_bwd(const float* img, const float* disp, int B, int H, int W, int x0, int x1,
                      float gamma, float scale, const float* gscale, float* gdisp, int accumulate, void* stream);
int falnet_l1_fwd_bwd(const float* a, const float* b, int B, int C, int64_t HW, float scale, float* out, const float* gscale, float* ga,
                      void* stream);
int falnet_l1_fwd_bwd_add(const float* a, const float* b, int B, int C, int64_t HW, float scale, float* out, const float* gscale,
                          const float* gadd, float* ga, void* stream);
int falnet_mse_fwd_bwd(const void* a, const void* b, int64_t npix, int Cpad, float scale_out, float* out, float scale_grad,
                       const float* gscale, void* ga, int dtype, void* stream);
int falnet_mse3_fwd_bwd(const void* const* a, const void* const* b, const int64_t* numel, const float* scale_out, float* out,
                        const float* scale_grad, const float* gscale, void* const* ga, int dtype, void* stream);
int falnet_smooth_fwd_bwd(const float* img, const float* disp, int B, int H, int W, int x0, int x1, float gamma, float scale, float* out,
                          const float* gscale, float* gdisp, void* stream);
int falnet_step_scalars(float* S, float a, float* out, void* stream);
int falnet_mask_mix(const float* a, const float* b, const float* m, float* out, int B, int C, int64_t HW, void* stream);

int falnet_adam_step(float* p, const float* g, float* m, float* v, int64_t n, float lr, float b1, float b2,
                     float eps, int step, float grad_scale, void* stream);

int falnet_adam_step_dev(float* p, const float* g, float* m, float* v, int64_t n, float* state, float b1, float b2,
                         float eps, float grad_scale, void* stream);

int falnet_grad_guard(const float* g, int64_t n, float* scaler, void* stream);
int falnet_adam_step_guarded(float* p, const float* g, float* m, float* v, int64_t n, float* state, float b1, float b2,
                             float eps, float grad_scale, const float* scaler, void* stream);
int falnet_adam_step_wd(float* p, const float* g, float* m, float* v, int64_t n, const int64_t* seg_end_dev, const double* seg_decay_dev, int n_seg,
                        float* state, float b1, float b2, float eps, float grad_scale, const float* scaler, void* stream);
int falnet_loss_scale_update(float* scaler, float growth, float backoff, int interval, float min_scale, float max_scale, void* stream);
int falnet_loss_seeds(const float* scaler, const float* coef, float* seeds, int n, void* stream);

int falnet_occlusion_mask(const float* a, const float* b, float* out, int B, int H, int W, int x0, int x1, void* stream);
int falnet_mirror_weight(const float* occ, const float* rowmax, float* out, int B, int H, int W, int x0, int x1, void* stream);
int falnet_hflip(const float* src, float* dst, int64_t n_rows, int W, void* stream);
int falnet_rowmax(const float* src, float* out, int B, int64_t n, void* stream);

int falnet_gemm_f32_small(const float* A, int64_t sam, int64_t sak, const float* B, int64_t sbk, int64_t sbn, float* C,
                          int M, int N, int K, int accumulate, void* stream);
int falnet_resize_planar(const float* src, float* dst, int64_t planes, int H, int W, int OH, int OW, int bilinear, float scale,
                         void* stream);

int falnet_disp_prologue(const float* max_disp, const float* min_disp, float mul, float div, float* min_out, float* max_out,
                         void* flow, int flow_stride, int B, int dtype, void* stream);

int falnet_resample_u8(const uint8_t* src, uint8_t* dst, int H, int W, int C, int out_size, int horizontal,
                       const int32_t* bounds, const int32_t* kk, int ksize, void* stream);
int falnet_augment_normalize(const uint8_t* src, int H, int W, int x1, int y1, int th, int tw, int flip, double gamma,
                             double bright, double cb0, double cb1, double cb2, float mean0, float mean1, float mean2,
                             float* dst, void* stream);

#define FALNET_AUG_MAX_SCALE 2
typedef struct {
    uint64_t src[2];
    int32_t H, W, rw, rh, x1, y1, flip, reserved;
    double gamma, bright, cb[2][3];
} falnet_aug_t;
int falnet_augment_batch(const falnet_aug_t* table_dev, const falnet_aug_t* table_host, int B, int th, int tw, float mean0, float mean1,
                         float mean2, float* out0, float* out1, void* stream);

#define FALNET_CMD_RECORD (-1)
#define FALNET_CMD_WAIT (-2)
typedef struct {
    int32_t op, stream, event, nint, nflt, reserved;
    uint64_t iarg[18];
    double farg[8];
} falnet_cmd_t;
#define FALNET_CMD_MAX_INT 18
#define FALNET_CMD_MAX_FLT 8
int falnet_replay_op_index(const char* name);
int falnet_replay_op_args(int op, int* nint, int* nflt);
int falnet_replay(const falnet_cmd_t* cmds, int n, void* const* streams, int nstreams, void* const* events, int nevents, int* failed_at);
int falnet_fill_f32(float* p, int64_t n, float value, void* stream);
int falnet_copy_bytes(void* dst, const void* src, int64_t nbytes, void* stream);
int falnet_spin(int microseconds, void* stream);
int falnet_mfma_probe(const void* ab, float* out, int iters, int dtype, void* stream);

int64_t falnet_percentile_workspace_bytes(int B);
int falnet_percentile_f32(const float* x, int64_t n_per_sample, int B, double q, float* out, void* workspace, void* stream);
int falnet_disp_to_plasma_u8(const float* disp, const float* p95, const void* lut_rgba, void* out_rgba, int B, int H, int W, void* stream);
int falnet_image_to_u8(const float* x, float mean_r, float mean_g, float mean_b, void* out, int B, int H, int W, void* stream);
int falnet_feature_to_u8(const float* x, void* out, int64_t n, void* stream);
int falnet_local_norm(const float* x, float mean_r, float mean_g, float mean_b, float* out, float* mu_out, float* sigma_out, int win, int B, int H, int W,
                      void* stream);
int falnet_point_cloud(const float* img, float mean_r, float mean_g, float mean_b, float rgb_scale, const float* disp, double focal, double baseline,
                       float* out_planar, void* out_packed, int B, int H, int W, void* stream);

#define FALNET_DEPTH_KITTI2015 0
#define FALNET_DEPTH_EIGEN 1
#define FALNET_DEPTH_MAKE3D 2
#define FALNET_MET_ROW 24
#define FALNET_MET_ABS_REL 0
#define FALNET_MET_SQ_REL 1
#define FALNET_MET_RMS 2
#define FALNET_MET_LOG 3
#define FALNET_MET_A1 4
#define FALNET_MET_A2 5
#define FALNET_MET_A3 6
#define FALNET_MET_N 7
#define FALNET_MET_N_A1 8
#define FALNET_MET_N_A2 9
#define FALNET_MET_N_A3 10
#define FALNET_MET_SCALE 11
#define FALNET_MET_MEDIAN_GT 12
#define FALNET_MET_MEDIAN_PRED 13
#define FALNET_MET_EPE 14
#define FALNET_MET_EPE_N 15
#define FALNET_MET_RMSE 16
#define FALNET_MET_MEA 17
#define FALNET_MET_PSNR 18
#define FALNET_MET_VIEW_SUM_SQ 19
#define FALNET_MET_VIEW_SUM_ABS 20
#define FALNET_MET_VIEW_SUM_RSQ 21
#define FALNET_MET_VIEW_N 22
int64_t falnet_metrics_workspace_bytes(void);
int falnet_depth_median_scale(const float* pred_disp, const float* gt, int H, int W, int mode, double fb, double max_d, double* scale_out,
                              void* workspace, void* stream);
int falnet_depth_errors(const float* pred_disp, const float* gt, int H, int W, int mode, double fb, const double* scale, double min_d, double max_d,
                        double* row, void* workspace, void* stream);
int falnet_epe(const float* pred, int h, int w, const float* target, int B, int H, int W, int sparse, double* row, void* workspace, void* stream);
int falnet_view_errors(const float* out, const float* label, float mean_r, float mean_g, float mean_b, int B, int H, int W, double* row, void* workspace,
                       void* stream);

#ifdef __cplusplus
}
#endif
#endif
```

Baseline: 1600 stereo-pairs/s.

## Store argmax codes from fused VGG max-pool instead of full pre-pool activation

In the VGG perceptual-loss forward, the last conv of each block now writes 4-bit argmax codes (with a ReLU-positive mask) for its fused 2x2 max pool, in place of the full-resolution pre-pool activation. The backward pass scatters the pooled gradient through these codes with a new kernel, so it no longer re-reads the full activation and the pooled output. This is meant to drop a large activation write in forward and a large read in backward. It forces variant 23 (dma16) for these convs, which may not be the autotuned best choice, and it rounds values to 16-bit before comparing so ties resolve consistently.

```diff
diff --git a/fal_net_amd/_lib.py b/fal_net_amd/_lib.py
--- a/fal_net_amd/_lib.py
+++ b/fal_net_amd/_lib.py
@@ -38,7 +38,7 @@
                 ("actout_kind", C.c_int32), ("dtype", C.c_int32), ("ksplit", C.c_int32), ("splitk_ws", C.c_void_p),
                 ("splitk_ws_bytes", C.c_int64), ("variant", C.c_int32), ("pool_out", C.c_void_p),
                 ("pool_mode", C.c_int32), ("pool_actout_kind", C.c_int32), ("pool_actout", C.c_void_p), ("weight_up2", C.c_void_p),
-                ("scratch", C.c_void_p), ("scratch_bytes", C.c_int64)]
+                ("scratch", C.c_void_p), ("scratch_bytes", C.c_int64), ("pool_code", C.c_void_p)]
 
 
 class Wgrad(C.Structure):
@@ -121,6 +121,7 @@
     "falnet_wgrad_const_plane": [_P, _P, _L, _P, _L, _P, _I, _I, _I, _I, _I, _I, _I, _I, _I, _P],
     "falnet_maxpool2_fwd": [_P, _P, _I, _I, _I, _I, _I, _P],
     "falnet_maxpool2_bwd": [_P, _P, _P, _P, _I, _I, _I, _I, _I, _P],
+    "falnet_maxpool2_bwd_codes": [_P, _P, _P, _I, _I, _I, _I, _I, _P],
     "falnet_act_bwd": [_P, _P, _P, _L, _I, _I, _P],
     "falnet_med_head_fwd": [_P, _P, _P, _P, _P, _P, _P, _I, _I, _I, _I, _P],
     "falnet_med_head_bwd": [_P, _P, _P, _P, _P, _P, _P, _P, _P, _P, _I, _I, _I, _I, _P],
diff --git a/fal_net_amd/csrc/conv.hip b/fal_net_amd/csrc/conv.hip
--- a/fal_net_amd/csrc/conv.hip
+++ b/fal_net_amd/csrc/conv.hip
@@ -1502,6 +1502,12 @@
         }
         variant = 1;
     }
+    if (p.pool_code && !(variant == 23 && p.dtype != FALNET_F32 && p.pool_out && p.pool_mode == 0 && !planar && p.OH % 2 == 0 && p.OW % 2 == 0 &&
+                         p.Cout % 32 == 0 && p.out_cstride % 32 == 0)) {
+        falnet_set_error("conv2d: pool_code (argmax codes of the fused max pool) needs variant 23, a 16-bit type, pool_out with pool_mode 0, an NHWC "
+                         "launch with even OH / OW and whole 32-channel groups (variant %d, dtype %d, pool_mode %d)", p.variant, p.dtype, p.pool_mode);
+        return -2;
+    }
     if (g_disable_patch) variant = 1;
     switch (variant) {
         case 0: case 1: case 2: case 3: case 4: case 5: case 6: case 7: case 8: case 9: case 10:
@@ -1780,7 +1786,10 @@
     {ConvFamily::Up2Dma, SYMBOL("_Z22conv3x3_up2_dma_kernelI%sEv13falnet_conv_tiiiii", t), LAUNCH(falnet_conv_up2_dma_launch(p, st))},
     {ConvFamily::Deep, SYMBOL("_Z19conv3x3_deep_kernelI%sLi%dELi%dEEv13falnet_conv_t18falnet_deep_geom_t", t, c.kcb, c.nwaves), LAUNCH(falnet_conv_deep_launch(p, st))},
     {ConvFamily::Dma2, SYMBOL("_Z19conv3x3_dma2_kernelI%sLb%dELi%dEEv13falnet_conv_tiiiii", t, p.pool_out ? 1 : 0, c.nwaves), LAUNCH(falnet_conv_dma2_launch(p, c.flip, st, c.th))},
-    {ConvFamily::Dma16, SYMBOL("_Z20conv3x3_dma16_kernelI%sLb%dELi%dELi%dELb%dEEv13falnet_conv_tiiii", t, p.pool_out ? 1 : 0, c.th, c.nwaves, p.out_layout == FALNET_OUT_PLANAR_F32 ? 1 : 0),
+    {ConvFamily::Dma16, [](char* buf, int len, const char* t, const falnet_conv_t& p, const ConvChoice& c) {
+         if (p.pool_out && p.pool_code) return snprintf(buf, len, "_Z20conv3x3_dma16_kernelI9PoolCodesI%sELb1ELi16ELi8ELb0EEv13falnet_conv_tiiii", t);
+         return snprintf(buf, len, "_Z20conv3x3_dma16_kernelI%sLb%dELi%dELi%dELb%dEEv13falnet_conv_tiiii", t, p.pool_out ? 1 : 0, c.th, c.nwaves, p.out_layout == FALNET_OUT_PLANAR_F32 ? 1 : 0);
+     },
      LAUNCH(falnet_conv_dma16_launch(p, c.flip, st, c.th))},
     {ConvFamily::Up2d, SYMBOL("_Z25conv2x2_up2d_dma16_kernelI%sEv13falnet_conv_tiii", t), LAUNCH(falnet_conv_up2d_launch(p, st))},
     {ConvFamily::Wave32, SYMBOL("_Z21conv3x3_wave32_kernelI%sEv13falnet_conv_tiiii", t), LAUNCH(falnet_conv_wave32_launch(p, c.flip, st))},
diff --git a/fal_net_amd/csrc/conv_dma.hip b/fal_net_amd/csrc/conv_dma.hip
--- a/fal_net_amd/csrc/conv_dma.hip
+++ b/fal_net_amd/csrc/conv_dma.hip
@@ -578,8 +578,13 @@
     FALNET_RETURN_LAUNCH();
 }
 
-template <typename T, bool POOL, int TH, int NWAVES, bool PLANAR>
+template <typename T> struct PoolCodes {};
+template <typename TT> struct Dma16Operand { typedef TT type; static constexpr bool codes = false; };
+template <typename T> struct Dma16Operand<PoolCodes<T>> { typedef T type; static constexpr bool codes = true; };
+template <typename TT, bool POOL, int TH, int NWAVES, bool PLANAR>
 __global__ __launch_bounds__(NWAVES * 64, NWAVES == 8 ? 2 : 1) void conv3x3_dma16_kernel(const falnet_conv_t p, int tiles_x, int tiles_y, int flip, int ntiles) {
+    typedef typename Dma16Operand<TT>::type T;
+    constexpr bool CODES = Dma16Operand<TT>::codes;
     constexpr int MT = TH / NWAVES, BN = 64, NT = BN / 32;
     static_assert(sizeof(T) == 2 && (MT == 1 || MT == 2) && (MT == 2 || !POOL), "16-bit operands; one or two rows per wave; the fused pool needs row pairs");
     constexpr int KCV = 32;
@@ -843,7 +848,7 @@
                     acc[mt][nt].to32(v[mt][0]);
                     acc[mt][nt].zero();
                 }
-                if constexpr (POOL) epilogue_direct<T, MT, 1, decltype(pixoff), decltype(pooloff), -1, false, true>(p, v, bias, n0 + 32 * nt, lane, pixoff, pooloff);
+                if constexpr (POOL) epilogue_direct<T, MT, 1, decltype(pixoff), decltype(pooloff), -1, false, true, false, CODES>(p, v, bias, n0 + 32 * nt, lane, pixoff, pooloff);
                 else epilogue_direct<T, MT, 1, decltype(pixoff), NoPool, (PLANAR ? -1 : FALNET_DMA16_EPI_AHEAD), false, !PLANAR, PLANAR>(p, v, bias, n0 + 32 * nt, lane, pixoff);
                 if (nt == 0) CD16_B();
             }
@@ -872,6 +877,7 @@
         if (th == 4) DMA16_K(T, false, 4, 4, false);      \
         else if (th == 8) DMA16_K(T, false, 8, 8, false); \
         else if (planar) DMA16_K(T, false, 16, 8, true);  \
+        else if (p.pool_out && p.pool_code) DMA16_K(PoolCodes<T>, true, 16, 8, false); \
         else if (p.pool_out) DMA16_K(T, true, 16, 8, false); \
         else DMA16_K(T, false, 16, 8, false);             \
     } while (0)
diff --git a/fal_net_amd/csrc/conv_epilogue.h b/fal_net_amd/csrc/conv_epilogue.h
--- a/fal_net_amd/csrc/conv_epilogue.h
+++ b/fal_net_amd/csrc/conv_epilogue.h
@@ -259,7 +259,8 @@
 __device__ __forceinline__ float lane_xor1(float v) {
     return __int_as_float(__builtin_amdgcn_mov_dpp(__float_as_int(v), 0xB1, 0xF, 0xF, true));
 }
-template <typename T, int MT, int NT, typename PixOff, typename PoolOff = NoPool, int AHEAD = 1, bool DEFER = false, bool NHWC_ONLY = false, bool PLANAR_PTR = false>
+template <typename T, int MT, int NT, typename PixOff, typename PoolOff = NoPool, int AHEAD = 1, bool DEFER = false, bool NHWC_ONLY = false, bool PLANAR_PTR = false,
+          bool CODES = false>
 __device__ __forceinline__ void epilogue_direct(const falnet_conv_t& p, f32x16 (&acc)[MT][NT], const float (&bias)[NT][16], int nbase, int lane,
                                                 PixOff pixoff, PoolOff pooloff = PoolOff(), PackedOut<T, MT, NT>* defer = nullptr) {
     constexpr bool POOL = !std::is_same<PoolOff, NoPool>::value;
@@ -274,6 +275,7 @@
     for (int nt = 0; nt < NT; ++nt) {
         const int cbase = nbase + nt * 32;
         float hp[16];
+        [[maybe_unused]] bool top_right[CODES ? 16 : 1];
         constexpr int NR = AHEAD < 0 ? 1 : 1 + AHEAD;
         TileRaw<T> ra[NR], rb[NR];
         if (AHEAD > 0) {
@@ -304,6 +306,10 @@
                 if constexpr (AHEAD < 0) tile_load<T>(actout, o, cbase, h, p.Cout, a);
                 else tile_unpack<T>(rb[mt & (AHEAD < 0 ? 0 : AHEAD)], a);
                 actgrad16(v, a, p.actout_kind);
+            }
+            if constexpr (CODES) {
+#pragma unroll
+                for (int j = 0; j < 16; ++j) v[j] = to_f32(from_f32<T>(v[j]));
             }
             if constexpr (DEFER) {
                 tile_pack<T>(v, defer->out[mt][nt]);
@@ -329,7 +335,41 @@
                     }
                 }
             } else if (!POOL || out) tile_store<T>(out, o, cbase, h, p.Cout, v);
-            if constexpr (POOL) {
+            if constexpr (POOL && CODES) {
+                static_assert(!DEFER && sizeof(T) == 2 && MT % 2 == 0, "argmax codes: direct stores, 16-bit types, row pairs");
+                if (pooling) {
+                    float m[16];
+                    bool right[16];
+#pragma unroll
+                    for (int j = 0; j < 16; ++j) {
+                        const float n = lane_xor1(v[j]);
+                        right[j] = n > v[j];
+                        m[j] = fmaxf(v[j], n);
+                    }
+                    if ((mt & 1) == 0) {
+#pragma unroll
+                        for (int j = 0; j < 16; ++j) {
+                            hp[j] = m[j];
+                            top_right[j] = right[j];
+                        }
+                    } else {
+                        unsigned cw[2] = {0u, 0u};
+#pragma unroll
+                        for (int j = 0; j < 16; ++j) {
+                            const bool lower = m[j] > hp[j];
+                            m[j] = fmaxf(m[j], hp[j]);
+                            const unsigned nib = m[j] > 0.f ? (lower ? (right[j] ? 8u : 4u) : (top_right[j] ? 2u : 1u)) : 0u;
+                            cw[j >> 3] |= nib << (4 * (j & 7));
+                        }
+                        const int64_t po = (lane & 1) ? (int64_t)-1 : pooloff(mt);
+                        tile_store<T>(pool_out, po, cbase, h, p.Cout, m);
+                        half_swap(cw[0], cw[1]);
+                        const unsigned c0 = (cw[0] & 0xffffu) | (cw[1] << 16), c1 = (cw[0] >> 16) | (cw[1] & 0xffff0000u);
+                        if (po >= 0 && cbase + 16 * h < p.Cout)
+                            *reinterpret_cast<uint2*>(reinterpret_cast<char*>(p.pool_code) + (po >> 1) + (cbase >> 1) + 8 * h) = make_uint2(c0, c1);
+                    }
+                }
+            } else if constexpr (POOL) {
                 if (pooling) {
                     float m[16];
                     if (psum) {
diff --git a/fal_net_amd/csrc/elementwise.hip b/fal_net_amd/csrc/elementwise.hip
--- a/fal_net_amd/csrc/elementwise.hip
+++ b/fal_net_amd/csrc/elementwise.hip
@@ -193,6 +193,28 @@
 }
 
 template <typename T>
+__global__ __launch_bounds__(EW_THREADS) void maxpool2_bwd_codes_kernel(const unsigned char* __restrict__ codes, const T* __restrict__ gy,
+                                                                        T* __restrict__ gx, int B, int H, int W, int C) {
+    const int OH = H / 2, OW = W / 2, cg = C / 8;
+    const int64_t total = (int64_t)B * OH * OW * cg;
+    for (int64_t i = (int64_t)blockIdx.x * blockDim.x + threadIdx.x; i < total; i += (int64_t)gridDim.x * blockDim.x) {
+        const int c0 = (int)(i % cg) * 8, ox = (int)((i / cg) % OW), oy = (int)((i / ((int64_t)cg * OW)) % OH);
+        const int b = (int)(i / ((int64_t)cg * OW * OH));
+        const int64_t base = (((int64_t)b * H + 2 * oy) * W + 2 * ox) * C + c0;
+        const int64_t off[4] = {0, C, (int64_t)W * C, (int64_t)W * C + C};
+        const unsigned code = *reinterpret_cast<const unsigned*>(codes + i * 4);
+        float g[8], o[4][8];
+        load8_as(gy + (((int64_t)b * OH + oy) * OW + ox) * C + c0, g);
+#pragma unroll
+        for (int e = 0; e < 8; ++e)
+#pragma unroll
+            for (int j = 0; j < 4; ++j) o[j][e] = ((code >> (4 * e + j)) & 1u) ? g[e] : 0.f;
+#pragma unroll
+        for (int j = 0; j < 4; ++j) store8_as(gx + base + off[j], o[j]);
+    }
+}
+
+template <typename T>
 __global__ __launch_bounds__(EW_THREADS) void act_bwd_kernel(const T* __restrict__ g, const T* __restrict__ y,
                                                              T* __restrict__ gx, int64_t n, int kind) {
     for (int64_t i = (int64_t)blockIdx.x * blockDim.x + threadIdx.x; i < n; i += (int64_t)gridDim.x * blockDim.x) {
@@ -376,6 +398,20 @@
     }
     const int64_t total = (int64_t)B * (H / 2) * (W / 2) * C;
 #define EW_L(T) hipLaunchKernelGGL(maxpool2_bwd_kernel<T>, dim3(ew_grid(total)), dim3(EW_THREADS), 0, (hipStream_t)stream, (const T*)x, (const T*)gy, (T*)gx, B, H, W, C)
+    FALNET_DISPATCH_DTYPE(dtype, EW_L);
+#undef EW_L
+    FALNET_RETURN_LAUNCH();
+}
+
+extern "C" int falnet_maxpool2_bwd_codes(const void* codes, const void* gy, void* gx, int B, int H, int W, int C, int dtype, void* stream) {
+    FALNET_ENTER(stream);
+    FALNET_CHECK_ARG(codes && gy && gx && B > 0 && H >= 2 && W >= 2 && H % 2 == 0 && W % 2 == 0 && C > 0,
+                     "maxpool2_bwd_codes: bad argument (even H, W required)");
+    FALNET_CHECK_ARG(dtype == FALNET_F32 || dtype == FALNET_BF16 || dtype == FALNET_F16, "maxpool2_bwd_codes: bad dtype %d", dtype);
+    FALNET_CHECK_ARG(C % 8 == 0 && (((uintptr_t)gy | (uintptr_t)gx) & 15) == 0 && ((uintptr_t)codes & 3) == 0,
+                     "maxpool2_bwd_codes: C must be a multiple of 8, gy / gx 16-B and codes 4-B aligned");
+    const int64_t tv = (int64_t)B * (H / 2) * (W / 2) * (C / 8);
+#define EW_L(T) hipLaunchKernelGGL(maxpool2_bwd_codes_kernel<T>, dim3(ew_grid(tv)), dim3(EW_THREADS), 0, (hipStream_t)stream, (const unsigned char*)codes, (const T*)gy, (T*)gx, B, H, W, C)
     FALNET_DISPATCH_DTYPE(dtype, EW_L);
 #undef EW_L
     FALNET_RETURN_LAUNCH();
diff --git a/fal_net_amd/csrc/replay.cpp b/fal_net_amd/csrc/replay.cpp
--- a/fal_net_amd/csrc/replay.cpp
+++ b/fal_net_amd/csrc/replay.cpp
@@ -67,7 +67,7 @@
     FALNET_OP(falnet_mirror_weight), FALNET_OP(falnet_hflip), FALNET_OP(falnet_rowmax), FALNET_OP(falnet_gemm_f32_small),
     FALNET_OP(falnet_resize_planar), FALNET_OP(falnet_disp_prologue), FALNET_OP(falnet_resample_u8), FALNET_OP(falnet_augment_normalize),
     FALNET_OP(falnet_fill_f32), FALNET_OP(falnet_copy_bytes), FALNET_OP(falnet_spin), FALNET_OP(falnet_adam_pack_batched_wd),
-    FALNET_OP(falnet_adam_ranges_wd), FALNET_OP(falnet_adam_step_wd), FALNET_OP(falnet_augment_batch),
+    FALNET_OP(falnet_adam_ranges_wd), FALNET_OP(falnet_adam_step_wd), FALNET_OP(falnet_augment_batch), FALNET_OP(falnet_maxpool2_bwd_codes),
 };
 constexpr int g_nops = (int)(sizeof(g_ops) / sizeof(g_ops[0]));
 
diff --git a/fal_net_amd/loss_functions.py b/fal_net_amd/loss_functions.py
--- a/fal_net_amd/loss_functions.py
+++ b/fal_net_amd/loss_functions.py
@@ -29,9 +29,12 @@
 
 class _VggPlan:
 
-    def __init__(self, owner, B, H, W, dtype, device, need_grad=True):
+    def __init__(self, owner, B, H, W, dtype, device, need_grad=True, pool_codes=None, pool_variant=None):
         self.B, self.H, self.W, self.dtype, self.device = B, H, W, dtype, device
         self.busy, self.need_grad, self.gen = False, need_grad, 0
+        if pool_codes is None:
+            pool_codes = L.ab("FALNET_POOL_CODES", "1") == "1"
+        self.pool_maps, self.pool_codes = [], []
         code = L.dtype_code(dtype)
         self.fwd, self.bwd = [], []
         _conv = lambda *a, **kw: ops.conv_call(*a, ws_owner=("vgg", id(self)), **kw)
@@ -46,16 +49,27 @@
                 pc = pcs[idx]
                 last = idx == convs[-1]
                 pooled = torch.empty(B, h // 2, w // 2, pc.cout, dtype=dtype, device=device) if last else None
-                y = torch.empty(B, h, w, pc.cout, dtype=dtype, device=device) if (need_grad or not last) else None
+                codes = None
                 kw = dict(bias=pc.bias, act=L.ACT_RELU, name=f"vgg conv{idx}", flops=2 * B * h * w * pc.cout * pc.cin * 9)
                 args = (dtype, [ops.nhwc_src(cur)], h, w, pc.wf, pc.cin_pad, ops.fwd_taps(3), 9, pc.cout_pad, 1, B, h, w)
                 fused = False
-                if cur is x0:
+                fuse_pool = last and cur is not x0 and L.ab("FALNET_FUSED_POOL", "1") == "1"
+                if fuse_pool and need_grad and pool_codes:
+                    try:
+                        codes = torch.empty(B, h // 2, w // 2, pc.cout // 2, dtype=torch.uint8, device=device)
+                        self.fwd.append(_conv(*args, None, h, w, pc.cout, pc.cout, pool_out=pooled, pool_code=codes, variant=23, **kw))
+                        fused = True
+                    except ValueError:
+                        codes = None
+                y = torch.empty(B, h, w, pc.cout, dtype=dtype, device=device) if ((need_grad and codes is None) or not last) else None
+                if fused:
+                    pass
+                elif cur is x0:
                     self.c3_call = ops.conv_c3_call(dtype, x_in, pc, y, L.ACT_RELU, name="vgg conv0(c3)")
                     self.fwd.append(self.c3_call)
-                elif last and L.ab("FALNET_FUSED_POOL", "1") == "1":
+                elif fuse_pool:
                     try:
-                        self.fwd.append(_conv(*args, y, h, w, pc.cout, pc.cout, pool_out=pooled, **kw))
+                        self.fwd.append(_conv(*args, y, h, w, pc.cout, pc.cout, pool_out=pooled, variant=pool_variant if need_grad else None, **kw))
                         fused = True
                     except ValueError:
                         pass
@@ -67,7 +81,9 @@
                     self.fwd.append(ops.simple_call("falnet_maxpool2_fwd", L.ptr(y), L.ptr(pooled), B, h, w, pc.cout, code))
                 acts.append((pc, cur, y, h, w))
                 cur = y
-            acts.append(("pool", cur, pooled, h, w))
+            acts.append(("pool", cur, pooled, h, w, codes))
+            self.pool_maps.append(cur)
+            self.pool_codes.append(codes)
             self.outs.append(pooled)
             cur, h, w = pooled, h // 2, w // 2
         self.run_fwd = ops.ReplayList(self.fwd, eager_head=1)
@@ -82,11 +98,15 @@
         slice_i = len(self.outs) - 1
         for entry in reversed(acts):
             if entry[0] == "pool":
-                _, x, pooled, h, w = entry
+                _, x, pooled, h, w, codes = entry
                 gy = self.gouts[slice_i] if g_next is None else g_next
-                gx = torch.empty_like(x)
-                self.bwd.append(ops.simple_call("falnet_maxpool2_bwd", L.ptr(x), L.ptr(pooled), L.ptr(gy), L.ptr(gx), B, h, w,
-                                                x.shape[3], code))
+                ch = pooled.shape[3]
+                gx = torch.empty(B, h, w, ch, dtype=dtype, device=device)
+                if codes is not None:
+                    self.bwd.append(ops.simple_call("falnet_maxpool2_bwd_codes", L.ptr(codes), L.ptr(gy), L.ptr(gx), B, h, w, ch, code))
+                    self.keep.append(codes)
+                else:
+                    self.bwd.append(ops.simple_call("falnet_maxpool2_bwd", L.ptr(x), L.ptr(pooled), L.ptr(gy), L.ptr(gx), B, h, w, ch, code))
                 g_next, slice_i = gx, slice_i - 1
                 self.keep.append(gx)
             else:
diff --git a/fal_net_amd/ops.py b/fal_net_amd/ops.py
--- a/fal_net_amd/ops.py
+++ b/fal_net_amd/ops.py
@@ -326,7 +326,7 @@
               Cout, out_cstride, out_layout=L.OUT_NHWC, out_step=(1, 1, 0, 0), bias=None, addend=None,
               act=L.ACT_NONE, actout=None, actout_kind=L.ACT_NONE, weight_offset_elems=0, name="conv", flops=0,
               autotune=True, ws_owner=None, pool_out=None, pool_mode=0, pool_actout=None, pool_actout_kind=L.ACT_NONE, weight_up2=None,
-              variant=None):
+              variant=None, pool_code=None):
     lib = L.lib()
     d = L.Conv()
     d.nsrc = len(srcs)
@@ -344,6 +344,7 @@
     d.pool_mode, d.pool_actout_kind = pool_mode, pool_actout_kind
     d.pool_actout = 0 if pool_actout is None else pool_actout.data_ptr()
     d.weight_up2 = 0 if weight_up2 is None else weight_up2.data_ptr()
+    d.pool_code = 0 if pool_code is None else pool_code.data_ptr()
     dev_t = out if out is not None else pool_out
     d.bias = 0 if bias is None else bias.data_ptr()
     d.addend = 0 if addend is None else addend.data_ptr()
@@ -361,7 +362,7 @@
         scratch = _deep_scratch(dev_t.device, ws_owner)
         d.scratch, d.scratch_bytes = scratch.data_ptr(), scratch.numel() * 4
     ref = C.byref(d)
-    keep = (d, srcs, weight, out, bias, addend, actout, ws, pool_out, pool_actout, weight_up2, scratch)
+    keep = (d, srcs, weight, out, bias, addend, actout, ws, pool_out, pool_actout, weight_up2, scratch, pool_code)
     if variant is not None:
         d.variant = variant
         if lib.falnet_conv2d_kernel_name(ref, C.create_string_buffer(160), 160) != 0:
diff --git a/include/falnet_hip.h b/include/falnet_hip.h
--- a/include/falnet_hip.h
+++ b/include/falnet_hip.h
@@ -60,6 +60,7 @@
     const void* weight_up2;
     void* scratch;
     int64_t scratch_bytes;
+    void* pool_code;
 } falnet_conv_t;
 int falnet_conv2d(const falnet_conv_t* p, void* stream);
 int falnet_conv3x3_c3(const float* x_nchw, const float* w_oihw, const float* bias, void* out, int B, int H, int W, int Cout,
@@ -146,6 +147,7 @@
 int falnet_maxpool2_fwd(const void* x, void* y, int B, int H, int W, int C, int dtype, void* stream);
 int falnet_maxpool2_bwd(const void* x, const void* y, const void* gy, void* gx, int B, int H, int W, int C,
                         int dtype, void* stream);
+int falnet_maxpool2_bwd_codes(const void* codes, const void* gy, void* gx, int B, int H, int W, int C, int dtype, void* stream);
 int falnet_act_bwd(const void* g, const void* y, void* gx, int64_t n, int kind, int dtype, void* stream);
 
 int falnet_med_head_fwd(const float* dlog0, const float* left, const float* min_disp, const float* max_disp,
```

After: 1631 stereo-pairs/s (median of 6 runs). 1.9% higher.
